# Michaelszeng/GCS-ADMM

Hardware: AMD Instinct MI355X
Metric: admm_iterations_per_sec (higher is better)
Workload: dtype f64; 1 GPU; benchmark4; V=42, E=94, n=2, state_dtype=f64, state_columns=incidence, inner_arithmetic=f64, vertex_program=workgroup, vertex_solves=warm start from the previous iteration's record (csrc/warm_start.h), parallelism=1 GPU

## Files before the change

### gcs_admm_amd/abi.py

```python
from __future__ import annotations

import ctypes as C
import os

import numpy as np

LIB_PATH = os.path.join(os.path.dirname(os.path.abspath(__file__)), "libgcsadmm.so")

F64, F32 = 0, 1
RUNNING, CONVERGED, MAX_IT, DIVERGED = -1, 0, 1, 2
BATCH_LARGE = 1
BATCH_TERMINALS = 4
STATUS_NAME = {RUNNING: "running", CONVERGED: "converged", MAX_IT: "max_it", DIVERGED: "diverged"}


class GraphDesc(C.Structure):
    _fields_ = [("n", C.c_int32), ("num_vertices", C.c_int32), ("num_edges", C.c_int32), ("num_incidences", C.c_int32),
                ("inc_ptr", C.c_void_p), ("inc_edge", C.c_void_p), ("inc_out", C.c_void_p),
                ("edge_inc_tail", C.c_void_p), ("edge_inc_head", C.c_void_p),
                ("poly_ptr", C.c_void_p), ("poly_A", C.c_void_p), ("poly_b", C.c_void_p), ("center", C.c_void_p),
                ("src", C.c_int32), ("dst", C.c_int32), ("state_dtype", C.c_int32), ("device", C.c_int32),
                ("inc_counted", C.c_void_p), ("edge_counted", C.c_void_p),
                ("nx_global", C.c_double), ("nmu_global", C.c_double),
                ("vertex_program", C.c_int32), ("wave_slots", C.c_int32), ("wave_align", C.c_int32),
                ("wave_store_dl", C.c_int32), ("wave_generic_rows", C.c_int32), ("edge_major_columns", C.c_int32),
                ("vertex_workspace", C.c_int32)]


class Params(C.Structure):
    _fields_ = [("rho", C.c_double), ("tau_incr", C.c_double), ("tau_decr", C.c_double), ("nu", C.c_double),
                ("it_rho_limit", C.c_int32), ("max_it", C.c_int32), ("eps_abs", C.c_double), ("eps_rel", C.c_double),
                ("eps_edge", C.c_double), ("ipm_tol", C.c_double), ("ipm_max_iter", C.c_int32), ("cold_start", C.c_int32)]


class State(C.Structure):
    _fields_ = [("copy", C.c_void_p), ("mu", C.c_void_p), ("zedge", C.c_void_p),
                ("xv", C.c_void_p), ("zv", C.c_void_p), ("yv", C.c_void_p)]


class HaloDesc(C.Structure):
    _fields_ = [("num_peers", C.c_int32), ("peer_rank", C.c_void_p), ("send_ptr", C.c_void_p), ("send_cols", C.c_void_p),
                ("recv_ptr", C.c_void_p), ("recv_cols", C.c_void_p)]


class ControlBlock(C.Structure):
    _fields_ = [("rho", C.c_double), ("mu_scale", C.c_double), ("sums", C.c_double * 5),
                ("pri", C.c_double), ("dual", C.c_double), ("eps_pri", C.c_double), ("eps_dual", C.c_double),
                ("it", C.c_int32), ("status", C.c_int32), ("inner_failures", C.c_int32), ("inner_iters", C.c_int32)]


class Snapshot(C.Structure):
    _fields_ = [("n", C.c_int32), ("state_dtype", C.c_int32), ("V", C.c_int32), ("E", C.c_int32),
                ("edge_key", C.c_void_p), ("edge_words", C.c_void_p), ("vertex_id", C.c_void_p), ("vertex_words", C.c_void_p),
                ("rho", C.c_void_p)]


_p, _i, _d = C.c_void_p, C.c_int32, C.c_double
_run, _run_timed = [_p, _p, _i, _p, _p], [_p, _p, _i, _p, _p] + [_p] * 4
_csr = [_i, _i, _p, _p, _p]
PROTOTYPES = {
    "gcsadmm_create": ([_p, _p], _i),
    "gcsadmm_destroy": ([_p], None),
    "gcsadmm_last_error": ([_p], C.c_char_p),
    "gcsadmm_reset": ([_p] * 3, _i),
    "gcsadmm_vertex_step": ([_p] * 3, _i),
    "gcsadmm_edge_step": ([_p] * 4, _i),
    "gcsadmm_control": ([_p] * 4, _i),
    "gcsadmm_run": (_run, _i),
    "gcsadmm_set_fused_tail": ([_p, _i], _i),
    "gcsadmm_read_control": ([_p] * 3, _i),
    "gcsadmm_cost": ([_p, _p, _d, _p, _p], _i),
    "gcsadmm_query": ([_p] * 6, _i),
    "gcsadmm_query_workspace": ([_p] * 4, _i),
    "gcsadmm_unit_iterations": ([_p, _p, _i, _p, _p], _i),
    "gcsadmm_run_timed": (_run_timed, _i),
    "gcsadmm_batch_create": ([_p, _i, _p], _i),
    "gcsadmm_batch_create_ex": ([_p, _i, _i, _p], _i),
    "gcsadmm_batch_query": ([_p] * 4, _i),
    "gcsadmm_batch_query_terminals": ([_p] * 3, _i),
    "gcsadmm_batch_destroy": ([_p], None),
    "gcsadmm_batch_last_error": ([_p], C.c_char_p),
    "gcsadmm_batch_bind": ([_p] * 4, _i),
    "gcsadmm_batch_run": ([_p, _i, _p], _i),
    "gcsadmm_batch_poll": ([_p] * 4, _i),
    "gcsadmm_export_state": ([_p] * 5, _i),
    "gcsadmm_import_state": ([_p] * 5, _i),
    "gcsadmm_batch_export_state": ([_p] * 4, _i),
    "gcsadmm_batch_import_state": ([_p] * 4, _i),
    "gcsadmm_vertex_prox": ([_p] * 6 + [_d, _i, _p, _p], _i),
    "gcsadmm_comm_unique_id": ([_p], _i),
    "gcsadmm_attach_comm": ([_p, _i, _i, _p, _p], _i),
    "gcsadmm_check_halo": ([_p, _i, _i, _p], _i),
    "gcsadmm_run_partitioned": (_run, _i),
    "gcsadmm_run_partitioned_timed": (_run_timed, _i),
    "gcsadmm_set_overlap": ([_p, _i, _p], _i),
    "gcsadmm_comm_count": ([_p, _p], _i),
    "gcsadmm_halo_pack": ([_p] * 3, _i),
    "gcsadmm_halo_unpack": ([_p] * 3, _i),
    "gcsadmm_halo_exchange": ([_p] * 3, _i),
    "gcsadmm_halo_buffers": ([_p] * 4, _i),
    "gcsadmm_polytope_last_error": ([], C.c_char_p),
    "gcsadmm_polytope_centers": (_csr + [_i, _p, _p, _p], _i),
    "gcsadmm_polytope_bounds": (_csr + [_p, _i, _p, _p, _p], _i),
    "gcsadmm_polytope_overlaps": (_csr + [_p, C.c_long, _p, _p, _d, _i, _p, _p], _i),
    "gcsadmm_scene_create": (_csr + [_i, _p], _i),
    "gcsadmm_scene_destroy": ([_p], None),
    "gcsadmm_scene_centers": ([_p] * 4, _i),
    "gcsadmm_scene_bounds": ([_p] * 4, _i),
    "gcsadmm_scene_set_boxes": ([_p] * 3, _i),
    "gcsadmm_scene_candidate_pairs": ([_p, _d, _p], _i),
    "gcsadmm_scene_overlaps": ([_p, _d, _p, _p], _i),
    "gcsadmm_scene_read_pairs": ([_p] * 5, _i),
    "gcsadmm_scene_restrict_paths": ([_p, _i, _p, _p, _p, _d, _i, _p, _p, _p, _p], _i),
    "gcsadmm_scene_locate_points": ([_p, _i, _p, _d, _d, _p], _i),
    "gcsadmm_scene_locate_boxes": ([_p, _i, _p, _p, _d, _p], _i),
    "gcsadmm_scene_read_hits": ([_p] * 4, _i),
    "gcsadmm_scene_project_points": ([_p, _i, _p, _p, _i, _p], _i),
    "gcsadmm_scene_read_projections": ([_p] * 5, _i),
    "gcsadmm_scene_add_regions": ([_p, _i, _p, _p, _p, _d, _d] + [_p] * 6, _i),
    "gcsadmm_scene_remove_regions": ([_p, _i, _p, _p], _i),
    "gcsadmm_scene_read_regions": ([_p] * 7, _i),
    "gcsadmm_scene_build_region_graph": ([_p] * 3, _i),
    "gcsadmm_scene_read_region_graph": ([_p] * 5, _i),
    "gcsadmm_scene_query_graphs": ([_p, _i, _p, _p, _p, _i] + [_p] * 8, _i),
    "gcsadmm_scene_region_paths": ([_p, _i, _p, _p, _p, _i] + [_p] * 4, _i),
    "gcsadmm_scene_informed_regions": ([_p, _i, _p, _p, _d, _p, _p], _i),
    "gcsadmm_scene_region_paths_sets": ([_p, _i, _p, _p, _p, _p, _i] + [_p] * 4, _i),
    "gcsadmm_scene_informed_regions_sets": ([_p, _i, _p, _p, _p, _d, _p, _p], _i),
    "gcsadmm_scene_induced_sizes": ([_p, _i] + [_p] * 6, _i),
    "gcsadmm_scene_induced_query_graphs": ([_p, _i, _p, _p, _p, _p, _i] + [_p] * 9, _i),
    "gcsadmm_walks_create": ([_i] + [_p] * 7 + [_i, _p], _i),
    "gcsadmm_walks_destroy": ([_p], None),
    "gcsadmm_walks_last_error": ([_p], C.c_char_p),
    "gcsadmm_walks_sample": ([_p, _p, _i, _p, _i, _i, _i] + [_p] * 4, _i),
}
EXPORTS = list(PROTOTYPES)


class GcsAdmmError(RuntimeError):
    pass


def check(status, message):
    if status:
        raise GcsAdmmError(message())


_lib = None


def select_library(path: str) -> None:
    global LIB_PATH
    path = os.path.abspath(path)
    if _lib is not None and _lib._name != path:
        raise RuntimeError(f"{_lib._name} is already loaded: select {path} before the first handle is made")
    LIB_PATH = path


def load_library() -> C.CDLL:
    global _lib
    if _lib is None:
        if not os.path.exists(LIB_PATH):
            raise RuntimeError(f"{LIB_PATH} is missing: run `python -m gcs_admm_amd.build` (hipcc, gfx950). "
                               "There is no CPU fallback.")
        import torch
        lib = C.CDLL(LIB_PATH)
        for name, (argtypes, restype) in PROTOTYPES.items():
            f = getattr(lib, name)
            f.argtypes, f.restype = argtypes, restype
        _lib = lib
    return _lib


def graph_desc(g, *, state_dtype, device, num_incidences=None, inc_counted=None, edge_counted=None, nx_global=0.0,
               nmu_global=0.0, columns="incidence", **knobs):
    if columns not in ("incidence", "edge"):
        raise ValueError("columns must be 'incidence' or 'edge'")
    E = g.num_edges
    NI = int(num_incidences) if num_incidences is not None else int(g.inc_ptr[-1])
    tail, head = g.edge_inc_tail.astype(np.int32), g.edge_inc_head.astype(np.int32)
    col_of = np.arange(NI, dtype=np.int64)
    if columns == "edge":
        if NI != 2 * E:
            raise ValueError("edge-major columns need exactly two columns per edge")
        col_of = np.empty(NI, dtype=np.int64)
        col_of[tail] = np.arange(E); col_of[head] = E + np.arange(E)
        tail, head = np.arange(E, dtype=np.int32), (E + np.arange(E)).astype(np.int32)
        if inc_counted is not None:
            ic = np.empty(NI, dtype=np.uint8)
            ic[col_of] = np.asarray(inc_counted, dtype=np.uint8)
            inc_counted = ic
    arrays = dict(inc_ptr=g.inc_ptr.astype(np.int32), inc_edge=g.inc_edge.astype(np.int32), inc_out=g.inc_out.astype(np.int32),
                  edge_inc_tail=tail, edge_inc_head=head, poly_ptr=g.poly_ptr.astype(np.int32), poly_A=g.poly_A.astype(np.float64),
                  poly_b=g.poly_b.astype(np.float64), center=g.interior.astype(np.float64),
                  inc_counted=None if inc_counted is None else np.asarray(inc_counted, dtype=np.uint8),
                  edge_counted=None if edge_counted is None else np.asarray(edge_counted, dtype=np.uint8))
    arrays = {k: None if a is None else np.ascontiguousarray(a) for k, a in arrays.items()}
    desc = GraphDesc(n=g.n, num_vertices=g.num_vertices, num_edges=E, num_incidences=NI, src=g.src, dst=g.dst,
                     state_dtype=state_dtype, device=device, nx_global=float(nx_global), nmu_global=float(nmu_global),
                     edge_major_columns=int(columns == "edge"), **{k: int(v) for k, v in knobs.items()},
                     **{k: None if a is None else a.ctypes.data for k, a in arrays.items()})
    return desc, list(arrays.values()), col_of
```

### gcs_admm_amd/csrc/create_plan.h

```cpp
#pragma once
#include <algorithm>
#include <cmath>
#include <string>
#include <vector>

#include "canonical_box.h"
#include "gcsadmm.h"
#include "state_transfer_core.h"
#include "step_args.h"
#include "vertex_program.h"
#include "warm_start.h"

int gcsadmm_wg_lds_bytes(int n, int units, int facets, bool box = false);
int gcsadmm_wg_lds_bytes_t512(int n, int units, int facets, bool box = false);
bool gcsadmm_wg_has_box(int n);
long long gcsadmm_terminal_ws_doubles(int n, int facets, int live_edges);
long long gcsadmm_terminal_record_doubles(int n, int facets, int live_edges);

namespace gcsadmm_k {

constexpr int REORDER_MIN_UNITS = 512;
constexpr int LDS_CU_BYTES = 160 * 1024;

inline int edge_unroll_rt(int dtype, int c, int E)
{
    const int u = dtype == GCSADMM_F32 ? (c <= 7 ? 4 : 2) : (c <= 7 ? 2 : 1);
    return (E + EDGE_BLOCK * u - 1) / (EDGE_BLOCK * u) >= 256 ? u : 1;
}

struct CreatePlan {
    std::vector<int> deg_in;
    std::vector<double> bc;
    std::vector<int> special_vtx, special_kind;
    int n_term = 0, term_vtx[2] = {-1, -1}, term_is_src[2] = {0, 0};
    long long term_ws_off[2] = {0, 0}, term_rec_off[2] = {0, 0}, term_ws_doubles = 0, term_rec_doubles = 0;
    int term_threads = 256, term_lds_doubles = 0;
    std::vector<int> wg_vtx;
    int wg_lds_bytes = 0, wg_box = 0, wg_t512 = 0;
    std::vector<int> split_vtx;
    std::vector<long long> split_off;
    long long split_doubles = 0;
    int split_lds_bytes = 0;
    std::vector<int> wave_slot_ptr{0}, wave_vtx;
    int slots_cap = 1, align_rows = 0, store_dl = 0, all_m4 = 0;
    int wave_mm = 1;
    int lds_bytes = 0;
    std::vector<long long> warm_ptr;
    bool wave_reorder = false, wg_reorder = false;
    std::vector<int> prox_vtx;
    int prox_lds_bytes = 0;
    std::vector<char> col_owned;
    std::vector<int> col_vertex;
    double nx = 0, nmu = 0;
    int edge_unroll = 1, edge_blocks = 1;
    int fused_tail = 0;
    std::vector<int> edge_tail, edge_head;
    int edges_ascending = 0;
    int n_waves() const { return (int)wave_slot_ptr.size() - 1; }
};

inline gcsadmm_status check_graph_desc(const gcsadmm_graph_desc *g, std::string &err)
{
    auto fail = [&](gcsadmm_status st, const char *msg) { err = msg; return st; };
    if (!g) return fail(GCSADMM_ERR_BAD_ARG, "null descriptor or output pointer");
    if (g->n < 1 || g->n > 8) return fail(GCSADMM_ERR_UNSUPPORTED, "the vertex kernels are instantiated for n = 1 .. 8");
    if (g->num_vertices < 0 || g->num_edges < 0) return fail(GCSADMM_ERR_BAD_ARG, "negative size");
    if (!g->inc_ptr || !g->poly_ptr || (g->num_edges > 0 && (!g->inc_edge || !g->inc_out || !g->edge_inc_tail || !g->edge_inc_head)) ||
        (g->num_vertices > 0 && (!g->poly_A || !g->poly_b || !g->center)))
        return fail(GCSADMM_ERR_BAD_ARG, "null graph array");
    if (g->state_dtype != GCSADMM_F64 && g->state_dtype != GCSADMM_F32) return fail(GCSADMM_ERR_BAD_ARG, "bad state_dtype");
    const int NIo = g->inc_ptr[g->num_vertices];
    if (g->inc_ptr[0] != 0 || NIo < 0 || g->num_incidences < NIo) return fail(GCSADMM_ERR_BAD_ARG, "inconsistent incidence CSR");
    return GCSADMM_OK;
}

inline gcsadmm_status make_create_plan(const gcsadmm_graph_desc &g, CreatePlan &p, std::string &err)
{
    auto fail = [&](gcsadmm_status st, const char *msg) { err = msg; return st; };
    const int V = g.num_vertices, E = g.num_edges, n = g.n;
    p = CreatePlan();

    std::vector<int> deg(V), fac(V);
    p.deg_in.assign(V, 0);
    int mm_all = 1;
    for (int v = 0; v < V; ++v) {
        const int lo = g.inc_ptr[v], hi = g.inc_ptr[v + 1];
        if (hi < lo) return fail(GCSADMM_ERR_BAD_ARG, "inc_ptr not monotone");
        bool seen_out = false;
        for (int k = lo; k < hi; ++k) {
            if (g.inc_edge[k] < 0 || g.inc_edge[k] >= E) return fail(GCSADMM_ERR_BAD_ARG, "inc_edge out of range");
            if (g.inc_out[k]) seen_out = true;
            else { if (seen_out) return fail(GCSADMM_ERR_BAD_ARG, "incoming incidences must precede outgoing ones"); p.deg_in[v]++; }
        }
        deg[v] = hi - lo;
        fac[v] = g.poly_ptr[v + 1] - g.poly_ptr[v];
        if (fac[v] < n + 1) return fail(GCSADMM_ERR_BAD_ARG, "polytope with fewer than n+1 facets cannot be bounded");
        mm_all = std::max(mm_all, fac[v]);
    }
    for (int e = 0; e < E; ++e)
        if (g.edge_inc_tail[e] < 0 || g.edge_inc_tail[e] >= g.num_incidences || g.edge_inc_head[e] < 0 || g.edge_inc_head[e] >= g.num_incidences)
            return fail(GCSADMM_ERR_BAD_ARG, "edge incidence slot out of range");
    if (g.edge_major_columns != 0 && g.edge_major_columns != 1) return fail(GCSADMM_ERR_BAD_ARG, "edge_major_columns must be 0 or 1");
    if (g.edge_major_columns) {
        if (g.num_incidences != 2 * (int64_t)E) return fail(GCSADMM_ERR_BAD_ARG, "edge-major columns: num_incidences must be 2 num_edges");
        for (int e = 0; e < E; ++e)
            if (g.edge_inc_tail[e] != e || g.edge_inc_head[e] != E + e)
                return fail(GCSADMM_ERR_BAD_ARG, "edge-major columns: edge_inc_tail[e] must be e and edge_inc_head[e] num_edges + e");
    }
    p.edge_tail.assign(E, -1); p.edge_head.assign(E, -1);
    for (int v = 0; v < V; ++v)
        for (int k = g.inc_ptr[v]; k < g.inc_ptr[v + 1]; ++k) (g.inc_out[k] ? p.edge_tail : p.edge_head)[g.inc_edge[k]] = v;
    p.edges_ascending = transfer_edges_ascend(E, p.edge_tail.data(), p.edge_head.data());
    auto poly_A = [&](int v) { return g.poly_A + (size_t)g.poly_ptr[v] * n; };

    const int MT = g.poly_ptr[V];
    p.bc.assign(MT > 0 ? MT : 1, 0.0);
    for (int v = 0; v < V; ++v)
        for (int j = g.poly_ptr[v]; j < g.poly_ptr[v + 1]; ++j) {
            double s = g.poly_b[j];
            for (int k = 0; k < n; ++k) s -= g.poly_A[(size_t)j * n + k] * g.center[(size_t)v * n + k];
            p.bc[j] = s;
            if (v != g.src && v != g.dst && !(s > 0.0)) return fail(GCSADMM_ERR_BAD_ARG, "center is not strictly inside its polytope");
        }

    auto live_edges = [&](int v, bool is_src) { return is_src ? deg[v] - p.deg_in[v] : p.deg_in[v]; };
    for (int term : {g.src, g.dst}) {
        if (term < 0 || term >= V) continue;
        double ext = 0;
        for (int j = g.poly_ptr[term]; j < g.poly_ptr[term + 1]; ++j) {
            double nrm = 0;
            for (int k = 0; k < n; ++k) nrm += g.poly_A[(size_t)j * n + k] * g.poly_A[(size_t)j * n + k];
            ext = std::max(ext, std::fabs(p.bc[j]) / std::sqrt(nrm > 0 ? nrm : 1.0));
        }
        if (ext > 1e-5) {
            if (g.src == g.dst) return fail(GCSADMM_ERR_UNSUPPORTED, "source and target are the same region");
            if (live_edges(term, term == g.src) < 1)
                return fail(GCSADMM_ERR_UNSUPPORTED, "a terminal that is a region needs an edge on its live side (outgoing for the source, incoming for the target)");
            p.term_vtx[p.n_term] = term; p.term_is_src[p.n_term] = term == g.src; ++p.n_term;
        }
    }
    auto is_region_terminal = [&](int v) { return (p.n_term > 0 && v == p.term_vtx[0]) || (p.n_term > 1 && v == p.term_vtx[1]); };
    auto is_special = [&](int v) { return v == g.src || v == g.dst || p.deg_in[v] == 0 || deg[v] - p.deg_in[v] == 0; };
    int n_generic = 0;
    for (int v = 0; v < V; ++v) n_generic += !is_region_terminal(v) && !is_special(v);
    constexpr int WG_AUTO_MAX = 1024;
    if (g.vertex_program < 0 || g.vertex_program > 3) return fail(GCSADMM_ERR_BAD_ARG, "vertex_program must be 0, 1, 2 or 3");
    if (g.vertex_workspace < 0 || g.vertex_workspace > 2) return fail(GCSADMM_ERR_BAD_ARG, "vertex_workspace must be 0, 1 or 2");
    const int ws_mode = g.vertex_workspace;
    const bool prefer_wg = g.vertex_program >= 2 || (g.vertex_program == 0 && n_generic <= WG_AUTO_MAX);
    bool wg_box = g.wave_generic_rows == 0 && gcsadmm_wg_has_box(n);
    bool wave_box = n == 2 && g.wave_generic_rows != 1 && g.wave_generic_rows != 2;
    std::vector<int> wave_cand;
    p.warm_ptr.assign(V + 1, 0);
    for (int v = 0; v < V; ++v) {
        p.warm_ptr[v + 1] = p.warm_ptr[v];
        if (is_region_terminal(v)) continue;
        if (is_special(v)) {
            if (deg[v] > MAX_SPECIAL_DEG) return fail(GCSADMM_ERR_UNSUPPORTED, "terminal vertex degree above 256");
            p.special_vtx.push_back(v);
            p.special_kind.push_back(v == g.src ? 1 : (v == g.dst ? 2 : 0));
            continue;
        }
        p.warm_ptr[v + 1] += gcs_ws::warm_record_doubles(n, fac[v], deg[v]);
        const bool wave_too_small = ws_mode == 1 && n == 2 && (size_t)gcs::lds_doubles(n, fac[v], 1, 0) * 8 > (size_t)LDS_CU_BYTES;
        if (n != 2 || deg[v] + 1 > gcs::WAVE || prefer_wg || wave_too_small) {
            p.wg_vtx.push_back(v);
            if (wg_box && !canonical_box(n, fac[v], poly_A(v))) wg_box = false;
        } else {
            wave_cand.push_back(v);
            p.wave_mm = std::max(p.wave_mm, fac[v]);
            if (wave_box && !canonical_box(2, fac[v], poly_A(v))) wave_box = false;
        }
    }

    const int n_wg = (int)p.wg_vtx.size();
    p.wg_t512 = n_wg > 0 && g.vertex_program != 3 && n_wg + 1 <= 256;
    p.wg_box = n_wg > 0 && wg_box;
    auto wg_bytes = [&](int v) { return p.wg_t512 ? gcsadmm_wg_lds_bytes_t512(n, deg[v] + 1, fac[v], wg_box)
                                                  : gcsadmm_wg_lds_bytes(n, deg[v] + 1, fac[v], wg_box); };
    if (ws_mode > 0) {
        std::vector<int> keep;
        for (int v : p.wg_vtx) (ws_mode == 2 || wg_bytes(v) > LDS_CU_BYTES ? p.split_vtx : keep).push_back(v);
        p.wg_vtx.swap(keep);
    }
    for (int v : p.wg_vtx) p.wg_lds_bytes = std::max(p.wg_lds_bytes, wg_bytes(v));
    if (p.wg_lds_bytes > LDS_CU_BYTES) return fail(GCSADMM_ERR_UNSUPPORTED, "a vertex sub-problem (degree x facets) does not fit the 160 KB of LDS of a CU");
    auto heavier = [&](int a, int b) { return (long)(deg[a] + 1) * fac[a] > (long)(deg[b] + 1) * fac[b]; };
    std::stable_sort(p.wg_vtx.begin(), p.wg_vtx.end(), heavier);
    std::stable_sort(p.split_vtx.begin(), p.split_vtx.end(), heavier);
    for (int v : p.split_vtx) {
        const int lds = gcsadmm_wg_lds_bytes(n, 0, fac[v], wg_box);
        if (lds > LDS_CU_BYTES) return fail(GCSADMM_ERR_UNSUPPORTED, "a vertex's border system and polytope do not fit the 160 KB of LDS of a CU");
        p.split_lds_bytes = std::max(p.split_lds_bytes, lds);
        p.split_off.push_back(p.split_doubles);
        p.split_doubles += ((gcsadmm_wg_lds_bytes(n, deg[v] + 1, fac[v], wg_box) - lds) / 8 + 31) / 32 * 32;
    }

    auto lds_need = [&](int slots, int store_dl) {
        return (size_t)(wave_box ? gcs_box::lds_doubles(n, p.wave_mm, slots, store_dl) : gcs::lds_doubles(n, p.wave_mm, slots, store_dl)) * 8;
    };
    int slots_max = gcs::MAX_SLOTS;
    if (!wave_cand.empty()) {
        while (slots_max > 1 && lds_need(slots_max, 0) > LDS_CU_BYTES) --slots_max;
        if (lds_need(slots_max, 0) > LDS_CU_BYTES) return fail(GCSADMM_ERR_UNSUPPORTED, "facet count too large for LDS");
        if (g.wave_slots > 0) slots_max = std::max(1, std::min(slots_max, (int)g.wave_slots));
        else slots_max = std::min(slots_max, std::max(1, ((int)wave_cand.size() + 1023) / 1024));
    }
    auto pack = [&](int align) {
        p.wave_slot_ptr.assign(1, 0); p.wave_vtx.clear();
        int lanes = 0, slots = 0, slots_used = 0;
        for (int v : wave_cand) {
            int base = gcs::group_base(lanes, deg[v], p.deg_in[v], align);
            if (base < 0 || slots + 1 > slots_max) {
                p.wave_slot_ptr.push_back((int)p.wave_vtx.size());
                slots = 0;
                base = gcs::group_base(0, deg[v], p.deg_in[v], align);
            }
            p.wave_vtx.push_back(v);
            lanes = base + deg[v] + 1; slots += 1;
            slots_used = std::max(slots_used, slots);
        }
        if ((int)p.wave_vtx.size() > p.wave_slot_ptr.back()) p.wave_slot_ptr.push_back((int)p.wave_vtx.size());
        p.slots_cap = std::max(1, slots_used);
    };
    pack(1);
    p.align_rows = g.wave_align == 1 ? 1 : (g.wave_align == 2 ? 0 : (p.n_waves() > 2048 ? 0 : 1));
    if (!p.align_rows) pack(0);
    p.all_m4 = wave_box ? 2 : 0;
    if (p.n_waves() > 0) {
        p.store_dl = g.wave_store_dl == 1 ? 1 : (g.wave_store_dl == 2 ? 0 : (lds_need(p.slots_cap, 1) <= 40 * 1024 ? 1 : 0));
        if (p.store_dl && lds_need(p.slots_cap, 1) > LDS_CU_BYTES) p.store_dl = 0;
        p.lds_bytes = (int)lds_need(p.slots_cap, p.store_dl);
    }

    long long largest = 0;
    int rows = 0;
    for (int i = 0; i < p.n_term; ++i) {
        const int v = p.term_vtx[i], live = live_edges(v, p.term_is_src[i]);
        const long long need = gcsadmm_terminal_ws_doubles(n, fac[v], live);
        p.term_ws_off[i] = p.term_ws_doubles; p.term_ws_doubles += need; largest = std::max(largest, need);
        p.term_rec_off[i] = p.term_rec_doubles; p.term_rec_doubles += gcsadmm_terminal_record_doubles(n, fac[v], live);
        rows = std::max(rows, live * 2 * fac[v]);
    }
    if (p.n_term > 0) {
        p.term_lds_doubles = largest * 8 <= 48 * 1024 ? (int)largest : 0;
        p.term_threads = rows <= 256 ? 64 : 256;
    }

    p.wave_reorder = p.n_waves() >= REORDER_MIN_UNITS;
    p.wg_reorder = n_wg >= REORDER_MIN_UNITS;
    for (int v = 0; v < V; ++v)
        if (v != g.src && v != g.dst) p.prox_vtx.push_back(v);
    p.prox_lds_bytes = gcsadmm_wg_lds_bytes(n, 1, mm_all);

    const size_t ncol = (size_t)std::max<int64_t>(g.num_incidences, 1);
    p.col_owned.assign(ncol, 0);
    p.col_vertex.assign(ncol, -1);
    for (int v = 0; v < V; ++v)
        for (int k = g.inc_ptr[v]; k < g.inc_ptr[v + 1]; ++k) {
            const int col = state_column(g.edge_major_columns, E, 0, k, g.inc_edge[k], g.inc_out[k]);
            p.col_owned[col] = 1; p.col_vertex[col] = v;
        }
    p.nx = g.nx_global > 0 ? g.nx_global : (4.0 * n + 1) * (V + 2.0 * E);
    p.nmu = g.nmu_global > 0 ? g.nmu_global : (4.0 * n + 2) * E;
    p.edge_unroll = edge_unroll_rt(g.state_dtype, 2 * n + 1, E);
    const int tile = EDGE_BLOCK * p.edge_unroll;
    p.edge_blocks = std::max(1, std::min((E + tile - 1) / tile, 2048));
    const bool partitioned = g.num_incidences > g.inc_ptr[V] || g.inc_counted != nullptr || g.edge_counted != nullptr;
    p.fused_tail = p.edge_blocks == 1 && E <= EDGE_BLOCK && p.n_waves() == 0 && p.split_vtx.empty() && p.n_term == 0 && !p.wg_vtx.empty() && !partitioned;
    return GCSADMM_OK;
}

}
```

### gcs_admm_amd/csrc/edge_step.h

```cpp
#pragma once
#include <hip/hip_runtime.h>

#include <cstdint>

#include "gcsadmm.h"
#include "step_args.h"

namespace gcsadmm_k {

constexpr int EDGE_WAVE = 64;

template <class T> struct EdgeArgs {
    int E, NI, c;
    const int *edge_inc_tail, *edge_inc_head;
    const uint8_t *inc_counted, *edge_counted;
    const T *copy;
    T *zedge, *mu;
    double *partials;
};
template <class U, class V> EdgeArgs<U> retype(const EdgeArgs<V> &a)
{
    return EdgeArgs<U>{a.E, a.NI, a.c, a.edge_inc_tail, a.edge_inc_head, a.inc_counted, a.edge_counted, (const U *)a.copy, (U *)a.zedge, (U *)a.mu, a.partials};
}

__device__ __forceinline__ double wave_sum(double v)
{
#pragma unroll
    for (int off = 32; off > 0; off >>= 1) v += __shfl_down(v, off, 64);
    return v;
}

__device__ __forceinline__ double scaled_plus(double scale, double x, double r)
{
#pragma clang fp contract(off)
    return scale * x + r;
}

struct ControlParams {
    double tau_incr, tau_decr, nu, eps_abs, eps_rel, nx, nmu;
    int it_rho_limit, max_it;
};

struct EdgeInKernel {
    static constexpr bool TAIL = false;
    template <class T> static __device__ __forceinline__ T load_copy(const T *p) { return *p; }
    static __device__ __forceinline__ int load_counter(const int *p) { return *p; }
    static __device__ __forceinline__ void store_counter(int *p, int v) { *p = v; }
    static __device__ __forceinline__ bool edge_thread() { return true; }
    static __device__ __forceinline__ void sync() { __syncthreads(); }
};
struct EdgeInTail {
    static constexpr bool TAIL = true;
    template <class T> static __device__ __forceinline__ T load_copy(const T *p) { return __hip_atomic_load(p, __ATOMIC_RELAXED, __HIP_MEMORY_SCOPE_AGENT); }
    static __device__ __forceinline__ int load_counter(const int *p) { return __hip_atomic_load(p, __ATOMIC_RELAXED, __HIP_MEMORY_SCOPE_AGENT); }
    static __device__ __forceinline__ void store_counter(int *p, int v) { __hip_atomic_store(p, v, __ATOMIC_RELAXED, __HIP_MEMORY_SCOPE_AGENT); }
    static __device__ __forceinline__ bool edge_thread() { return threadIdx.x < (unsigned)EDGE_BLOCK; }
    static __device__ __forceinline__ void sync() { __syncthreads(); }
};

struct EdgePre {
    int it = 0, ih = 0;
    double mu_scale = 1.0;
};
template <class T> __device__ __forceinline__ EdgePre edge_prefetch(const EdgeArgs<T> &a, double mu_scale)
{
    EdgePre p;
    p.mu_scale = mu_scale;
    if (threadIdx.x < (unsigned)EDGE_BLOCK && a.E > 0) {
        const int e = (int)threadIdx.x, ee = e < a.E ? e : a.E - 1;
        p.it = a.edge_inc_tail ? a.edge_inc_tail[ee] : ee; p.ih = a.edge_inc_head ? a.edge_inc_head[ee] : a.E + ee;
    }
    return p;
}

template <class P = EdgeInKernel>
__device__ void control_body(gcsadmm_control_block *cb, const double *sums, const ControlParams &p, int *counters, double *trace,
                             bool global_fails = false)
{
    if (cb->status != GCSADMM_RUNNING) return;
    double s[5];
    for (int k = 0; k < 5; ++k) { s[k] = sums[k]; cb->sums[k] = s[k]; }
    const int it = cb->it;
    double rho = cb->rho;
    const int fails = global_fails ? (int)(sums[5] + 0.5) : P::load_counter(&counters[0]), iters = P::load_counter(&counters[1]);
    P::store_counter(&counters[0], 0); P::store_counter(&counters[1], 0);
    cb->inner_failures = fails; cb->inner_iters = iters;
    const double tot = s[0] + s[1] + s[2] + s[3] + s[4];
    if (!(fabs(tot) <= 1.7976931348623157e308)) {
        cb->status = GCSADMM_DIVERGED;
        return;
    }
    const double pri = sqrt(s[0]), dual = rho * sqrt(2.0 * s[1]);
    double mu_scale = 1.0;
    if (pri >= p.nu * dual && it < p.it_rho_limit) { rho *= p.tau_incr; mu_scale = 1.0 / p.tau_incr; }
    else if (dual >= p.nu * pri && it < p.it_rho_limit) { rho *= 1.0 / p.tau_decr; mu_scale = p.tau_incr; }
    const double eps_pri = sqrt(p.nx) * p.eps_abs + p.eps_rel * fmax(sqrt(s[2]), sqrt(2.0 * s[3]));
    const double eps_dual = sqrt(p.nmu) * p.eps_abs + p.eps_rel * mu_scale * sqrt(s[4]);
    cb->rho = rho; cb->mu_scale = mu_scale;
    cb->pri = pri; cb->dual = dual; cb->eps_pri = eps_pri; cb->eps_dual = eps_dual;
    if (trace) {
        double *tr = trace + (size_t)(it - 1) * 6;
        tr[0] = rho; tr[1] = pri; tr[2] = dual; tr[3] = eps_pri; tr[4] = eps_dual; tr[5] = (double)fails;
    }
    if (pri < eps_pri && dual < eps_dual) { cb->status = GCSADMM_CONVERGED; return; }
    cb->it = it + 1;
    if (it + 1 > p.max_it) cb->status = GCSADMM_MAX_IT;
}

template <class T, int C> __host__ __device__ constexpr int edge_unroll() { return sizeof(T) == 4 ? (C <= 7 ? 4 : 2) : (C <= 7 ? 2 : 1); }

template <class T>
__device__ __forceinline__ void edge_word(const EdgeArgs<T> &a, int w, int e, int it, int ih, T cu_t, T cw_t, T zo_t, T mu_t, T mw_t, double mu_scale,
                                          double we, double wt, double wh, double (&s)[5])
{
    const double cu = (double)cu_t, cw = (double)cw_t, zo = (double)zo_t;
    const T zn_t = (T)(0.5 * (cu + cw));
    const double zn = (double)zn_t;
    const double ru = cu - zn, rw = cw - zn;
    const T mu_u_t = (T)scaled_plus(mu_scale, (double)mu_t, ru);
    const T mu_w_t = (T)scaled_plus(mu_scale, (double)mw_t, rw);
    a.mu[(size_t)w * a.NI + it] = mu_u_t;
    a.mu[(size_t)w * a.NI + ih] = mu_w_t;
    a.zedge[(size_t)w * a.E + e] = zn_t;
    const double mu_u = (double)mu_u_t, mu_w = (double)mu_w_t;
    s[0] += wt * ru * ru + wh * rw * rw;
    s[1] += we * (zn - zo) * (zn - zo);
    s[2] += wt * cu * cu + wh * cw * cw;
    s[3] += we * zn * zn;
    s[4] += wt * mu_u * mu_u + wh * mu_w * mu_w;
}

#ifndef GCS_TAIL_WORDS
#define GCS_TAIL_WORDS 5
#endif
template <class T, int C> __host__ __device__ constexpr int tail_words() { return C < GCS_TAIL_WORDS ? C : GCS_TAIL_WORDS; }

template <class T, int MODE, int C, int U, class P = EdgeInKernel>
__device__ __forceinline__ void edge_body(const EdgeArgs<T> &a, gcsadmm_control_block *cb, double *sums, const ControlParams &cp, int *counters,
                                          double *trace, unsigned *ticket, const unsigned bx, const unsigned nblocks, double (*red)[5], int *is_last,
                                          const EdgePre &pre = EdgePre())
{
    static_assert(!P::TAIL || (MODE == 1 && U == 1), "the tail of the vertex launch is the single-workgroup edge step");
    double mu_scale;
    if constexpr (P::TAIL) mu_scale = pre.mu_scale;
    else {
        if (cb->status != GCSADMM_RUNNING) return;
        mu_scale = cb->mu_scale;
    }
    double s[5] = {0, 0, 0, 0, 0};
    if constexpr (P::TAIL) {
        constexpr int CH = tail_words<T, C>();
        const int e = (int)threadIdx.x;
        if (P::edge_thread() && e < a.E) {
            const int it = pre.it, ih = pre.ih;
            const double we = a.edge_counted ? (double)a.edge_counted[e] : 1.0;
            const double wt = a.inc_counted ? (double)a.inc_counted[it] : 1.0;
            const double wh = a.inc_counted ? (double)a.inc_counted[ih] : 1.0;
#pragma unroll
            for (int w0 = 0; w0 < C; w0 += CH) {
                T cu_[CH], cw_[CH], zo_[CH], mu_[CH], mw_[CH];
#pragma unroll
                for (int j = 0; j < CH; ++j) {
                    const int w = w0 + j;
                    if (w >= C) break;
                    cu_[j] = P::load_copy(&a.copy[(size_t)w * a.NI + it]); cw_[j] = P::load_copy(&a.copy[(size_t)w * a.NI + ih]);
                    zo_[j] = a.zedge[(size_t)w * a.E + e];
                    mu_[j] = a.mu[(size_t)w * a.NI + it]; mw_[j] = a.mu[(size_t)w * a.NI + ih];
                }
#pragma unroll
                for (int j = 0; j < CH; ++j) {
                    const int w = w0 + j;
                    if (w >= C) break;
                    edge_word(a, w, e, it, ih, cu_[j], cw_[j], zo_[j], mu_[j], mw_[j], mu_scale, we, wt, wh, s);
                }
            }
        }
    } else
    for (int base = bx * (U * EDGE_BLOCK); base < a.E; base += nblocks * (U * EDGE_BLOCK)) {
        int it[U], ih[U];
        T cu_[U][C], cw_[U][C], zo_[U][C], mu_[U][C], mw_[U][C];
#pragma unroll
        for (int q = 0; q < U; ++q) {
            const int e = base + q * EDGE_BLOCK + (int)threadIdx.x, ee = e < a.E ? e : a.E - 1;
            it[q] = a.edge_inc_tail ? a.edge_inc_tail[ee] : ee; ih[q] = a.edge_inc_head ? a.edge_inc_head[ee] : a.E + ee;
#pragma unroll
            for (int w = 0; w < C; ++w) {
                cu_[q][w] = a.copy[(size_t)w * a.NI + it[q]]; cw_[q][w] = a.copy[(size_t)w * a.NI + ih[q]];
                zo_[q][w] = a.zedge[(size_t)w * a.E + ee];
                mu_[q][w] = a.mu[(size_t)w * a.NI + it[q]]; mw_[q][w] = a.mu[(size_t)w * a.NI + ih[q]];
            }
        }
#pragma unroll
        for (int q = 0; q < U; ++q) {
            const int e = base + q * EDGE_BLOCK + (int)threadIdx.x;
            if (e >= a.E) break;
            const double we = a.edge_counted ? (double)a.edge_counted[e] : 1.0;
            const double wt = a.inc_counted ? (double)a.inc_counted[it[q]] : 1.0;
            const double wh = a.inc_counted ? (double)a.inc_counted[ih[q]] : 1.0;
#pragma unroll
            for (int w = 0; w < C; ++w)
                edge_word(a, w, e, it[q], ih[q], cu_[q][w], cw_[q][w], zo_[q][w], mu_[q][w], mw_[q][w], mu_scale, we, wt, wh, s);
        }
    }
    const int lane = threadIdx.x & 63, wv = threadIdx.x >> 6;
#pragma unroll
    for (int k = 0; k < 5; ++k) {
        const double t = wave_sum(s[k]);
        if (lane == 0 && P::edge_thread()) red[wv][k] = t;
    }
    P::sync();
    if (threadIdx.x < 5) {
        double t = 0;
        for (int q = 0; q < EDGE_BLOCK / EDGE_WAVE; ++q) t += red[q][threadIdx.x];
        if (MODE >= 2) __hip_atomic_store(&a.partials[(size_t)bx * 5 + threadIdx.x], t, __ATOMIC_RELAXED, __HIP_MEMORY_SCOPE_AGENT);
        else a.partials[(size_t)bx * 5 + threadIdx.x] = t;
        if (MODE == 1) sums[threadIdx.x] = t;
        if constexpr (P::TAIL) red[0][threadIdx.x] = t;
    }
    if (MODE == 1) {
        P::sync();
        if (threadIdx.x == 0) control_body<P>(cb, P::TAIL ? &red[0][0] : sums, cp, counters, trace);
    }
    if (MODE >= 2) {
        if (threadIdx.x < EDGE_WAVE) asm volatile("s_waitcnt vmcnt(0)" ::: "memory");
        if (threadIdx.x == 0) {
            const unsigned t = __hip_atomic_fetch_add(ticket, 1u, __ATOMIC_RELAXED, __HIP_MEMORY_SCOPE_AGENT);
            *is_last = (t == nblocks - 1);
        }
        __syncthreads();
        if (!*is_last) return;
        double acc[5] = {0, 0, 0, 0, 0};
        for (int b = threadIdx.x; b < (int)nblocks; b += EDGE_BLOCK)
            for (int k = 0; k < 5; ++k) acc[k] += __hip_atomic_load(&a.partials[(size_t)b * 5 + k], __ATOMIC_RELAXED, __HIP_MEMORY_SCOPE_AGENT);
        __syncthreads();
        for (int k = 0; k < 5; ++k) red[threadIdx.x][k] = acc[k];
        __syncthreads();
        for (int off = EDGE_BLOCK / 2; off > 0; off >>= 1) {
            if ((int)threadIdx.x < off)
                for (int k = 0; k < 5; ++k) red[threadIdx.x][k] += red[threadIdx.x + off][k];
            __syncthreads();
        }
        if (threadIdx.x < 5) sums[threadIdx.x] = red[0][threadIdx.x];
        __syncthreads();
        if (threadIdx.x == 0) {
            if (MODE == 2) control_body(cb, sums, cp, counters, trace);
            else sums[5] = (double)counters[0];
            __hip_atomic_store(ticket, 0u, __ATOMIC_RELAXED, __HIP_MEMORY_SCOPE_AGENT);
        }
    }
}

}
```

### gcs_admm_amd/csrc/gcsadmm.hip

```cpp
#include <hip/hip_runtime.h>

#include <algorithm>
#include <cmath>
#include <cstdio>
#include <cstring>
#include <memory>
#include <new>
#include <string>
#include <type_traits>
#include <vector>

#include "gcsadmm.h"
#include "hip_owners.h"
#include "terminal_launch.h"
#ifdef GCS_PHASE_TIMING
__device__ unsigned long long g_sub_cycles[16];
__device__ __forceinline__ void gcs_stamp(int k)
{
    static __shared__ unsigned long long last;
    __builtin_amdgcn_sched_barrier(0);
    if (threadIdx.x == 0) {
        const unsigned long long t = __builtin_amdgcn_s_memtime();
        if (k > 0) atomicAdd(&g_sub_cycles[k], t - last);
        last = t;
    }
    __builtin_amdgcn_sched_barrier(0);
}
#define GCS_STAMP(k) gcs_stamp(k)
#endif
#include "vertex_kernel.h"
#include "vertex_wave_batch_kernel.h"
#include "vertex_wg_launch.h"
#include "warm_start.h"
#include "canonical_box.h"
#include "create_plan.h"
#include "batch_plan.h"
#include "edge_step.h"
#include "halo_plan.h"
#include "loop_kernels.h"
#include "rccl_api.h"

struct Halo : HaloPlan {
    DevBuf<int> d_send_cols, d_send_base, d_send_stride, d_recv_cols, d_recv_base, d_recv_stride;
    DevBuf<char> d_sendbuf, d_recvbuf;
    DevBuf<double> d_sums6;
    bool attached() const { return (bool)d_sums6; }
};
struct Overlap {
    int n_wave_b = 0;
    DevBuf<int> d_split_ids, d_split_order;
    Stream comm_stream;
    Event ev_boundary, ev_halo;
};
struct Terminals {
    DevBuf<double> d_term_ws, d_term_rec;
    Stream term_stream;
    Event ev_term_fork, ev_term_join;
};

struct gcsadmm_handle_s {
    int n = 0, V = 0, E = 0, NI = 0, c = 0, dtype = 0, device = 0, src = -1, dst = -1;
    int edge_major = 0;
    CreatePlan plan;
    gcsadmm_params params{};
    bool params_set = false;
    int vertex_steps = 0;
    unsigned resets = 0;
    gcsadmm_batch_s *batch = nullptr;
    std::vector<gcsadmm_batch_s *> batches;
    int overlap_mode = 0;
    int fused_tail_mode = 1;
    std::string err;
    void *comm = nullptr;
    int rank = 0, world = 1;
    std::vector<int> iota;
    struct Graph {
        DevBuf<int> d_inc_ptr, d_deg_in, d_inc_edge, d_poly_ptr, d_edge_inc_tail, d_edge_inc_head;
        DevBuf<int> d_edge_tail, d_edge_head;
        DevBuf<int> d_wave_slot_ptr, d_wave_vtx, d_special_vtx, d_special_kind, d_wg_vtx;
        DevBuf<double> d_poly_A, d_poly_bc, d_center;
        DevBuf<uint8_t> d_inc_counted, d_edge_counted;
        DevBuf<int> d_split_vtx;
        DevBuf<long long> d_split_off;
        DevBuf<double> d_split_ws;
        DevBuf<double> d_warm;
        DevBuf<long long> d_warm_ptr;
        DevBuf<int> d_wave_iters, d_wave_order, d_wg_iters, d_wg_order;
    } g;
    struct Loop {
        DevBuf<gcsadmm_control_block> d_cb;
        DevBuf<int> d_counters;
        DevBuf<double> d_partials, d_sums;
        DevBuf<unsigned> d_ticket;
        DevBuf<char> d_transfer;
    } loop;
    struct Prox { DevBuf<int> d_prox_vtx, d_prox_counters; } prox;
    Halo halo;
    Overlap overlap;
    Terminals term;
    std::vector<Event> events;

    int n_special() const { return (int)g.d_special_vtx.size(); }
    int n_wg() const { return (int)g.d_wg_vtx.size(); }
    int n_split() const { return (int)g.d_split_vtx.size(); }
    bool fuses() const { return plan.fused_tail && fused_tail_mode != 0 && !halo.attached(); }
};

struct gcsadmm_batch_s {
    int device = 0;
    std::string err;
    std::vector<gcsadmm_handle> members;
    std::vector<unsigned> resets;
    std::vector<gcsadmm_state> states;
    DevBuf<char> d_transfer;
    BatchPlan plan;
    bool bound = false;
    unsigned flags = 0;
    DevBuf<char> d_vertex_table, d_edge_table;
    DevBuf<char> d_wave_table;
    DevBuf<const gcsadmm_control_block *> d_cbs;
    DevBuf<int> d_poll;
    DevBuf<char> d_term_table;
    Stream term_stream;
    Event ev_term_fork, ev_term_join;
    std::vector<int> poll_host;
};


static thread_local std::string g_create_error;

#define HIPCHK(obj, call)                                                                            \
    do {                                                                                             \
        hipError_t e_ = (call);                                                                      \
        if (e_ != hipSuccess) {                                                                      \
            (obj)->err = std::string(#call) + ": " + hipGetErrorString(e_);                          \
            return GCSADMM_ERR_HIP;                                                                  \
        }                                                                                            \
    } while (0)

template <class F> static gcsadmm_status entry(std::string &err, F &&body)
{
    try {
        return body();
    } catch (const std::bad_alloc &) {
        try { err = "out of host memory"; } catch (...) { err.clear(); }
        return GCSADMM_ERR_NO_MEMORY;
    }
}
template <class O, class A, class F> static gcsadmm_status guarded_entry(O *obj, A &&args, F &&body)
{
    if (!obj) return GCSADMM_ERR_BAD_ARG;
    return entry(obj->err, [&]() -> gcsadmm_status {
        const gcsadmm_status refused = args();
        if (refused != GCSADMM_OK) return refused;
        DeviceGuard device_guard_(obj->device);
        if (device_guard_.err != hipSuccess) { obj->err = std::string("hipSetDevice: ") + hipGetErrorString(device_guard_.err); return GCSADMM_ERR_HIP; }
        return body();
    });
}
template <class A, class F> static gcsadmm_status handle_entry(gcsadmm_handle h, A &&args, F &&body) { return guarded_entry(h, args, body); }
template <class A, class F> static gcsadmm_status batch_entry(gcsadmm_batch_s *b, A &&args, F &&body) { return guarded_entry(b, args, body); }
static gcsadmm_status bad_unless(bool ok) { return ok ? GCSADMM_OK : GCSADMM_ERR_BAD_ARG; }

template <class F> static auto with_state(const gcsadmm_handle_s *h, F &&f) { return with_state_type(h->dtype == GCSADMM_F64, f); }
static size_t state_bytes(const gcsadmm_handle_s *h) { return h->dtype == GCSADMM_F64 ? 8 : 4; }

static ControlParams control_params(const gcsadmm_handle_s *h)
{
    const gcsadmm_params &p = h->params;
    return ControlParams{p.tau_incr, p.tau_decr, p.nu, p.eps_abs, p.eps_rel, h->plan.nx, h->plan.nmu, p.it_rho_limit, p.max_it};
}

static StepDesc make_step_graph(gcsadmm_handle h)
{
    StepDesc a{};
    a.inc_ptr = h->g.d_inc_ptr.get(); a.deg_in = h->g.d_deg_in.get(); a.inc_edge = h->g.d_inc_edge.get(); a.poly_ptr = h->g.d_poly_ptr.get();
    a.poly_A = h->g.d_poly_A.get(); a.poly_bc = h->g.d_poly_bc.get(); a.center = h->g.d_center.get();
    return a;
}
static StepDesc make_step(gcsadmm_handle h, const gcsadmm_state *st)
{
    StepDesc a = make_step_graph(h);
    a.E = h->E; a.NI = h->NI; a.edge_major = h->edge_major;
    a.zedge = st->zedge; a.mu = st->mu; a.copy = st->copy; a.xv = st->xv; a.zv = st->zv; a.yv = st->yv;
    a.counters = h->loop.d_counters.get(); a.cb = h->loop.d_cb.get();
    a.eps_edge = h->params.eps_edge; a.ipm_tol = h->params.ipm_tol; a.ipm_max_iter = h->params.ipm_max_iter;
    a.warm = h->params.cold_start ? nullptr : h->g.d_warm.get(); a.warm_ptr = h->g.d_warm_ptr.get();
    return a;
}

static WgLaunchDesc make_wg_desc(gcsadmm_handle h, const gcsadmm_state *st, bool with_special)
{
    WgLaunchDesc d;
    d.step = make_step(h, st);
    d.n = h->n; d.dtype = h->dtype; d.n_vtx = h->n_wg(); d.n_special = with_special ? h->n_special() : 0; d.lds_bytes = h->plan.wg_lds_bytes;
    d.vtx = h->g.d_wg_vtx.get(); d.special_vtx = h->g.d_special_vtx.get(); d.special_kind = h->g.d_special_kind.get(); d.box = h->plan.wg_box;
    d.order = h->g.d_wg_order.get(); d.unit_iters = h->g.d_wg_iters.get();
    return d;
}

static gcsadmm_k::TermLaunchDesc make_term_desc(gcsadmm_handle h, const gcsadmm_state *st)
{
    gcsadmm_k::TermLaunchDesc d;
    const CreatePlan &p = h->plan;
    d.step = make_step(h, st);
    d.n = h->n; d.dtype = h->dtype; d.count = p.n_term; d.threads = p.term_threads; d.lds_doubles = p.term_lds_doubles;
    for (int i = 0; i < 2; ++i) {
        d.t.vtx[i] = p.term_vtx[i]; d.t.is_src[i] = p.term_is_src[i]; d.t.ws_off[i] = p.term_ws_off[i]; d.t.rec_off[i] = p.term_rec_off[i];
    }
    d.t.ws = h->term.d_term_ws.get();
    d.t.rec = h->params.cold_start ? nullptr : h->term.d_term_rec.get();
    return d;
}

static VertexLaunchDesc make_launch_desc(gcsadmm_handle h, const gcsadmm_state *st)
{
    VertexLaunchDesc d;
    const CreatePlan &p = h->plan;
    d.step = make_step(h, st);
    d.n_waves = p.n_waves(); d.n_special = h->n_special(); d.all_m4 = p.all_m4; d.lds_bytes = p.lds_bytes; d.align_rows = p.align_rows;
    d.store_dl = p.store_dl; d.MM = p.wave_mm;
    d.wave_slot_ptr = h->g.d_wave_slot_ptr.get(); d.wave_vtx = h->g.d_wave_vtx.get(); d.special_vtx = h->g.d_special_vtx.get(); d.special_kind = h->g.d_special_kind.get();
    d.wave_order = h->g.d_wave_order.get(); d.wave_iters = h->g.d_wave_iters.get();
    return d;
}

struct VertexLaunch {
    int part = -1;
    bool reorder = false;
    const WgTailDesc *tail = nullptr;
};
static gcsadmm_status launch_vertex(gcsadmm_handle h, const gcsadmm_state *st, hipStream_t s, const VertexLaunch &req = {})
{
    const int part = req.part;
    const auto &g = h->g;
    const int n_waves = h->plan.n_waves();
    const gcsadmm_control_block *cb = h->loop.d_cb.get();
    auto launch_waves = [&](const VertexLaunchDesc &d) { with_state(h, [&](auto t) { launch_vertex_dim<2, decltype(t)>(d, s); }); };
    const bool with_term = h->plan.n_term > 0 && part <= 0;
    if (with_term) {
        HIPCHK(h, hipEventRecord(h->term.ev_term_fork.get(), s));
        HIPCHK(h, hipStreamWaitEvent(h->term.term_stream.get(), h->term.ev_term_fork.get(), 0));
        gcsadmm_terminal_launch(make_term_desc(h, st), h->term.term_stream.get());
        HIPCHK(h, hipEventRecord(h->term.ev_term_join.get(), h->term.term_stream.get()));
    }
    struct Join {
        gcsadmm_handle h; hipStream_t s; bool on;
        ~Join() { if (on) (void)hipStreamWaitEvent(s, h->term.ev_term_join.get(), 0); }
    } join_{h, s, with_term};
    if (part >= 0) {
        const Overlap &o = h->overlap;
        VertexLaunchDesc d = make_launch_desc(h, st);
        const int off = part ? o.n_wave_b : 0, cnt = part ? n_waves - o.n_wave_b : o.n_wave_b;
        d.wave_order = o.d_split_order.get() + off;
        d.n_waves = cnt;
        if (part) d.n_special = 0;
        launch_waves(d);
        if (req.reorder && g.d_wave_iters)
            hipLaunchKernelGGL(reorder_kernel, dim3(1), dim3(REORDER_THREADS), 0, s, cnt, g.d_wave_iters.get(), o.d_split_order.get() + off, cb, o.d_split_ids.get() + off);
        HIPCHK(h, hipGetLastError());
        return GCSADMM_OK;
    }
    const bool special_on_wave = n_waves > 0;
    if (n_waves > 0) launch_waves(make_launch_desc(h, st));
    if (h->n_wg() > 0 || (!special_on_wave && h->n_special() > 0)) {
        WgLaunchDesc d = make_wg_desc(h, st, !special_on_wave);
        if (req.tail) d.tail = *req.tail;
        if (h->plan.wg_t512) gcsadmm_wg_launch_t512(d, s);
        else gcsadmm_wg_launch(d, s);
    }
    if (h->n_split() > 0) {
        WgLaunchDesc d = make_wg_desc(h, st, false);
        d.n_vtx = h->n_split(); d.vtx = g.d_split_vtx.get(); d.lds_bytes = h->plan.split_lds_bytes; d.order = nullptr; d.unit_iters = nullptr;
        gcsadmm_wg_launch_split(d, WgSplitArgs{g.d_split_ws.get(), g.d_split_off.get()}, s);
    }
    if (++h->vertex_steps % REORDER_EVERY == 0) {
        if (g.d_wave_order) hipLaunchKernelGGL(reorder_kernel, dim3(1), dim3(REORDER_THREADS), 0, s, n_waves, g.d_wave_iters.get(), g.d_wave_order.get(), cb);
        if (g.d_wg_order) hipLaunchKernelGGL(reorder_kernel, dim3(1), dim3(REORDER_THREADS), 0, s, h->n_wg(), g.d_wg_iters.get(), g.d_wg_order.get(), cb);
    }
    HIPCHK(h, hipGetLastError());
    return GCSADMM_OK;
// ... 344 lines not shown
        HIPCHK(b, hipEventRecord(b->ev_term_join.get(), b->term_stream.get()));
    }
    if (bp.vertex_grid_x > 0)
        gcsadmm_wg_launch_batch(WgBatchLaunch{bp.n, bp.dtype, bp.box, b->d_vertex_table.get(), (unsigned)bp.vertex_grid_x, (unsigned)bp.wg_members.size(), bp.vertex_lds_bytes}, s);
    each_wave_launch(b, [&](const WaveBatchLaunch &w) { wave_batch_launch(w, s); });
    if (with_term) HIPCHK(b, hipStreamWaitEvent(s, b->ev_term_join.get(), 0));
    with_state_type(bp.dtype == GCSADMM_F64, [&](auto t) {
        using T = decltype(t);
        const auto *table = (const EdgeBatchEntry<T> *)b->d_edge_table.get();
        dispatch_dim<1, 2, 3, 4, 5, 6, 7, 8>(bp.n, [&](auto N) {
            hipLaunchKernelGGL((edge_batch_kernel<T, 2 * decltype(N)::value + 1>), dim3(bp.edge_grid_x, bp.count), dim3(EDGE_BLOCK), 0, s, table);
        });
    });
    HIPCHK(b, hipGetLastError());
    return GCSADMM_OK;
}

static gcsadmm_status partitioned_tail(gcsadmm_handle h, const gcsadmm_state *st, double *trace_dev, hipStream_t s, const Event *ev)
{
    double *sums6 = h->halo.d_sums6.get();
    gcsadmm_status r = launch_edge(h, st, sums6, s, EdgeMode::Sums6);
    if (r != GCSADMM_OK) return r;
    if (ev) HIPCHK(h, hipEventRecord(ev[0].get(), s));
    const double *reduced = sums6;
    if (h->comm) {
        NCCLCHK(h, rccl().AllReduce(sums6, sums6 + 6, 6, ncclFloat64, ncclSum, (ncclComm_t)h->comm, s));
        reduced = sums6 + 6;
    }
    if (ev) HIPCHK(h, hipEventRecord(ev[1].get(), s));
    hipLaunchKernelGGL(control_kernel, dim3(1), dim3(1), 0, s, h->loop.d_cb.get(), reduced, control_params(h), h->loop.d_counters.get(), trace_dev, true);
    HIPCHK(h, hipGetLastError());
    if (ev) HIPCHK(h, hipEventRecord(ev[2].get(), s));
    return GCSADMM_OK;
}

static gcsadmm_status run_partitioned_loop(gcsadmm_handle h, const gcsadmm_state *st, int k, double *trace_dev, hipStream_t s, const Event *ev)
{
    if (!h->comm && h->world > 1) { h->err = "gcsadmm_run_partitioned needs a communicator (gcsadmm_attach_comm with an id)"; return GCSADMM_ERR_BAD_ARG; }
    gcsadmm_status r;
    const Overlap &o = h->overlap;
    if (!ev && o.n_wave_b > 0 && h->overlap_mode != 2) {
        hipStream_t sc = o.comm_stream.get();
        for (int i = 0; i < k; ++i) {
            const bool reorder = ++h->vertex_steps % REORDER_EVERY == 0;
            HIPCHK(h, hipEventRecord(o.ev_boundary.get(), s));
            HIPCHK(h, hipStreamWaitEvent(sc, o.ev_boundary.get(), 0));
            if ((r = launch_vertex(h, st, sc, VertexLaunch{0, reorder})) != GCSADMM_OK) return r;
            if ((r = halo_exchange(h, st, sc)) != GCSADMM_OK) return r;
            HIPCHK(h, hipEventRecord(o.ev_halo.get(), sc));
            if ((r = launch_vertex(h, st, s, VertexLaunch{1, reorder})) != GCSADMM_OK) return r;
            HIPCHK(h, hipStreamWaitEvent(s, o.ev_halo.get(), 0));
            if ((r = partitioned_tail(h, st, trace_dev, s, nullptr)) != GCSADMM_OK) return r;
        }
        HIPCHK(h, hipEventRecord(o.ev_halo.get(), sc));
        HIPCHK(h, hipStreamWaitEvent(s, o.ev_halo.get(), 0));
        return GCSADMM_OK;
    }
    for (int i = 0; i < k; ++i) {
        if (ev) HIPCHK(h, hipEventRecord(ev[6 * i + 0].get(), s));
        if ((r = launch_vertex(h, st, s)) != GCSADMM_OK) return r;
        if (ev) HIPCHK(h, hipEventRecord(ev[6 * i + 1].get(), s));
        if ((r = halo_exchange(h, st, s)) != GCSADMM_OK) return r;
        if (ev) HIPCHK(h, hipEventRecord(ev[6 * i + 2].get(), s));
        if ((r = partitioned_tail(h, st, trace_dev, s, ev ? ev + 6 * i + 3 : nullptr)) != GCSADMM_OK) return r;
    }
    return GCSADMM_OK;
}
static gcsadmm_status need_partitioned(gcsadmm_handle h, bool args_ok)
{
    if (!args_ok) return GCSADMM_ERR_BAD_ARG;
    if (!h->halo.attached()) h->err = "gcsadmm_attach_comm has not been called";
    return bad_unless(h->halo.attached());
}

extern "C" gcsadmm_status gcsadmm_batch_create_ex(const gcsadmm_handle *members, int32_t count, int32_t flags, struct gcsadmm_batch_s **out)
{
    if (out) *out = nullptr;
    return entry(g_create_error, [&]() -> gcsadmm_status {
        std::unique_ptr<gcsadmm_batch_s> b;
        gcsadmm_status st = batch_make(members, count, (unsigned)flags, out, b);
        if (st != GCSADMM_OK) return st;
        st = guarded_entry(b.get(), [] { return GCSADMM_OK; }, [&] { return batch_finish(b, hipSuccess, out); });
        if (b) g_create_error = b->err;
        return st;
    });
}

extern "C" {

const char *gcsadmm_last_error(gcsadmm_handle h) { return h ? h->err.c_str() : g_create_error.c_str(); }

void gcsadmm_destroy(gcsadmm_handle h)
{
    if (!h) return;
    DeviceGuard device_guard_(h->device);
    batches_forget(h);
    if (h->comm && rccl().ok()) (void)rccl().CommDestroy((ncclComm_t)h->comm);
    delete h;
}

gcsadmm_status gcsadmm_create(const gcsadmm_graph_desc *g, gcsadmm_handle *out)
{
    if (out) *out = nullptr;
    return entry(g_create_error, [&]() -> gcsadmm_status {
        auto fail = [&](gcsadmm_status st, const std::string &msg) { g_create_error = msg; return st; };
        std::string msg;
        gcsadmm_status st;
        if (!out) return fail(GCSADMM_ERR_BAD_ARG, "null descriptor or output pointer");
        if ((st = check_graph_desc(g, msg)) != GCSADMM_OK) return fail(st, msg);
        int ndev = 0;
        if (hipGetDeviceCount(&ndev) != hipSuccess || ndev <= 0) return fail(GCSADMM_ERR_NO_DEVICE, "no HIP device");
        if (g->device < 0 || g->device >= ndev) return fail(GCSADMM_ERR_BAD_ARG, "device ordinal out of range");
        CreatePlan plan;
        if ((st = make_create_plan(*g, plan, msg)) != GCSADMM_OK) return fail(st, msg);

        const int V = g->num_vertices, E = g->num_edges, n = g->n, NIo = g->inc_ptr[V], MT = g->poly_ptr[V];
        DeviceGuard device_guard_(g->device);
        auto h = std::make_unique<gcsadmm_handle_s>();
        h->n = n; h->V = V; h->E = E; h->NI = g->num_incidences; h->c = 2 * n + 1;
        h->edge_major = g->edge_major_columns; h->src = g->src; h->dst = g->dst;
        h->dtype = g->state_dtype; h->device = g->device;
        h->plan = std::move(plan);
        CreatePlan &p = h->plan;
        auto bail = [&](hipError_t e, const char *what) { return fail(GCSADMM_ERR_HIP, std::string(what) + ": " + hipGetErrorString(e)); };
        hipError_t e;
        if ((e = device_guard_.err) != hipSuccess) return bail(e, "hipSetDevice");
#define UP(group, dst, src, cnt) if ((e = h->group.dst.upload(src, (size_t)(cnt))) != hipSuccess) return bail(e, "upload " #dst)
        UP(g, d_inc_ptr, g->inc_ptr, V + 1);
        UP(g, d_deg_in, p.deg_in.data(), V);
        UP(g, d_inc_edge, g->inc_edge, NIo);
        UP(g, d_poly_ptr, g->poly_ptr, V + 1);
        UP(g, d_edge_inc_tail, g->edge_inc_tail, E);
        UP(g, d_edge_inc_head, g->edge_inc_head, E);
        UP(g, d_wave_slot_ptr, p.wave_slot_ptr.data(), p.wave_slot_ptr.size());
        UP(g, d_wave_vtx, p.wave_vtx.data(), p.wave_vtx.size());
        UP(g, d_special_vtx, p.special_vtx.data(), p.special_vtx.size());
        UP(g, d_special_kind, p.special_kind.data(), p.special_kind.size());
        UP(g, d_wg_vtx, p.wg_vtx.data(), p.wg_vtx.size());
        if (!p.split_vtx.empty()) {
            UP(g, d_split_vtx, p.split_vtx.data(), p.split_vtx.size());
            UP(g, d_split_off, p.split_off.data(), p.split_off.size());
            UP(g, d_split_ws, nullptr, p.split_doubles);
        }
        UP(g, d_poly_A, g->poly_A, (size_t)MT * n);
        UP(g, d_poly_bc, p.bc.data(), MT);
        UP(g, d_center, g->center, (size_t)V * n);
        if (g->inc_counted) UP(g, d_inc_counted, g->inc_counted, g->num_incidences);
        if (g->edge_counted) UP(g, d_edge_counted, g->edge_counted, E);
        UP(loop, d_cb, nullptr, 1);
        UP(loop, d_counters, nullptr, 2);
        UP(loop, d_partials, nullptr, (size_t)p.edge_blocks * 5);
        UP(loop, d_sums, nullptr, 5);
        UP(loop, d_ticket, nullptr, 1);
        if (p.n_term > 0) {
            UP(term, d_term_ws, nullptr, p.term_ws_doubles);
            UP(term, d_term_rec, nullptr, p.term_rec_doubles);
            if ((e = create_owned(h->term.term_stream, hipStreamCreateWithFlags, hipStreamNonBlocking)) != hipSuccess) return bail(e, "hipStreamCreate");
            if ((e = create_owned(h->term.ev_term_fork, hipEventCreateWithFlags, hipEventDisableTiming)) != hipSuccess) return bail(e, "hipEventCreate");
            if ((e = create_owned(h->term.ev_term_join, hipEventCreateWithFlags, hipEventDisableTiming)) != hipSuccess) return bail(e, "hipEventCreate");
        }
        UP(g, d_warm_ptr, p.warm_ptr.data(), V + 1);
        UP(g, d_warm, nullptr, p.warm_ptr[V]);
        const int n_waves = p.n_waves(), n_wg = h->n_wg();
        h->iota.resize(std::max(std::max(n_waves, n_wg), 1));
        for (size_t i = 0; i < h->iota.size(); ++i) h->iota[i] = (int)i;
        if (p.wave_reorder) { UP(g, d_wave_iters, nullptr, n_waves); UP(g, d_wave_order, h->iota.data(), n_waves); }
        if (p.wg_reorder) { UP(g, d_wg_iters, nullptr, n_wg); UP(g, d_wg_order, h->iota.data(), n_wg); }
        UP(prox, d_prox_vtx, p.prox_vtx.data(), p.prox_vtx.size());
        UP(prox, d_prox_counters, nullptr, 2);
#undef UP
        auto release = [](auto &v) { v.clear(); v.shrink_to_fit(); };
        release(p.bc); release(p.deg_in); release(p.warm_ptr); release(p.prox_vtx); release(p.special_vtx); release(p.special_kind);
        release(p.wg_vtx); release(p.split_vtx); release(p.split_off);
        if (p.lds_bytes > 48 * 1024) {
            e = with_state(h.get(), [&](auto t) { return set_lds_attr<2, decltype(t)>(p.all_m4, p.lds_bytes); });
            if (e != hipSuccess) return bail(e, "hipFuncSetAttribute(MaxDynamicSharedMemorySize)");
        }
        if (p.wg_lds_bytes > 48 * 1024 && (e = p.wg_t512 ? gcsadmm_wg_set_lds_t512(h->n, h->dtype, p.wg_lds_bytes)
                                                          : gcsadmm_wg_set_lds(h->n, h->dtype, p.wg_lds_bytes)) != hipSuccess)
            return bail(e, "hipFuncSetAttribute(MaxDynamicSharedMemorySize, workgroup program)");
        if (p.split_lds_bytes > 48 * 1024 && (e = gcsadmm_wg_set_split_lds(h->n, h->dtype, p.split_lds_bytes)) != hipSuccess)
            return bail(e, "hipFuncSetAttribute(MaxDynamicSharedMemorySize, split workgroup program)");
        *out = h.release();
        return GCSADMM_OK;
    });
}

gcsadmm_status gcsadmm_reset(gcsadmm_handle h, const gcsadmm_params *p, void *stream)
{
    return handle_entry(h, [&] {
        if (!p) return GCSADMM_ERR_BAD_ARG;
        if (!(p->rho > 0) || p->max_it < 1 || !(p->ipm_tol > 0) || p->ipm_max_iter < 1) { h->err = "bad parameter"; return GCSADMM_ERR_BAD_ARG; }
        h->params = *p; h->params_set = true; ++h->resets;
        return GCSADMM_OK;
    }, [&] {
        gcsadmm_control_block cb{};
        cb.rho = p->rho; cb.mu_scale = 1.0; cb.it = 1; cb.status = GCSADMM_RUNNING;
        hipStream_t s = (hipStream_t)stream;
        HIPCHK(h, hipMemcpyAsync(h->loop.d_cb.get(), &cb, sizeof(cb), hipMemcpyHostToDevice, s));
        HIPCHK(h, h->loop.d_counters.zero(s));
        HIPCHK(h, h->g.d_warm.zero(s));
        HIPCHK(h, h->term.d_term_rec.zero(s));
        h->vertex_steps = 0;
        const Overlap &o = h->overlap;
        if (o.d_split_order) HIPCHK(h, hipMemcpyAsync(o.d_split_order.get(), o.d_split_ids.get(), sizeof(int) * o.d_split_order.size(), hipMemcpyDeviceToDevice, s));
        for (const DevBuf<int> *order : {&h->g.d_wave_order, &h->g.d_wg_order})
            if (*order) HIPCHK(h, hipMemcpyAsync(order->get(), h->iota.data(), sizeof(int) * order->size(), hipMemcpyHostToDevice, s));
        HIPCHK(h, hipStreamSynchronize(s));
        return GCSADMM_OK;
    });
}

gcsadmm_status gcsadmm_vertex_step(gcsadmm_handle h, const gcsadmm_state *st, void *stream)
{
    return handle_entry(h, [&] { return bad_unless(state_ok(h, st)); }, [&] { return launch_vertex(h, st, (hipStream_t)stream); });
}

gcsadmm_status gcsadmm_edge_step(gcsadmm_handle h, const gcsadmm_state *st, double *sums_dev, void *stream)
{
    return handle_entry(h, [&] { return bad_unless(state_ok(h, st) && sums_dev); },
                        [&] { return launch_edge(h, st, sums_dev, (hipStream_t)stream, EdgeMode::Partials); });
}

gcsadmm_status gcsadmm_control(gcsadmm_handle h, const double *sums_dev, double *trace_dev, void *stream)
{
    return handle_entry(h, [&] { return bad_unless(sums_dev && h->params_set); }, [&] {
        hipLaunchKernelGGL(control_kernel, dim3(1), dim3(1), 0, (hipStream_t)stream, h->loop.d_cb.get(), sums_dev, control_params(h), h->loop.d_counters.get(), trace_dev, false);
        HIPCHK(h, hipGetLastError());
        return GCSADMM_OK;
    });
}

gcsadmm_status gcsadmm_run(gcsadmm_handle h, const gcsadmm_state *st, int32_t k, double *trace_dev, void *stream)
{
    return handle_entry(h, [&] { return bad_unless(state_ok(h, st) && k >= 0); }, [&] {
        hipStream_t s = (hipStream_t)stream;
        gcsadmm_status r = GCSADMM_OK;
        if (h->fuses()) {
            const WgTailDesc tail = make_wg_tail(h, st, trace_dev);
            for (int i = 0; i < k && r == GCSADMM_OK; ++i) r = launch_vertex(h, st, s, VertexLaunch{-1, false, &tail});
            return r;
        }
        const EdgeMode mode = edge_mode_with_control(h);
        for (int i = 0; i < k && r == GCSADMM_OK; ++i)
            if ((r = launch_vertex(h, st, s)) == GCSADMM_OK) r = launch_edge(h, st, h->loop.d_sums.get(), s, mode, trace_dev);
        return r;
    });
}

gcsadmm_status gcsadmm_comm_unique_id(void *id128)
{
    return entry(g_create_error, [&] {
        if (!id128) return GCSADMM_ERR_BAD_ARG;
        if (!rccl().ok()) { g_create_error = rccl().err; return GCSADMM_ERR_HIP; }
        static_assert(sizeof(ncclUniqueId) == 128, "ncclUniqueId is 128 bytes");
        ncclUniqueId id;
        if (rccl().GetUniqueId(&id) != ncclSuccess) { g_create_error = "ncclGetUniqueId failed"; return GCSADMM_ERR_HIP; }
        std::memcpy(id128, &id, sizeof(id));
        return GCSADMM_OK;
    });
}

gcsadmm_status gcsadmm_check_halo(gcsadmm_handle h, int32_t rank, int32_t world, const gcsadmm_halo_desc *halo)
{
    return h ? check_halo_of(h, rank, world, halo) : GCSADMM_ERR_BAD_ARG;
}

gcsadmm_status gcsadmm_attach_comm(gcsadmm_handle h, int32_t rank, int32_t world, const void *id128, const gcsadmm_halo_desc *halo)
{
    return handle_entry(h, [&] {
        const gcsadmm_status st = check_halo_of(h, rank, world, halo);
        if (st != GCSADMM_OK) return st;
        if (id128 && !rccl().ok()) { h->err = rccl().err; return GCSADMM_ERR_HIP; }
        return GCSADMM_OK;
    }, [&] {
        h->rank = rank; h->world = world;
        const gcsadmm_status st = halo_upload(h, halo);
        if (st != GCSADMM_OK) { h->halo = {}; return st; }
        if (id128) {
            ncclUniqueId id;
            std::memcpy(&id, id128, sizeof(id));
            ncclComm_t comm = nullptr;
            const ncclResult_t r = rccl().CommInitRank(&comm, world, id, rank);
            if (r != ncclSuccess) {
                h->err = std::string("ncclCommInitRank: ") + rccl().text(r);
                h->halo = {};
                return GCSADMM_ERR_HIP;
            }
            h->comm = comm;
        }
        return overlap_setup(h);
    });
}

gcsadmm_status gcsadmm_halo_pack(gcsadmm_handle h, const gcsadmm_state *st, void *stream)
{
    return handle_entry(h, [&] { return bad_unless(need_halo(h, st)); },
                        [&] { return with_state(h, [&](auto t) { return halo_pack<decltype(t)>(h, st, (hipStream_t)stream); }); });
}
gcsadmm_status gcsadmm_halo_unpack(gcsadmm_handle h, const gcsadmm_state *st, void *stream)
{
    return handle_entry(h, [&] { return bad_unless(need_halo(h, st)); },
                        [&] { return with_state(h, [&](auto t) { return halo_unpack<decltype(t)>(h, st, (hipStream_t)stream); }); });
}
gcsadmm_status gcsadmm_halo_buffers(gcsadmm_handle h, void **send_buf, void **recv_buf, int64_t *num_elements)
{
    if (!h || !h->halo.attached()) { if (h) h->err = "no halo attached"; return GCSADMM_ERR_BAD_ARG; }
    if (send_buf) *send_buf = h->halo.d_sendbuf.get();
    if (recv_buf) *recv_buf = h->halo.d_recvbuf.get();
    if (num_elements) *num_elements = (int64_t)h->c * h->halo.n_send;
    return GCSADMM_OK;
}

gcsadmm_status gcsadmm_halo_exchange(gcsadmm_handle h, const gcsadmm_state *st, void *stream)
{
    return handle_entry(h, [&] { return bad_unless(need_halo(h, st)); }, [&] { return halo_exchange(h, st, (hipStream_t)stream); });
}

gcsadmm_status gcsadmm_run_partitioned(gcsadmm_handle h, const gcsadmm_state *st, int32_t k, double *trace_dev, void *stream)
{
    return handle_entry(h, [&] { return need_partitioned(h, state_ok(h, st) && k >= 0); },
                        [&] { return run_partitioned_loop(h, st, k, trace_dev, (hipStream_t)stream, nullptr); });
}

gcsadmm_status gcsadmm_run_partitioned_timed(gcsadmm_handle h, const gcsadmm_state *st, int32_t k, double *trace_dev, void *stream,
                                             float *vertex_ms, float *halo_ms, float *edge_ms, float *reduce_ms)
{
    return handle_entry(h, [&] { return need_partitioned(h, state_ok(h, st) && k >= 0 && vertex_ms && halo_ms && edge_ms && reduce_ms); }, [&] {
        hipStream_t s = (hipStream_t)stream;
        gcsadmm_status r = ensure_events(h, (size_t)6 * k);
        if (r == GCSADMM_OK) r = run_partitioned_loop(h, st, k, trace_dev, s, h->events.data());
        if (r != GCSADMM_OK) return r;
        HIPCHK(h, hipStreamSynchronize(s));
        float *const out[4] = {vertex_ms, halo_ms, edge_ms, reduce_ms};
        const int from[4] = {0, 1, 2, 3}, to[4] = {1, 2, 3, 5};
        for (int q = 0; q < 4 && r == GCSADMM_OK; ++q) r = elapsed_sum(h, 6, k, from[q], to[q], out[q]);
        return r;
    });
}

int32_t gcsadmm_set_fused_tail(gcsadmm_handle h, int32_t mode)
{
    if (!h) return 0;
    h->fused_tail_mode = mode != 0;
    return h->fuses() ? 1 : 0;
}

gcsadmm_status gcsadmm_set_overlap(gcsadmm_handle h, int32_t mode, int32_t *boundary_units)
{
    return handle_entry(h, [&] {
        if (mode < 0 || mode > 2) return GCSADMM_ERR_BAD_ARG;
        if (boundary_units) *boundary_units = 0;
        return need_partitioned(h, true);
    }, [&] {
        h->overlap_mode = mode;
        const gcsadmm_status r = overlap_setup(h);
        if (boundary_units) *boundary_units = h->overlap.n_wave_b;
        return r;
    });
}

gcsadmm_status gcsadmm_comm_count(gcsadmm_handle h, int32_t *count)
{
    return handle_entry(h, [&] {
        if (!count) return GCSADMM_ERR_BAD_ARG;
        *count = 0;
        if (h->comm && !rccl().CommCount) { h->err = "librccl lacks ncclCommCount"; return GCSADMM_ERR_HIP; }
        return GCSADMM_OK;
    }, [&] {
        int n = 0;
        if (h->comm) NCCLCHK(h, rccl().CommCount((ncclComm_t)h->comm, &n));
        *count = n;
        return GCSADMM_OK;
    });
}

gcsadmm_status gcsadmm_vertex_prox(gcsadmm_handle h, const double *q_dev, const double *c_dev, double *xv_dev, double *zv_dev,
                                   double *yv_dev, double ipm_tol, int32_t ipm_max_iter, int32_t *failures_host, void *stream)
{
    return handle_entry(h, [&] {
        if (!q_dev || !c_dev || !xv_dev || !zv_dev || !yv_dev || !(ipm_tol > 0) || ipm_max_iter < 1) { h->err = "bad prox argument"; return GCSADMM_ERR_BAD_ARG; }
        if (h->plan.prox_lds_bytes > 160 * 1024) { h->err = "facet count too large for LDS"; return GCSADMM_ERR_UNSUPPORTED; }
        if (h->plan.n_term > 0) { h->err = "the prox kernel (v1 x-update) takes its terminals as points; this graph has a terminal that is a region"; return GCSADMM_ERR_UNSUPPORTED; }
        return GCSADMM_OK;
    }, [&] {
        hipStream_t s = (hipStream_t)stream;
        HIPCHK(h, h->prox.d_prox_counters.zero(s));
        WgLaunchDesc d{};
        d.n = h->n; d.dtype = GCSADMM_F64; d.n_vtx = (int)h->prox.d_prox_vtx.size(); d.lds_bytes = h->plan.prox_lds_bytes; d.vtx = h->prox.d_prox_vtx.get();
        StepDesc &p = d.step = make_step_graph(h);
        p.xv = xv_dev; p.zv = zv_dev; p.yv = yv_dev; p.counters = h->prox.d_prox_counters.get(); p.ipm_tol = ipm_tol; p.ipm_max_iter = ipm_max_iter;
        gcsadmm_wg_launch_prox(d, q_dev, c_dev, h->src, h->dst, s);
        HIPCHK(h, hipGetLastError());
        if (failures_host) {
            int cnt[2] = {0, 0};
            HIPCHK(h, hipMemcpyAsync(cnt, h->prox.d_prox_counters.get(), sizeof(cnt), hipMemcpyDeviceToHost, s));
            HIPCHK(h, hipStreamSynchronize(s));
            *failures_host = cnt[0];
        }
        return GCSADMM_OK;
    });
}

gcsadmm_status gcsadmm_run_timed(gcsadmm_handle h, const gcsadmm_state *st, int32_t k, double *trace_dev, void *stream,
                                 float *vertex_ms, int32_t *vertex_launches, float *edge_ms, int32_t *edge_launches)
{
    return handle_entry(h, [&] { return bad_unless(state_ok(h, st) && k >= 0 && vertex_ms && edge_ms && vertex_launches && edge_launches); }, [&] {
        hipStream_t s = (hipStream_t)stream;
        gcsadmm_status r = ensure_events(h, (size_t)4 * k);
        if (r != GCSADMM_OK) return r;
        const std::vector<Event> &ev = h->events;
        const EdgeMode mode = edge_mode_with_control(h);
        for (int i = 0; i < k; ++i) {
            HIPCHK(h, hipEventRecord(ev[4 * i + 0].get(), s));
            if ((r = launch_vertex(h, st, s)) != GCSADMM_OK) return r;
            HIPCHK(h, hipEventRecord(ev[4 * i + 1].get(), s));
            HIPCHK(h, hipEventRecord(ev[4 * i + 2].get(), s));
            if ((r = launch_edge(h, st, h->loop.d_sums.get(), s, mode, trace_dev)) != GCSADMM_OK) return r;
            HIPCHK(h, hipEventRecord(ev[4 * i + 3].get(), s));
        }
        HIPCHK(h, hipStreamSynchronize(s));
        if ((r = elapsed_sum(h, 4, k, 0, 1, vertex_ms)) != GCSADMM_OK || (r = elapsed_sum(h, 4, k, 2, 3, edge_ms)) != GCSADMM_OK) return r;
        *vertex_launches = k; *edge_launches = k;
        return GCSADMM_OK;
    });
}

gcsadmm_status gcsadmm_read_control(gcsadmm_handle h, gcsadmm_control_block *out, void *stream)
{
    return handle_entry(h, [&] { return bad_unless(out); }, [&] {
        HIPCHK(h, hipMemcpyAsync(out, h->loop.d_cb.get(), sizeof(*out), hipMemcpyDeviceToHost, (hipStream_t)stream));
        HIPCHK(h, hipStreamSynchronize((hipStream_t)stream));
        return GCSADMM_OK;
    });
}

gcsadmm_status gcsadmm_cost(gcsadmm_handle h, const gcsadmm_state *st, double eps_edge, double *cost_dev, void *stream)
{
    return handle_entry(h, [&] { return bad_unless(st && st->zv && st->zedge && cost_dev); }, [&] {
        with_state(h, [&](auto t) {
            using T = decltype(t);
            hipLaunchKernelGGL((cost_kernel<T>), dim3(1), dim3(256), 0, (hipStream_t)stream, h->V, h->E, h->n, st->zv,
                               (const T *)st->zedge, h->g.d_edge_counted.get(), eps_edge, cost_dev);
        });
        HIPCHK(h, hipGetLastError());
        return GCSADMM_OK;
    });
}

#ifdef GCS_PHASE_TIMING
int gcsadmm_debug_sub_cycles(unsigned long long *out16)
{
    return (int)hipMemcpyFromSymbol(out16, HIP_SYMBOL(g_sub_cycles), 16 * sizeof(unsigned long long));
}

int gcsadmm_debug_phase_cycles(unsigned long long *out64)
{
    return (int)hipMemcpyFromSymbol(out64, HIP_SYMBOL(g_phase_cycles), 64 * sizeof(unsigned long long));
}
#endif

gcsadmm_status gcsadmm_query(gcsadmm_handle h, int32_t *num_waves, int32_t *lds_bytes, int32_t *num_special,
                             int32_t *num_workgroup_vertices, int32_t *workgroup_lds_bytes)
{
    if (!h) return GCSADMM_ERR_BAD_ARG;
    if (num_waves) *num_waves = h->plan.n_waves();
    if (lds_bytes) *lds_bytes = h->plan.lds_bytes;
    if (num_special) *num_special = h->n_special();
    if (num_workgroup_vertices) *num_workgroup_vertices = h->n_wg();
    if (workgroup_lds_bytes) *workgroup_lds_bytes = h->plan.wg_lds_bytes;
    return GCSADMM_OK;
}

gcsadmm_status gcsadmm_query_workspace(gcsadmm_handle h, int32_t *num_split_vertices, int32_t *split_lds_bytes, int64_t *workspace_bytes)
{
    if (!h) return GCSADMM_ERR_BAD_ARG;
    if (num_split_vertices) *num_split_vertices = h->n_split();
    if (split_lds_bytes) *split_lds_bytes = h->plan.split_lds_bytes;
    if (workspace_bytes) *workspace_bytes = (int64_t)((size_t)h->plan.split_doubles * sizeof(double));
    return GCSADMM_OK;
}

gcsadmm_status gcsadmm_unit_iterations(gcsadmm_handle h, int32_t *out, int32_t capacity, int32_t *count, void *stream)
{
    return handle_entry(h, [&] { return bad_unless(count); }, [&] {
        const auto &g = h->g;
        const int *src = g.d_wave_iters ? g.d_wave_iters.get() : g.d_wg_iters.get();
        const int n = g.d_wave_iters ? h->plan.n_waves() : (g.d_wg_iters ? h->n_wg() : 0);
        *count = n;
        if (n == 0 || !out) return GCSADMM_OK;
        HIPCHK(h, hipStreamSynchronize((hipStream_t)stream));
        HIPCHK(h, hipMemcpy(out, src, sizeof(int) * (size_t)(n < capacity ? n : capacity), hipMemcpyDeviceToHost));
        return GCSADMM_OK;
    });
}

const char *gcsadmm_batch_last_error(struct gcsadmm_batch_s *b) { return b ? b->err.c_str() : g_create_error.c_str(); }

void gcsadmm_batch_destroy(struct gcsadmm_batch_s *b)
{
    if (!b) return;
    DeviceGuard device_guard_(b->device);
    batch_unbind(b);
    for (gcsadmm_handle h : b->members)
        if (h) h->batches.erase(std::remove(h->batches.begin(), h->batches.end(), b), h->batches.end());
    delete b;
}

gcsadmm_status gcsadmm_batch_create(const gcsadmm_handle *members, int32_t count, struct gcsadmm_batch_s **out)
{
    if (out) *out = nullptr;
    return entry(g_create_error, [&]() -> gcsadmm_status {
        std::unique_ptr<gcsadmm_batch_s> b;
        const gcsadmm_status st = batch_make(members, count, 0, out, b);
        if (st != GCSADMM_OK) return st;
        DeviceGuard device_guard_(b->device);
        return batch_finish(b, device_guard_.err, out);
    });
}

gcsadmm_status gcsadmm_batch_query(struct gcsadmm_batch_s *b, int32_t *wg_members, int32_t *wave_groups, int32_t *wave_members)
{
    return batch_entry(b, [&] { return GCSADMM_OK; }, [&] {
        const BatchPlan &bp = b->plan;
        if (wg_members) *wg_members = bp.vertex_grid_x > 0 ? (int32_t)bp.wg_members.size() : 0;
        if (wave_groups) *wave_groups = (int32_t)bp.wave_groups.size();
        if (wave_members) *wave_members = (int32_t)std::count_if(bp.wave_grid.begin(), bp.wave_grid.end(), [](int g) { return g > 0; });
        return GCSADMM_OK;
    });
}

gcsadmm_status gcsadmm_batch_query_terminals(struct gcsadmm_batch_s *b, int32_t *term_groups, int32_t *terminals)
{
    return batch_entry(b, [&] { return GCSADMM_OK; }, [&] {
        const BatchPlan &bp = b->plan;
        int32_t total = 0;
        for (const TermGroup &g : bp.term_groups) total += (int32_t)g.member.size();
        if (term_groups) *term_groups = (int32_t)bp.term_groups.size();
        if (terminals) *terminals = total;
        return GCSADMM_OK;
    });
}

gcsadmm_status gcsadmm_batch_bind(struct gcsadmm_batch_s *b, const gcsadmm_state *states, double *const *traces_dev, void *stream)
{
    BatchPlan bp;
    return batch_entry(b, [&] {
        if (!states) { b->err = "null state array"; return GCSADMM_ERR_BAD_ARG; }
        const gcsadmm_status st = batch_plan_of(b->members, b->flags, bp, b->err);
        if (st != GCSADMM_OK) return st;
        for (int i = 0; i < (int)b->members.size(); ++i) {
            gcsadmm_handle h = b->members[i];
            const std::string who = "member " + std::to_string(i) + ": ";
            if (!state_ok(h, &states[i])) { b->err = who + h->err; return GCSADMM_ERR_BAD_ARG; }
            if (h->batch && h->batch != b) { b->err = who + "the handle is bound to another batch (destroy that batch, or bind it to other states, first)"; return GCSADMM_ERR_BAD_ARG; }
        }
        return GCSADMM_OK;
    }, [&] {
        const int count = (int)b->members.size();
        HIPCHK(b, hipStreamSynchronize((hipStream_t)stream));
        batch_unbind(b);
        b->plan = bp;
        const size_t vbytes = gcsadmm_wg_batch_entry_bytes(bp.dtype);
        std::vector<char> vtab(vbytes * bp.wg_members.size());
        std::vector<const gcsadmm_control_block *> cbs((size_t)count);
        b->resets.assign((size_t)count, 0u);
        b->states.assign(states, states + count);
        for (int i = 0; i < count; ++i) {
            cbs[i] = b->members[i]->loop.d_cb.get();
            b->resets[i] = b->members[i]->resets;
        }
        for (size_t r = 0; r < bp.wg_members.size(); ++r) {
            const int i = bp.wg_members[r];
            WgLaunchDesc d = make_wg_desc(b->members[i], &states[i], bp.wave_grid[i] == 0);
            d.order = nullptr;
            gcsadmm_wg_batch_fill(d, vtab.data() + vbytes * r);
        }
        if (!vtab.empty()) HIPCHK(b, hipMemcpy(b->d_vertex_table.get(), vtab.data(), vtab.size(), hipMemcpyHostToDevice));
        const size_t wbytes = wave_batch_entry_bytes(bp.dtype);
        std::vector<char> wtab;
        for (const WaveGroup &g : bp.wave_groups)
            for (int i : g.members) {
                wtab.resize(wtab.size() + wbytes);
                wave_batch_fill(make_launch_desc(b->members[i], &states[i]), bp.dtype, wtab.data() + wtab.size() - wbytes);
            }
// ... 100 lines not shown
```

### gcs_admm_amd/csrc/step_args.h

```cpp
#pragma once
#include <type_traits>

#include "gcs_math.h"

struct gcsadmm_control_block;

namespace gcsadmm_k {

constexpr int MAX_SPECIAL_DEG = 256;
constexpr int EDGE_BLOCK = 256;
constexpr int FUSED_TAIL_LDS_BYTES = (EDGE_BLOCK / 64 * 5 + 1) * 8;
constexpr int wg_launch_lds_bytes(int plan_lds_bytes, bool fused_tail)
{
    int b = 4 * MAX_SPECIAL_DEG * 8;
    if (plan_lds_bytes > b) b = plan_lds_bytes;
    if (fused_tail && FUSED_TAIL_LDS_BYTES > b) b = FUSED_TAIL_LDS_BYTES;
    return b;
}

struct StepArgsBase {
    const int *inc_ptr;
    const int *deg_in;
    const int *inc_edge;
    const int *poly_ptr;
    const double *poly_A;
    const double *poly_bc;
    const double *center;
    int E, NI;
    int edge_major = 0;
    double *xv, *zv, *yv;
    int *counters;
    double eps_edge, ipm_tol;
    int ipm_max_iter;
    double *warm = nullptr;
    const long long *warm_ptr = nullptr;
    int publish = 0;
};

template <class T> GCS_HD void store_copy(T *p, T v, int publish)
{
#if defined(__HIP_DEVICE_COMPILE__)
    if (publish) { __hip_atomic_store(p, v, __ATOMIC_RELAXED, __HIP_MEMORY_SCOPE_AGENT); return; }
#endif
    (void)publish;
    *p = v;
}

template <class T> struct StepArgs : StepArgsBase {
    const T *zedge, *mu;
    T *copy;
};

struct StepDesc : StepArgsBase {
    const void *zedge, *mu;
    void *copy;
    const gcsadmm_control_block *cb;
    template <class T> StepArgs<T> typed() const
    {
        StepArgs<T> a;
        static_cast<StepArgsBase &>(a) = *this;
        a.zedge = (const T *)zedge; a.mu = (const T *)mu; a.copy = (T *)copy;
        return a;
    }
};

GCS_HD int state_column(int edge_major, int E, int lo, int k, int edge, bool out) { return edge_major ? edge + (out ? 0 : E) : lo + k; }
template <class A> GCS_HD int state_column(const A &a, int lo, int k, int edge, bool out) { return state_column(a.edge_major, a.E, lo, k, edge, out); }
template <class A> GCS_HD int state_column(const A &a, int lo, int k, const int *edges, bool out)
{
    return state_column(a.edge_major, a.E, lo, k, a.edge_major ? edges[k] : 0, out);
}

template <class A> GCS_HD double consensus_target(const A &a, int w, int edge, int col, double mu_scale)
{
    return (double)a.zedge[(size_t)w * a.E + edge] - mu_scale * (double)a.mu[(size_t)w * a.NI + col];
}

template <int... Ns, class F> bool dispatch_dim(int n, F &&f)
{
    return ((n == Ns ? (f(std::integral_constant<int, Ns>()), true) : false) || ...);
}

template <class F> auto with_state_type(bool f64, F &&f) { return f64 ? f(double()) : f(float()); }

}
```

### gcs_admm_amd/csrc/vertex_wg.h

```cpp
#pragma once
#include <type_traits>

#include "gcs_math.h"
#include "step_args.h"
#include "warm_start.h"

#if defined(__HIP_DEVICE_COMPILE__)
#define WG_DEVICE 1
#else
#define WG_DEVICE 0
#endif

namespace gcs_wg {

using gcs_math::REG_DELTA;
using gcs_math::rcp;
using gcs_math::rcp1;
using gcs_math::rsqrt_nr;
using gcs_math::sqrt_nr;

#ifndef GCS_WG_THREADS
#define GCS_WG_THREADS 256
#endif
constexpr int WG_THREADS = GCS_WG_THREADS;
// ... 250 lines not shown
template <int DIM> GCS_HD void wave_ldl(double *Mq, double *rd)
{
    static_assert(DIM <= 64, "one row per lane");
#if WG_DEVICE
    const int lane = wg_tid() & 63, row = lane < DIM ? lane : DIM - 1;
    double a[DIM];
#pragma unroll
    for (int j = 0; j < DIM; ++j) a[j] = Mq[row * DIM + j];
    const double od = Mq[row * DIM + row];
    double myr = 0.0;
#pragma unroll
    for (int k = 0; k < DIM; ++k) {
        const double dk = lane_bcast(a[k], k);
        const double odk = lane_bcast(od, k);
        const double rk = rcp(gcs_math::pivot_floor(dk, odk)), col = a[k], l = col * rk;
        a[k] = l;
        if (lane == k) myr = rk;
#pragma unroll
        for (int j = k + 1; j < DIM; ++j) a[j] -= l * lane_bcast(col, j);
    }
    if (lane < DIM) {
#pragma unroll
        for (int j = 0; j < DIM - 1; ++j) Mq[lane * DIM + j] = a[j];
        rd[lane] = myr;
    }
#else
    double od[DIM], col[DIM];
    for (int k = 0; k < DIM; ++k) od[k] = Mq[k * DIM + k];
    for (int k = 0; k < DIM; ++k) {
        const double rk = rcp(gcs_math::pivot_floor(Mq[k * DIM + k], od[k]));
        rd[k] = rk;
        for (int i = k + 1; i < DIM; ++i) col[i] = Mq[i * DIM + k];
        for (int i = k + 1; i < DIM; ++i) {
            const double l = col[i] * rk;
            Mq[i * DIM + k] = l;
            for (int j = k + 1; j <= i; ++j) Mq[i * DIM + j] -= l * col[j];
        }
    }
#endif
}

template <int DIM> GCS_HD void wave_ldl_solve(const double *Mq, const double *rd, const double *b, double *x)
{
#if WG_DEVICE
    const int lane = wg_tid() & 63, row = lane < DIM ? lane : DIM - 1;
    double l[DIM], v = b[row];
#pragma unroll
    for (int k = 0; k < DIM - 1; ++k) l[k] = k < row ? Mq[row * DIM + k] : 0.0;
#pragma unroll
    for (int k = 0; k < DIM - 1; ++k) v -= l[k] * lane_bcast(v, k);
    v *= rd[row];
#pragma unroll
    for (int k = 1; k < DIM; ++k) l[k] = k > row ? Mq[k * DIM + row] : 0.0;
#pragma unroll
    for (int k = DIM - 1; k >= 1; --k) v -= l[k] * lane_bcast(v, k);
    if (lane < DIM) x[lane] = v;
#else
    double v[DIM];
    for (int i = 0; i < DIM; ++i) v[i] = b[i];
    for (int k = 0; k < DIM - 1; ++k)
        for (int i = k + 1; i < DIM; ++i) v[i] -= Mq[i * DIM + k] * v[k];
    for (int i = 0; i < DIM; ++i) v[i] *= rd[i];
    for (int k = DIM - 1; k >= 1; --k)
        for (int i = 0; i < k; ++i) v[i] -= Mq[k * DIM + i] * v[k];
    for (int i = 0; i < DIM; ++i) x[i] = v[i];
#endif
}

template <int DIM, bool LOWREG> GCS_HD void ldl_inverse_col(const double *Lm, const double *rd, int c, double *out, int ldo)
{
    double x[DIM];
#pragma unroll
    for (int i = 0; i < DIM; ++i) {
        double s = (i == c) ? 1.0 : 0.0;
#pragma unroll
        for (int k = 0; k < i; ++k) s -= Lm[i * DIM + k] * x[k];
        x[i] = s;
        if constexpr (DIM > 9) WG_FENCE();
    }
#pragma unroll
    for (int i = DIM - 1; i >= 0; --i) {
        double s = x[i] * rd[i];
#pragma unroll
        for (int k = i + 1; k < DIM; ++k) s -= Lm[k * DIM + i] * x[k];
        x[i] = s;
        if constexpr (LOWREG) out[i * ldo + c] = s;
        if constexpr (DIM > 9) WG_FENCE();
    }
    if constexpr (!LOWREG) {
#pragma unroll
        for (int i = 0; i < DIM; ++i) out[i * ldo + c] = x[i];
    }
}

template <int Q> GCS_HD void soc_apply_W(const double *wb, double eta, const double *x, double *y)
{
    double dd = 0;
#pragma unroll
    for (int k = 1; k < Q; ++k) dd += wb[k] * x[k];
    const double f = x[0] + dd * rcp(1.0 + wb[0]);
    y[0] = eta * (wb[0] * x[0] + dd);
#pragma unroll
    for (int k = 1; k < Q; ++k) y[k] = eta * (x[k] + wb[k] * f);
}
template <int Q> GCS_HD void soc_apply_Wi(const double *wb, double eta, const double *x, double *y)
{
    double dd = 0;
#pragma unroll
    for (int k = 1; k < Q; ++k) dd += wb[k] * x[k];
    const double ieta = rcp(eta), f = -x[0] + dd * rcp(1.0 + wb[0]);
    y[0] = ieta * (wb[0] * x[0] - dd);
#pragma unroll
    for (int k = 1; k < Q; ++k) y[k] = ieta * (x[k] + wb[k] * f);
}
template <int Q> GCS_HD void soc_apply_W2(const double *wb, double eta, const double *x, double *y)
{
    double vx = wb[0] * x[0];
#pragma unroll
    for (int k = 1; k < Q; ++k) vx -= wb[k] * x[k];
    const double ieta = rcp(eta), ie2 = ieta * ieta;
    y[0] = ie2 * (2.0 * wb[0] * vx - x[0]);
#pragma unroll
    for (int k = 1; k < Q; ++k) y[k] = ie2 * (x[k] - 2.0 * wb[k] * vx);
}

#define WG_ROWS_BEGIN_(pl, DS)                                                                                                 \
    WG_FOR_AT(rt_, (BOX ? U * 2 * N : U * m2), (pl).at(BOX ? U * 2 * N : U * m2)) {                                            \
        int u, i, jk_;                                                                                                         \
        if constexpr (BOX) { u = rt_ / (2 * N); const int ik_ = rt_ - u * (2 * N); i = ik_ / N; jk_ = ik_ - i * N; }           \
        else { u = fdiv(rt_, inv_m2); const int rem_ = rt_ - u * m2; i = rem_ >= m; jk_ = rem_ - i * m; }                      \
        double *un = UN(u);                                                                                                    \
        double ap_ = 0, ax_ = 0, adp_ = 0, adx_ = 0;                                                                           \
        if constexpr (BOX) {                                                                                                   \
            ap_ = un[W::P + i * N + jk_]; ax_ = sm[W::XV + i * N + jk_];                                                       \
            if (DS) { adp_ = un[W::DW + i * N + jk_]; adx_ = sm[W::DX + i * N + jk_]; }                                        \
        } else {                                                                                                               \
            _Pragma("unroll") for (int k_ = 0; k_ < N; ++k_) {                                                                 \
                const double a_ = A[jk_ * N + k_];                                                                             \
                ap_ += a_ * un[W::P + i * N + k_]; ax_ += a_ * sm[W::XV + i * N + k_];                                         \
                if (DS) { adp_ += a_ * un[W::DW + i * N + k_]; adx_ += a_ * sm[W::DX + i * N + k_]; }                          \
            }                                                                                                                  \
        }                                                                                                                      \
        const double yy_ = un[W::P + 2 * N], dy_ = DS ? un[W::DW + 2 * N] : 0.0;                                               \
        _Pragma("unroll") for (int rq_ = 0; rq_ < (BOX ? 4 : 2); ++rq_) {                                                      \
            const int ty = BOX ? rq_ >> 1 : rq_, j = BOX ? jk_ + (rq_ & 1) * N : jk_, ro = ty * m2 + i * m + j;                \
            const double sg_ = (BOX && (rq_ & 1)) ? -1.0 : 1.0, b_ = BC[j];                                                    \
            const double s = ty == 0 ? b_ * yy_ - sg_ * ap_ : b_ * (1.0 - yy_) - sg_ * (ax_ - ap_);                            \
            const double ds = ty == 0 ? b_ * dy_ - sg_ * adp_ : -(b_ * dy_) - sg_ * (adx_ - adp_);                             \
            (void)ds;
#define WG_ROWS_BEGIN(pl) WG_ROWS_BEGIN_(pl, false)
#define WG_ROWS_BEGIN_DS(pl) WG_ROWS_BEGIN_(pl, true)
#define WG_ROWS_END() }}

template <int N, class T, bool BOX = false, bool SPLIT = false>
GCS_HD void wg_solve_vertex(const WgArgs<T> &a, int v, double rho, double mu_scale, double *sm, int &status_out, int &iters_out,
                            double *units = nullptr)
{
    using D = WD<N>;
    using SO = WSoc<N>;
    using W = std::conditional_t<BOX, WLBox<N>, WL<N>>;
    constexpr int NW = D::NW, NX = D::NX, NB1 = D::NB1, Q = D::Q, NS = D::NS, TA = D::TA;
#ifndef GCS_WG_CONE_PAIR_MAXN
#define GCS_WG_CONE_PAIR_MAXN 3
#endif
    constexpr bool CONE_PAIR = N <= GCS_WG_CONE_PAIR_MAXN;
    const bool prox = a.prox_q != nullptr;
    const int lo = a.inc_ptr[v], p0 = a.poly_ptr[v];
    int d = prox ? 0 : a.inc_ptr[v + 1] - lo, d_in = prox ? 0 : a.deg_in[v], m = a.poly_ptr[v + 1] - p0;
    int d_out, U, R, m2, US, oR1, oR2;
    bool sides;
    double *PA;
    const double *A, *BC;
    constexpr int oLAM = W::ROWS;
    auto derive = [&] {
        d_out = d - d_in; sides = d > 0;
        U = d + 1; R = 4 * m; m2 = 2 * m;
        US = W::unit_stride(m);
        oR1 = W::ROWS + R; oR2 = W::ROWS + 2 * R;
        PA = sm + W::FIXED + (SPLIT ? 0 : pad2(U * US));
        A = PA; BC = PA + pad2(m * N);
    };
    constexpr bool REGION_OPAQUE = N != 6 && N != 1;
    if constexpr (REGION_OPAQUE) { d = wg_uniform(d); d_in = wg_uniform(d_in); m = wg_uniform(m); }
    derive();
#define WG_REGION()                                                                                                            \
    do {                                                                                                                       \
        if constexpr (REGION_OPAQUE) {                                                                                         \
            gcs_wg::wg_opaque(d); gcs_wg::wg_opaque(d_in); gcs_wg::wg_opaque(m);                                               \
            derive();                                                                                                          \
        }                                                                                                                      \
    } while (0)
    const float inv_m2 = 1.0f / (float)m2;
    double *const UB = SPLIT ? units : sm + W::FIXED;
    auto UN = [&](int u) -> double * { return UB + u * US; };
    constexpr bool WG_VM = SPLIT;
    const double *CEN = sm + W::CEN;
    double *SOC = sm + W::SOC, *SC = sm + W::SC;
    int red_phase = 0;
    WG_STAMP_INIT();
    const int deg = (4 * m + 2) * (d + 1) + 1;
    const double inv_deg = 1.0 / (double)deg;
    auto side_of = [&](int u) { return (u - 1) >= d_in ? 1 : 0; };
    auto side_lo = [&](int s) { return s ? d_in + 1 : 1; };
    auto side_hi = [&](int s) { return s ? d : d_in; };

    using WR = gcs_ws::WRec<N>;
    double *const wrec = (a.warm != nullptr && !prox) ? a.warm + a.warm_ptr[v] : nullptr;
    const int WUS = WR::unit_stride(m);
    double dtm = 0.0;
    Place pl0;
    WG_FOR_AT(t, d * NW, pl0.at(d * NW)) {
        const int e = t / NW, w = t - e * NW, edge = a.inc_edge[lo + e];
        const bool out = e >= d_in;
        const int inc = gcsadmm_k::state_column(a, lo, e, edge, out);
        double *un = UN(e + 1);
        const double Tw = gcsadmm_k::consensus_target(a, w, edge, inc, mu_scale);
        int slot = -1;
        if (w == 2 * N) slot = 2 * N;
        else if (out) slot = w;
        else if (w < N) { un[W::TF + w] = Tw; un[W::TG + N + w] = 0.0; }
        else slot = w - N;
        if (slot >= 0) {
            un[W::TG + slot] = Tw;
            if (wrec) dtm = fmax(dtm, fabs(Tw - wrec[WR::UNITS + (e + 1) * WUS + WR::TG + slot]));
        }
    }
    WG_FOR_AT(t, m * N, pl0.at(m * N)) PA[t] = a.poly_A[(size_t)p0 * N + t];
    WG_FOR_AT(j, m + N, pl0.at(m + N)) {
        if (j < m) PA[pad2(m * N) + j] = a.poly_bc[p0 + j];
        else sm[W::CEN + (j - m)] = a.center[(size_t)v * N + (j - m)];
    }
    if (prox) {
        WG_FOR(k, NX + NW) {
            sm[W::PQ + k] = a.prox_q[(size_t)v * (NX + NW) + k];
            sm[W::PC + k] = a.prox_c[(size_t)v * (NX + NW) + k];
        }
    }
    bool use_warm = false;
    double mu_ref = gcs_ws::WS_COLD_REF, ws_dT = -1.0;
    if (wrec) {
        const Red3 rt = wg_reduce<WG_VM>(Red3{-dtm, 0.0, 0.0}, sm + W::RED, red_phase);
        const bool comparable = wg_uniform((int)(wrec[0] == 1.0 && wrec[1] == rho)) != 0;
        ws_dT = wg_uniform(comparable ? -rt.mn * rho : -1.0);
        use_warm = wg_uniform((int)(comparable && ws_dT <= gcs_ws::ws_theta(wrec))) != 0;
        if (use_warm) mu_ref = wg_uniform(fmax(gcs_ws::WS_MU_MIN, gcs_ws::WS_KAPPA * ws_dT));
    }
    const bool ws_started_warm = use_warm;
    const float inv_R2 = 1.0f / (float)(R / 2);

    WG_STAMP(0);
    auto gval = [&](const double *un, int u, int k, bool wk) {
        double g = un[W::G0 + k];
        if (wk) {
            g += un[W::GU + k];
            if (u == 0 && k < 2 * N) g += k < N ? -SOC[SO::KS + 1 + k] : SOC[SO::KS + 1 + (k - N)];
        }
        return g;
    };
    auto te_tasks = [&](Place &pl, bool wk) {
        WG_FOR_AT(t, d * NW, pl.at(d * NW)) {
            const int u = 1 + t / NW, i = t - (u - 1) * NW;
            double *un = UN(u);
            double s = 0;
            if constexpr (BOX) {
                double wg = 0;
#pragma unroll
                for (int k = 0; k < NW; ++k) wg += un[W::BW + k] * gval(un, u, k, wk);
                s = -(un[W::BRS] * un[W::BW + i]) * wg;
                if (i < 2 * N) s -= un[W::BD + i] * gval(un, u, i, wk);
            } else {
#pragma unroll
                for (int k = 0; k < NW; ++k) s -= un[W::B + i * NW + k] * gval(un, u, k, wk);
            }
            un[W::TE + i] = s;
        }
    };
    auto bg_tasks = [&](Place &pl) {
        WG_FOR_AT(t, 2 * NW, pl.at(2 * NW)) {
            const int s = t / NW, i = t - s * NW;
            double acc = 0;
#pragma unroll 4
            for (int u = side_lo(s); u <= side_hi(s); ++u) acc += UN(u)[W::TE + i];
            sm[W::BG + t] = acc;
        }
        WG_FOR_AT(t, 2 * NX, pl.at(2 * NX)) {
            const int part = t / NX, c = t - part * NX, h = c / N;
            const int ulo = part ? 1 + d / 2 : 1, uhi = part ? d : d / 2;
            double acc = 0;
#pragma unroll 2
            for (int u = ulo; u <= uhi; ++u) {
                const double *un = UN(u);
                if constexpr (BOX) acc += un[W::XD + c] * un[W::TE + c] + un[W::XY + c] * un[W::TE + 2 * N];
                else {
#pragma unroll
                    for (int k = 0; k < N; ++k) acc += un[W::X + (h * N + k) * NX + c] * un[W::TE + h * N + k];
                    acc += un[W::X + 2 * N * NX + c] * un[W::TE + 2 * N];
                }
            }
            sm[W::XBG + t] = acc;
        }
    };
    auto v_tasks = [&](Place &pl) {
        WG_FOR_AT(t, 2 * NW, pl.at(2 * NW)) {
            const int s = t / NW, i = t - s * NW;
            const double *Bsi = sm + W::BSI + s * NW * NW;
            double acc = 0;
#pragma unroll
            for (int k = 0; k < NW; ++k) acc += Bsi[i * NW + k] * (sm[W::RP + s * NW + k] - sm[W::BG + s * NW + k]);
            sm[W::VV + t] = acc;
        }
    };
    auto rhs_tasks = [&](Place &pl, bool wk) {
        const double *u0 = UN(0);
        auto base_z = [&](int i) { return -gval(u0, 0, i, wk) - sm[W::VV + i] - sm[W::VV + NW + i]; };
        WG_FOR_AT(q, NX, pl.at(NX)) {
            double r = -REG_DELTA * sm[W::XV + q] - sm[W::XBG + q] - sm[W::XBG + NX + q];
            if (prox) r -= sm[W::PQ + q] * (sm[W::XV + q] + CEN[q < N ? q : q - N] - sm[W::PC + q]);
            if (wk) r -= sm[W::SOL + q];
            for (int s = 0; s < 2; ++s) {
                const double *BXs = sm + W::BXS + s * NW * NX;
#pragma unroll
                for (int i = 0; i < NW; ++i) r -= BXs[i * NX + q] * sm[W::VV + s * NW + i];
            }
            sm[W::RHS + q] = r;
        }
        WG_FOR_AT(k, N, pl.at(N))
            sm[W::RHS + NX + k] = base_z(k) + SOC[SO::CV + k] * SC[SC_GT] * rcp(SC[SC_C0]);
        WG_FOR_AT(k, N, pl.at(N))
            sm[W::RHS + NX + N + k] = base_z(k) + base_z(N + k);
        WG_FOR_AT(k, 1, pl.at(1)) sm[W::RHS + NX + 2 * N + k] = base_z(2 * N);
    };
    auto solve_head = [&](bool wk) {
        {
            Place pl;
            te_tasks(pl, wk);
            if (wk) {
                WG_FOR_AT(q, NX, pl.at(NX)) {
                    double acc = 0;
#pragma unroll 4
                    for (int u = 0; u <= d; ++u) acc += UN(u)[W::GX + q];
                    sm[W::SOL + q] = acc;
                }
            }
        }
        WG_ARRIVE(30);
        WG_SYNC();
        WG_STAMP(30); WG_REGION();
        { Place pl; bg_tasks(pl); }
        WG_ARRIVE(31);
        WG_SYNC();
        WG_STAMP(31); WG_REGION();
        { Place pl; v_tasks(pl); }
        WG_ARRIVE(32);
        WG_SYNC();
        WG_STAMP(32); WG_REGION();
        { Place pl; rhs_tasks(pl, wk); }
        WG_ARRIVE(33);
        WG_SYNC();
        WG_STAMP(33); WG_REGION();
    };
    auto cone_dir = [&](int dt_slot, bool wk, double (&xs)[Q], double (&dl)[Q]) {
        const double *u0 = UN(0);
        double wb[Q], ys[Q];
        xs[0] = SC[dt_slot];
#pragma unroll
        for (int k = 0; k < N; ++k) xs[1 + k] = u0[W::DW + k] - u0[W::DW + N + k];
#pragma unroll
        for (int k = 0; k < Q; ++k) wb[k] = SOC[SO::WB + k];
        soc_apply_W2<Q>(wb, SC[SC_ETA], xs, ys);
// ... 885 lines not shown
```

### gcs_admm_amd/csrc/vertex_wg.hip

```cpp
#include "vertex_wg_kernel.h"

using namespace gcsadmm_k;

#ifndef GCS_WG_SYM
#define GCS_WG_SYM(name) name
#endif

hipError_t GCS_WG_SYM(gcsadmm_wg_set_lds_dims)(int n, int dtype, int lds_bytes);
void GCS_WG_SYM(gcsadmm_wg_launch_dims)(const WgLaunchDesc &d, hipStream_t s);
void GCS_WG_SYM(gcsadmm_wg_launch_prox_dims)(const WgLaunchDesc &d, const double *q, const double *c, int src, int dst, hipStream_t s);


int GCS_WG_SYM(gcsadmm_wg_lds_bytes)(int n, int units, int facets, bool box) { return 8 * gcs_wg::wg_lds_doubles_n(n, units, facets, box); }
bool GCS_WG_SYM(gcsadmm_wg_has_box)(int n) { return gcs_wg::wg_has_box(n); }

hipError_t GCS_WG_SYM(gcsadmm_wg_set_lds)(int n, int dtype, int lds_bytes)
{
    hipError_t e = hipSuccess;
    if (dispatch_dim<2, 3, 6>(n, [&](auto nn) { e = set_lds<InLdsKernels, decltype(nn)::value>(dtype, lds_bytes); })) return e;
    return GCS_WG_SYM(gcsadmm_wg_set_lds_dims)(n, dtype, lds_bytes);
}

void GCS_WG_SYM(gcsadmm_wg_launch)(const WgLaunchDesc &d, hipStream_t s)
{
    if (!dispatch_dim<2, 3, 6>(d.n, [&](auto nn) { launch<decltype(nn)::value>(d, s); })) GCS_WG_SYM(gcsadmm_wg_launch_dims)(d, s);
}

void GCS_WG_SYM(gcsadmm_wg_launch_prox)(const WgLaunchDesc &d, const double *q, const double *c, int src, int dst, hipStream_t s)
{
    if (!dispatch_dim<2, 3, 6>(d.n, [&](auto nn) { launch_prox<decltype(nn)::value>(d, q, c, src, dst, s); }))
        GCS_WG_SYM(gcsadmm_wg_launch_prox_dims)(d, q, c, src, dst, s);
}

#if GCS_WG_THREADS == 256
hipError_t gcsadmm_wg_set_split_lds_dims(int n, int dtype, int lds_bytes);
void gcsadmm_wg_launch_split_dims(const WgLaunchDesc &d, const WgSplitArgs &w, hipStream_t s);

hipError_t gcsadmm_wg_set_split_lds(int n, int dtype, int lds_bytes)
{
    hipError_t e = hipSuccess;
    if (dispatch_dim<2, 3, 6>(n, [&](auto nn) { e = set_lds<SplitKernels, decltype(nn)::value>(dtype, lds_bytes); })) return e;
    return gcsadmm_wg_set_split_lds_dims(n, dtype, lds_bytes);
}

void gcsadmm_wg_launch_split(const WgLaunchDesc &d, const WgSplitArgs &w, hipStream_t s)
{
    if (!dispatch_dim<2, 3, 6>(d.n, [&](auto nn) { launch_split<decltype(nn)::value>(d, w, s); })) gcsadmm_wg_launch_split_dims(d, w, s);
}

hipError_t gcsadmm_wg_set_batch_lds_dims(int n, int dtype, int lds_bytes);
void gcsadmm_wg_launch_batch_dims(const WgBatchLaunch &b, hipStream_t s);

size_t gcsadmm_wg_batch_entry_bytes(int dtype) { return dtype == GCSADMM_F64 ? sizeof(WgBatchEntry<double>) : sizeof(WgBatchEntry<float>); }

int gcsadmm_wg_batch_fill(const WgLaunchDesc &d, void *entry_host)
{
    const int grid_x = d.n_vtx + (d.n_special + WG_THREADS - 1) / WG_THREADS;
    with_state(d.dtype, [&](auto t) {
        using T = decltype(t);
        *(WgBatchEntry<T> *)entry_host = WgBatchEntry<T>{in_lds_args<T>(d), SpecialArgs{d.n_special, d.special_vtx, d.special_kind}, d.step.cb, grid_x};
    });
    return grid_x;
}

hipError_t gcsadmm_wg_set_batch_lds(int n, int dtype, int lds_bytes)
{
    hipError_t e = hipSuccess;
    if (dispatch_dim<2, 3, 6>(n, [&](auto nn) { e = set_lds<BatchKernels, decltype(nn)::value>(dtype, lds_bytes); })) return e;
    return gcsadmm_wg_set_batch_lds_dims(n, dtype, lds_bytes);
}

void gcsadmm_wg_launch_batch(const WgBatchLaunch &b, hipStream_t s)
{
    if (!dispatch_dim<2, 3, 6>(b.n, [&](auto nn) { launch_batch<decltype(nn)::value>(b, s); })) gcsadmm_wg_launch_batch_dims(b, s);
}
#endif

#ifdef GCS_WG_TIMING
extern "C" int gcsadmm_debug_wg_cycles(unsigned long long *cycles64, unsigned long long *counts64)
{
    int e = (int)hipMemcpyFromSymbol(cycles64, HIP_SYMBOL(gcs_wg::g_wg_cycles), 64 * sizeof(unsigned long long));
    if (e == 0) e = (int)hipMemcpyFromSymbol(counts64, HIP_SYMBOL(gcs_wg::g_wg_counts), 64 * sizeof(unsigned long long));
    return e;
}
extern "C" int gcsadmm_debug_wg_wave_cycles(unsigned long long *cycles512)
{
    return (int)hipMemcpyFromSymbol(cycles512, HIP_SYMBOL(gcs_wg::g_wg_wave_cycles), 512 * sizeof(unsigned long long));
}
#endif
#ifdef GCS_WG_BLOCKTIME
extern "C" int gcsadmm_debug_wg_blocks(unsigned long long *ticks64, unsigned long long *iters64)
{
    int e = (int)hipMemcpyFromSymbol(ticks64, HIP_SYMBOL(g_wg_block_ticks), 64 * sizeof(unsigned long long));
    if (e == 0) e = (int)hipMemcpyFromSymbol(iters64, HIP_SYMBOL(g_wg_block_iters), 64 * sizeof(unsigned long long));
    return e;
}
#endif
```

### gcs_admm_amd/csrc/vertex_wg_dims.hip

```cpp
#include "vertex_wg_kernel.h"

using namespace gcsadmm_k;

#ifndef GCS_WG_SYM
#define GCS_WG_SYM(name) name
#endif

hipError_t GCS_WG_SYM(gcsadmm_wg_set_lds_dims)(int n, int dtype, int lds_bytes)
{
    hipError_t e = hipErrorInvalidValue;
    dispatch_dim<1, 4, 5, 7, 8>(n, [&](auto nn) { e = set_lds<InLdsKernels, decltype(nn)::value>(dtype, lds_bytes); });
    return e;
}

void GCS_WG_SYM(gcsadmm_wg_launch_dims)(const WgLaunchDesc &d, hipStream_t s)
{
    dispatch_dim<1, 4, 5, 7, 8>(d.n, [&](auto nn) { launch<decltype(nn)::value>(d, s); });
}

void GCS_WG_SYM(gcsadmm_wg_launch_prox_dims)(const WgLaunchDesc &d, const double *q, const double *c, int src, int dst, hipStream_t s)
{
    dispatch_dim<1, 4, 5, 7, 8>(d.n, [&](auto nn) { launch_prox<decltype(nn)::value>(d, q, c, src, dst, s); });
}

#if GCS_WG_THREADS == 256
hipError_t gcsadmm_wg_set_split_lds_dims(int n, int dtype, int lds_bytes)
{
    hipError_t e = hipErrorInvalidValue;
    dispatch_dim<1, 4, 5, 7, 8>(n, [&](auto nn) { e = set_lds<SplitKernels, decltype(nn)::value>(dtype, lds_bytes); });
    return e;
}

void gcsadmm_wg_launch_split_dims(const WgLaunchDesc &d, const WgSplitArgs &w, hipStream_t s)
{
    dispatch_dim<1, 4, 5, 7, 8>(d.n, [&](auto nn) { launch_split<decltype(nn)::value>(d, w, s); });
}

hipError_t gcsadmm_wg_set_batch_lds_dims(int n, int dtype, int lds_bytes)
{
    hipError_t e = hipErrorInvalidValue;
    dispatch_dim<1, 4, 5, 7, 8>(n, [&](auto nn) { e = set_lds<BatchKernels, decltype(nn)::value>(dtype, lds_bytes); });
    return e;
}

void gcsadmm_wg_launch_batch_dims(const WgBatchLaunch &b, hipStream_t s)
{
    dispatch_dim<1, 4, 5, 7, 8>(b.n, [&](auto nn) { launch_batch<decltype(nn)::value>(b, s); });
}
#endif
```

### gcs_admm_amd/csrc/vertex_wg_kernel.h

```cpp
#pragma once
#include <hip/hip_runtime.h>

#include <algorithm>

#include "special_vertex.h"
#include "vertex_wg.h"
#include "vertex_wg_launch.h"

namespace {

using namespace gcsadmm_k;
using gcs_wg::WG_THREADS;

#ifdef GCS_WG_TIMING
#define GCS_WG_MIN_BLOCKS 1
#else
#define GCS_WG_MIN_BLOCKS (gcs_wg::WG_THREADS <= 256 ? 2 : 1)
#endif
#if defined(GCS_WG_TIMING) && !defined(GCS_WG_BLOCKTIME)
#define GCS_WG_BLOCKTIME 1
#endif
#ifdef GCS_WG_BLOCKTIME
__device__ unsigned long long g_wg_block_ticks[64], g_wg_block_iters[64];
#endif
template <int N, bool BOX> constexpr int wg_min_blocks() { return GCS_WG_MIN_BLOCKS == 1 ? 1 : (N <= 3 ? 4 : 2); }
template <int N, class T, bool BOX>
__device__ __forceinline__ void vertex_wg_body(const gcs_wg::WgArgs<T> &a, const SpecialArgs &sp, double rho, double mu_scale, int bx, double *smem)
{
    if (bx >= a.n_vtx) {
        const int i = (bx - a.n_vtx) * WG_THREADS + (int)threadIdx.x;
        if (i < sp.count) {
            double *vals = smem + (sp.kind[i] == 2 ? 2 * MAX_SPECIAL_DEG : 0);
            special_body<N, T>(a, sp, i, rho, mu_scale, vals, vals + MAX_SPECIAL_DEG);
        }
        return;
    }
    int status = 0, iters = 0;
#ifdef GCS_WG_BLOCKTIME
    const unsigned long long t_begin = __builtin_amdgcn_s_memtime();
#endif
    const int slot = a.order ? a.order[bx] : bx;
    gcs_wg::wg_solve_vertex<N, T, BOX>(a, a.vtx[slot], rho, mu_scale, smem, status, iters);
    if (threadIdx.x == 0) {
        if (status != 0) atomicAdd(&a.counters[0], 1);
        atomicAdd(&a.counters[1], iters);
        if (a.unit_iters) a.unit_iters[slot] = iters;
#ifdef GCS_WG_BLOCKTIME
        if (bx < 64) {
            g_wg_block_ticks[bx] += __builtin_amdgcn_s_memtime() - t_begin;
            g_wg_block_iters[bx] += (unsigned long long)iters;
        }
#endif
    }
}

template <class T> struct WgTail {
    int enabled;
    EdgeArgs<T> edge;
    gcsadmm_control_block *cb;
    double *sums;
    ControlParams cp;
    int *counters;
    double *trace;
    unsigned *ticket;
};

template <class T, int C>
__device__ __forceinline__ void wg_fused_tail(const WgTail<T> &t, double mu_scale, bool closed_form, double *smem)
{
    const EdgePre pre = edge_prefetch(t.edge, mu_scale);
    asm volatile("s_waitcnt vmcnt(0)" ::: "memory");
    __syncthreads();
    double(*red)[5] = (double(*)[5])smem;
    int *is_last = (int *)(smem + EDGE_BLOCK / EDGE_WAVE * 5);
    if (threadIdx.x == 0) {
        if (closed_form) {
            __builtin_amdgcn_fence(__ATOMIC_RELEASE, "agent");
            asm volatile("s_waitcnt vmcnt(0)" ::: "memory");
        }
        const unsigned k = __hip_atomic_fetch_add(t.ticket, 1u, __ATOMIC_RELAXED, __HIP_MEMORY_SCOPE_AGENT);
        *is_last = (k == gridDim.x - 1);
    }
    __syncthreads();
    if (!*is_last) return;
    edge_body<T, 1, C, 1, EdgeInTail>(t.edge, t.cb, t.sums, t.cp, t.counters, t.trace, t.ticket, 0, 1, red, is_last, pre);
    if (threadIdx.x == 0) __hip_atomic_store(t.ticket, 0u, __ATOMIC_RELAXED, __HIP_MEMORY_SCOPE_AGENT);
}

template <class T> constexpr size_t wg_tail_kernarg_offset()
{
    static_assert(alignof(gcs_wg::WgArgs<T>) == 8 && alignof(SpecialArgs) == 8 && alignof(WgTail<T>) == 8, "kernarg layout: every argument starts on 8 bytes");
    return sizeof(gcs_wg::WgArgs<T>) + sizeof(SpecialArgs) + sizeof(const gcsadmm_control_block *);
}

template <int N, class T, bool BOX>
__global__ __launch_bounds__(WG_THREADS, (wg_min_blocks<N, BOX>())) void vertex_wg_kernel(gcs_wg::WgArgs<T> a, SpecialArgs sp, const gcsadmm_control_block *cb,
                                                                                 WgTail<T> )
{
    extern __shared__ __attribute__((aligned(16))) double smem[];
    if (cb->status != GCSADMM_RUNNING) return;
    vertex_wg_body<N, T, BOX>(a, sp, cb->rho, cb->mu_scale, (int)blockIdx.x, smem);
    typedef const __attribute__((address_space(4))) char *KernargPtr;
    KernargPtr kp = (KernargPtr)__builtin_amdgcn_kernarg_segment_ptr();
    asm volatile("" : "+s"(kp));
    typedef const __attribute__((address_space(4))) WgTail<T> *TailPtr;
    TailPtr tp = (TailPtr)(kp + wg_tail_kernarg_offset<T>());
    if (!tp->enabled) return;
    const WgTail<T> tail = *(const WgTail<T> *)tp;
    const double mu_scale = __hip_atomic_load(&tail.cb->mu_scale, __ATOMIC_RELAXED, __HIP_MEMORY_SCOPE_WORKGROUP);
    wg_fused_tail<T, 2 * N + 1>(tail, mu_scale, (int)blockIdx.x >= a.n_vtx, smem);
}

#if GCS_WG_THREADS == 256
template <class T> struct WgBatchEntry {
    gcs_wg::WgArgs<T> a;
    SpecialArgs sp;
    const gcsadmm_control_block *cb;
    int grid_x;
};
template <int N, class T, bool BOX>
__global__ __launch_bounds__(WG_THREADS, (wg_min_blocks<N, BOX>())) void vertex_wg_batch_kernel(const WgBatchEntry<T> *__restrict__ table)
{
    extern __shared__ __attribute__((aligned(16))) double smem[];
    __builtin_assume_dereferenceable(table + blockIdx.y, sizeof(WgBatchEntry<T>));
    const WgBatchEntry<T> e = *(const WgBatchEntry<T> *)((const __attribute__((address_space(4))) WgBatchEntry<T> *)table + blockIdx.y);
    if ((int)blockIdx.x >= e.grid_x || e.cb->status != GCSADMM_RUNNING) return;
    vertex_wg_body<N, T, BOX>(e.a, e.sp, e.cb->rho, e.cb->mu_scale, (int)blockIdx.x, smem);
}
#endif

template <int N, bool BOX> constexpr int wg_split_min_blocks() { return N >= 7 ? 1 : wg_min_blocks<N, BOX>(); }
template <int N, class T, bool BOX>
__global__ __launch_bounds__(WG_THREADS, (wg_split_min_blocks<N, BOX>())) void vertex_wg_split_kernel(gcs_wg::WgArgs<T> a, WgSplitArgs w,
                                                                                              const gcsadmm_control_block *cb)
{
    extern __shared__ __attribute__((aligned(16))) double smem[];
    if (cb->status != GCSADMM_RUNNING) return;
    int status = 0, iters = 0;
    gcs_wg::wg_solve_vertex<N, T, BOX, true>(a, a.vtx[blockIdx.x], cb->rho, cb->mu_scale, smem, status, iters, w.units + w.unit_off[blockIdx.x]);
    if (threadIdx.x == 0) {
        if (status != 0) atomicAdd(&a.counters[0], 1);
        atomicAdd(&a.counters[1], iters);
    }
}

struct InLdsKernels { template <int N, class T, bool BOX> static constexpr auto kernel() { return vertex_wg_kernel<N, T, BOX>; } };
struct SplitKernels { template <int N, class T, bool BOX> static constexpr auto kernel() { return vertex_wg_split_kernel<N, T, BOX>; } };
#if GCS_WG_THREADS == 256
struct BatchKernels { template <int N, class T, bool BOX> static constexpr auto kernel() { return vertex_wg_batch_kernel<N, T, BOX>; } };
#endif
template <int N> constexpr bool WG_HAS_BOX = N == 3 || N == 6;
template <class F> auto with_state(int dtype, F &&f) { return with_state_type(dtype == GCSADMM_F64, f); }

template <class K, int N, class T, class X, class... More>
void launch_kernels(const WgLaunchDesc &d, const gcs_wg::WgArgs<T> &a, unsigned grid, int lds, const X &extra, hipStream_t s, const More &...more)
{
    if constexpr (WG_HAS_BOX<N>) {
        if (d.box) { hipLaunchKernelGGL((K::template kernel<N, T, true>()), dim3(grid), dim3(WG_THREADS), lds, s, a, extra, d.step.cb, more...); return; }
    }
    hipLaunchKernelGGL((K::template kernel<N, T, false>()), dim3(grid), dim3(WG_THREADS), lds, s, a, extra, d.step.cb, more...);
}

template <class K, int N> hipError_t set_lds(int dtype, int lds_bytes)
{
    return with_state(dtype, [&](auto t) {
        using T = decltype(t);
        hipError_t e = hipFuncSetAttribute((const void *)K::template kernel<N, T, false>(), hipFuncAttributeMaxDynamicSharedMemorySize, lds_bytes);
        if constexpr (WG_HAS_BOX<N>)
            if (e == hipSuccess) e = hipFuncSetAttribute((const void *)K::template kernel<N, T, true>(), hipFuncAttributeMaxDynamicSharedMemorySize, lds_bytes);
        return e;
    });
}

template <class T> gcs_wg::WgArgs<T> in_lds_args(const WgLaunchDesc &d)
{
    gcs_wg::WgArgs<T> a;
    static_cast<StepArgs<T> &>(a) = d.step.typed<T>();
    a.n_vtx = d.n_vtx; a.vtx = d.vtx; a.order = d.order; a.unit_iters = d.unit_iters;
    return a;
}

template <class T> WgTail<T> in_lds_tail(const WgTailDesc &d)
{
    return WgTail<T>{d.enabled, retype<T>(d.edge), d.cb, d.sums, d.cp, d.counters, d.trace, d.ticket};
}

template <int N> void launch(const WgLaunchDesc &d, hipStream_t s)
{
    with_state(d.dtype, [&](auto t) {
        using T = decltype(t);
        gcs_wg::WgArgs<T> a = in_lds_args<T>(d);
        a.publish = d.tail.enabled;
        const SpecialArgs sp{d.n_special, d.special_vtx, d.special_kind};
        const unsigned grid = (unsigned)(d.n_vtx + (d.n_special + WG_THREADS - 1) / WG_THREADS);
        if (grid == 0) return;
        launch_kernels<InLdsKernels, N, T>(d, a, grid, wg_launch_lds_bytes(d.lds_bytes, d.tail.enabled != 0), sp, s, in_lds_tail<T>(d.tail));
    });
}

#if GCS_WG_THREADS == 256
template <int N> void launch_batch(const WgBatchLaunch &b, hipStream_t s)
{
    with_state(b.dtype, [&](auto t) {
        using T = decltype(t);
        const auto *table = (const WgBatchEntry<T> *)b.table;
        if constexpr (WG_HAS_BOX<N>) {
            if (b.box) { hipLaunchKernelGGL((vertex_wg_batch_kernel<N, T, true>), dim3(b.grid_x, b.count), dim3(WG_THREADS), b.lds_bytes, s, table); return; }
        }
        hipLaunchKernelGGL((vertex_wg_batch_kernel<N, T, false>), dim3(b.grid_x, b.count), dim3(WG_THREADS), b.lds_bytes, s, table);
    });
}
#endif

template <int N> void launch_split(const WgLaunchDesc &d, const WgSplitArgs &w, hipStream_t s)
{
    if (d.n_vtx <= 0) return;
    with_state(d.dtype, [&](auto t) {
        using T = decltype(t);
        gcs_wg::WgArgs<T> a;
        static_cast<StepArgs<T> &>(a) = d.step.typed<T>();
        a.n_vtx = d.n_vtx; a.vtx = d.vtx;
        launch_kernels<SplitKernels, N, T>(d, a, (unsigned)d.n_vtx, d.lds_bytes, w, s);
    });
}

template <int N>
__global__ __launch_bounds__(WG_THREADS, 2) void vertex_prox_kernel(gcs_wg::WgArgs<double> a, int src, int dst)
{
    extern __shared__ __attribute__((aligned(16))) double smem[];
    constexpr int NX = 2 * N, NU = 4 * N + 1;
    if ((int)blockIdx.x >= a.n_vtx) {
        const int t = (int)threadIdx.x;
        const int v = t == 0 ? src : (t == 1 ? dst : -1);
        if (v < 0) return;
        const double *q = a.prox_q + (size_t)v * NU, *c = a.prox_c + (size_t)v * NU;
        double num = q[2 * NX] * c[2 * NX], den = q[2 * NX];
        for (int k = 0; k < NX; ++k) {
            const double pt = a.center[(size_t)v * N + (k < N ? k : k - N)];
            num += q[NX + k] * pt * c[NX + k];
            den += q[NX + k] * pt * pt;
        }
        double y = den > 0.0 ? num / den : 0.5;
        y = y < 0.0 ? 0.0 : (y > 1.0 ? 1.0 : y);
        for (int k = 0; k < NX; ++k) {
            const double pt = a.center[(size_t)v * N + (k < N ? k : k - N)];
            a.xv[(size_t)v * NX + k] = pt;
            a.zv[(size_t)v * NX + k] = y * pt;
        }
        a.yv[v] = y;
        return;
    }
    int status = 0, iters = 0;
    gcs_wg::wg_solve_vertex<N, double>(a, a.vtx[blockIdx.x], 1.0, 1.0, smem, status, iters);
    if (threadIdx.x == 0 && a.counters) {
        if (status != 0) atomicAdd(&a.counters[0], 1);
        atomicAdd(&a.counters[1], iters);
    }
}

template <int N> void launch_prox(const WgLaunchDesc &d, const double *q, const double *c, int src, int dst, hipStream_t s)
{
    gcs_wg::WgArgs<double> a{};
    static_cast<StepArgs<double> &>(a) = d.step.typed<double>();
    a.n_vtx = d.n_vtx; a.vtx = d.vtx; a.prox_q = q; a.prox_c = c;
    if (d.lds_bytes > 48 * 1024)
        (void)hipFuncSetAttribute((const void *)vertex_prox_kernel<N>, hipFuncAttributeMaxDynamicSharedMemorySize, d.lds_bytes);
    hipLaunchKernelGGL((vertex_prox_kernel<N>), dim3(d.n_vtx + 1), dim3(WG_THREADS), d.lds_bytes, s, a, src, dst);
}

}
```

### gcs_admm_amd/csrc/vertex_wg_launch.h

```cpp
#pragma once
#include <hip/hip_runtime.h>

#include "edge_step.h"
#include "gcsadmm.h"
#include "step_args.h"

namespace gcsadmm_k {

struct WgTailDesc {
    int enabled = 0;
    EdgeArgs<void> edge{};
    gcsadmm_control_block *cb = nullptr;
    double *sums = nullptr;
    ControlParams cp{};
    int *counters = nullptr;
    double *trace = nullptr;
    unsigned *ticket = nullptr;
};

struct WgLaunchDesc {
    StepDesc step;
    int n, dtype;
    int n_vtx, n_special, lds_bytes;
    const int *vtx;
    const int *special_vtx, *special_kind;
    int box;
    const int *order;
    int *unit_iters;
    WgTailDesc tail;
};

struct WgSplitArgs {
    double *units;
    const long long *unit_off;
};

struct WgBatchLaunch {
    int n, dtype, box;
    const void *table;
    unsigned grid_x, count;
    int lds_bytes;
};

}

hipError_t gcsadmm_wg_set_lds(int n, int dtype, int lds_bytes);
void gcsadmm_wg_launch(const gcsadmm_k::WgLaunchDesc &d, hipStream_t s);

hipError_t gcsadmm_wg_set_lds_t512(int n, int dtype, int lds_bytes);
void gcsadmm_wg_launch_t512(const gcsadmm_k::WgLaunchDesc &d, hipStream_t s);

hipError_t gcsadmm_wg_set_split_lds(int n, int dtype, int lds_bytes);
void gcsadmm_wg_launch_split(const gcsadmm_k::WgLaunchDesc &d, const gcsadmm_k::WgSplitArgs &w, hipStream_t s);

size_t gcsadmm_wg_batch_entry_bytes(int dtype);
int gcsadmm_wg_batch_fill(const gcsadmm_k::WgLaunchDesc &d, void *entry_host);
hipError_t gcsadmm_wg_set_batch_lds(int n, int dtype, int lds_bytes);
void gcsadmm_wg_launch_batch(const gcsadmm_k::WgBatchLaunch &b, hipStream_t s);

void gcsadmm_wg_launch_prox(const gcsadmm_k::WgLaunchDesc &d, const double *q, const double *c, int src, int dst, hipStream_t s);
```

### gcs_admm_amd/solver.py

```python
from __future__ import annotations

import contextlib
import ctypes as C
import time
from typing import Optional

import numpy as np

from . import abi
from .abi import (CONVERGED, DIVERGED, EXPORTS, F32, F64, MAX_IT, RUNNING, STATUS_NAME,
                  ControlBlock, GcsAdmmError, GraphDesc, HaloDesc, Params, State)
from .graph import GcsGraph


load_library = abi.load_library


def halo_arrays(send_idx, recv_idx):
    peers = sorted(send_idx)
    if sorted(recv_idx) != peers:
        raise ValueError("a partition sends to and receives from the same neighbours")
    cnt = [len(send_idx[r]) for r in peers]
    if cnt != [len(recv_idx[r]) for r in peers]:
        raise ValueError("send and receive lists of a neighbour must be equally long")
    ptr = np.zeros(len(peers) + 1, np.int32); ptr[1:] = np.cumsum(cnt)
    cat = lambda d: (np.concatenate([np.asarray(d[r], np.int32) for r in peers]) if peers else np.zeros(0, np.int32))
    return np.asarray(peers, np.int32), ptr, np.ascontiguousarray(cat(send_idx)), np.ascontiguousarray(cat(recv_idx))


class DeviceSolver:

    def __init__(self, graph: GcsGraph, state_dtype: str = "f64", device: Optional[int] = None,
                 num_incidences: Optional[int] = None, inc_counted=None, edge_counted=None,
                 nx_global: float = 0.0, nmu_global: float = 0.0, program: str = "auto", wave_slots: int = 0,
                 wave_align: int = 0, wave_store_dl: int = 0, wave_generic_rows: int = 0, columns: str = "incidence",
                 vertex_workspace: int = 0):
        import torch
        if not torch.cuda.is_available():
            raise RuntimeError("no HIP device visible: the ADMM loop only runs on the GPU (no CPU fallback)")
        self.torch = torch
        self.lib = load_library()
        self.g = g = graph
        self.device_index = torch.cuda.current_device() if device is None else int(device)
        self.device = torch.device("cuda", self.device_index)
        self.dtype_code = {"f64": F64, "f32": F32}[state_dtype]
        self.tdtype = torch.float64 if state_dtype == "f64" else torch.float32
        desc, self._keep, self.col_of = abi.graph_desc(
            g, state_dtype=self.dtype_code, device=self.device_index, num_incidences=num_incidences, inc_counted=inc_counted,
            edge_counted=edge_counted, nx_global=nx_global, nmu_global=nmu_global, columns=columns,
            vertex_program={"auto": 0, "wavefront": 1, "workgroup": 2, "workgroup256": 3}[program], wave_slots=wave_slots,
            wave_align=wave_align, wave_store_dl=wave_store_dl, wave_generic_rows=wave_generic_rows, vertex_workspace=vertex_workspace)
        self.NI, self.edge_major = desc.num_incidences, columns == "edge"
        h = C.c_void_p()
        self._call("gcsadmm_create", C.byref(desc), C.byref(h), handle=False, select=False)
        self.h = h
        c, E, V, n = g.c, g.num_edges, g.num_vertices, g.n
        z = lambda *s, dt=self.tdtype: torch.zeros(*s, dtype=dt, device=self.device)
        self.copy, self.mu, self.zedge = z(c, max(self.NI, 1)), z(c, max(self.NI, 1)), z(c, max(E, 1))
        self.xv, self.zv, self.yv = z(V, 2 * n, dt=torch.float64), z(V, 2 * n, dt=torch.float64), z(V, dt=torch.float64)
        self.sums = z(5, dt=torch.float64)
        self._cost = z(1, dt=torch.float64)
        self.state = State(self.copy.data_ptr(), self.mu.data_ptr(), self.zedge.data_ptr(),
                           self.xv.data_ptr(), self.zv.data_ptr(), self.yv.data_ptr())
        self.params = None
        self.trace = None

    def _call(self, name, *args, handle=True, select=True):
        h = self.h if handle else None
        with self.torch.cuda.device(self.device) if select else contextlib.nullcontext():
            st = getattr(self.lib, name)(*((h,) if handle else ()), *args)
        abi.check(st, lambda: f"{name} failed ({st}): {self.lib.gcsadmm_last_error(h).decode()}")

    def _stream(self):
        return self.torch.cuda.current_stream(self.device).cuda_stream

    def close(self):
        if getattr(self, "h", None):
            self._call("gcsadmm_destroy", select=False)
            self.h = None

    def __del__(self):
        try:
            self.close()
        except Exception:
            pass

    def reset(self, rho=1.0, tau_incr=2.0, tau_decr=2.0, nu=10.0, it_rho_limit=100, max_it=1000, eps_abs=1e-4,
              eps_rel=1e-3, eps_edge=1e-4, ipm_tol=None, ipm_max_iter=60, zero_state=True, cold_start=False):
        if ipm_tol is None:
            from . import IPM_TOL as ipm_tol
        self.params = Params(rho, tau_incr, tau_decr, nu, it_rho_limit, max_it, eps_abs, eps_rel, eps_edge,
                             ipm_tol, ipm_max_iter, 1 if cold_start else 0)
        if zero_state:
            for t in (self.copy, self.mu, self.zedge, self.xv, self.zv, self.yv):
                t.zero_()
        self.trace = self.torch.zeros(max_it, 6, dtype=self.torch.float64, device=self.device)
        self._call("gcsadmm_reset", C.byref(self.params), self._stream())

    def vertex_step(self):
        self._call("gcsadmm_vertex_step", C.byref(self.state), self._stream())

    def edge_step(self):
        self._call("gcsadmm_edge_step", C.byref(self.state), self.sums.data_ptr(), self._stream())
        return self.sums

    def control(self, sums=None):
        s = self.sums if sums is None else sums
        self._call("gcsadmm_control", s.data_ptr(), self.trace.data_ptr(), self._stream())

    def enqueue(self, k: int):
        self._call("gcsadmm_run", C.byref(self.state), int(k), self.trace.data_ptr(), self._stream())

    def set_fused_tail(self, mode: int = 1) -> bool:
        return bool(self.lib.gcsadmm_set_fused_tail(self.h, int(mode)))

    def enqueue_timed(self, k: int):
        vm, em = C.c_float(0), C.c_float(0)
        vl, el = C.c_int32(0), C.c_int32(0)
        self._call("gcsadmm_run_timed", C.byref(self.state), int(k), self.trace.data_ptr(), self._stream(),
                   C.byref(vm), C.byref(vl), C.byref(em), C.byref(el))
        return dict(vertex_ms=vm.value, vertex_launches=vl.value, edge_ms=em.value, edge_launches=el.value)

    def vertex_prox(self, q, c, ipm_tol: float = 1e-10, ipm_max_iter: int = 60):
        torch = self.torch
        V, n = self.g.num_vertices, self.g.n
        qd = torch.as_tensor(np.ascontiguousarray(q, dtype=np.float64), device=self.device)
        cd = torch.as_tensor(np.ascontiguousarray(c, dtype=np.float64), device=self.device)
        assert qd.shape == (V, 4 * n + 1) and cd.shape == qd.shape
        xv = torch.zeros(V, 2 * n, dtype=torch.float64, device=self.device); zv = torch.zeros_like(xv)
        yv = torch.zeros(V, dtype=torch.float64, device=self.device)
        fails = C.c_int32(0)
        self._call("gcsadmm_vertex_prox", qd.data_ptr(), cd.data_ptr(), xv.data_ptr(), zv.data_ptr(), yv.data_ptr(),
                   float(ipm_tol), int(ipm_max_iter), C.byref(fails), self._stream(), select=False)
        return xv, zv, yv, fails.value

    def unique_id(self) -> bytes:
        buf = (C.c_ubyte * 128)()
        self._call("gcsadmm_comm_unique_id", buf, handle=False, select=False)
        return bytes(buf)

    def _halo_desc(self, send_idx, recv_idx):
        peers, ptr, sc, rc = halo_arrays(send_idx, recv_idx)
        if self.edge_major:
            sc = np.ascontiguousarray(self.col_of[sc].astype(np.int32)); rc = np.ascontiguousarray(self.col_of[rc].astype(np.int32))
        self._halo_keep = (peers, ptr, sc, rc)
        return HaloDesc(len(peers), peers.ctypes.data, ptr.ctypes.data, sc.ctypes.data, ptr.ctypes.data, rc.ctypes.data)

    def check_halo(self, rank: int, world: int, send_idx, recv_idx):
        self._call("gcsadmm_check_halo", int(rank), int(world), C.byref(self._halo_desc(send_idx, recv_idx)), select=False)

    def attach_comm(self, rank: int, world: int, unique_id, send_idx, recv_idx):
        idb = (C.c_ubyte * 128).from_buffer_copy(unique_id) if unique_id is not None else None
        self._call("gcsadmm_attach_comm", int(rank), int(world), idb, C.byref(self._halo_desc(send_idx, recv_idx)))
        self.has_comm = unique_id is not None

    def enqueue_partitioned(self, k: int):
        self._call("gcsadmm_run_partitioned", C.byref(self.state), int(k), self.trace.data_ptr(), self._stream())

    def enqueue_partitioned_timed(self, k: int):
        v, hl, e, r = (C.c_float(0) for _ in range(4))
        self._call("gcsadmm_run_partitioned_timed", C.byref(self.state), int(k), self.trace.data_ptr(), self._stream(),
                   C.byref(v), C.byref(hl), C.byref(e), C.byref(r))
        return dict(vertex_ms=v.value, halo_ms=hl.value, edge_ms=e.value, reduce_ms=r.value)

    def set_overlap(self, mode: int = 0) -> int:
        n = C.c_int32(0)
        self._call("gcsadmm_set_overlap", int(mode), C.byref(n))
        return n.value

    def comm_count(self) -> int:
        n = C.c_int32(0)
        self._call("gcsadmm_comm_count", C.byref(n), select=False)
        return n.value

    def halo_pack(self):
        self._call("gcsadmm_halo_pack", C.byref(self.state), self._stream(), select=False)

    def halo_unpack(self):
        self._call("gcsadmm_halo_unpack", C.byref(self.state), self._stream(), select=False)

    def halo_exchange(self):
        self._call("gcsadmm_halo_exchange", C.byref(self.state), self._stream(), select=False)

    def halo_buffers(self):
        a, b, n = C.c_void_p(), C.c_void_p(), C.c_int64(0)
        self._call("gcsadmm_halo_buffers", C.byref(a), C.byref(b), C.byref(n), select=False)
        return a.value, b.value, n.value

    def read_control(self) -> ControlBlock:
        cb = ControlBlock()
        self._call("gcsadmm_read_control", C.byref(cb), self._stream(), select=False)
        return cb

    def query(self):
        a, b, c, d, e = (C.c_int32(0) for _ in range(5))
        self._call("gcsadmm_query", C.byref(a), C.byref(b), C.byref(c), C.byref(d), C.byref(e), select=False)
        return dict(num_waves=a.value, lds_bytes=b.value, num_special=c.value, num_workgroup_vertices=d.value,
                    workgroup_lds_bytes=e.value)

    def query_workspace(self):
        a, b, c = C.c_int32(0), C.c_int32(0), C.c_int64(0)
        self._call("gcsadmm_query_workspace", C.byref(a), C.byref(b), C.byref(c), select=False)
        return dict(num_split_vertices=a.value, split_lds_bytes=b.value, workspace_bytes=c.value)

    def unit_iterations(self):
        n = C.c_int32(0)
        self._call("gcsadmm_unit_iterations", None, 0, C.byref(n), self._stream())
        out = np.zeros(n.value, np.int32)
        if n.value:
            self._call("gcsadmm_unit_iterations", out.ctypes.data, n.value, C.byref(n), self._stream())
        return out

    def export_state(self, vertex_ids):
        from .transfer import StateSnapshot, check_vertex_ids
        ids = check_vertex_ids(vertex_ids, self.g.num_vertices)
        snap = StateSnapshot(self.g.n, "f64" if self.dtype_code == F64 else "f32", self.g.num_vertices, self.g.num_edges, self.device)
        self._call("gcsadmm_export_state", C.byref(self.state), ids.ctypes.data, C.byref(snap.c), self._stream())
        return snap

    def import_state(self, snapshot, vertex_ids):
        from .transfer import check_vertex_ids
        ids = check_vertex_ids(vertex_ids, self.g.num_vertices)
        self._call("gcsadmm_import_state", C.byref(self.state), ids.ctypes.data, C.byref(snapshot.c), self._stream())

    def cost(self) -> float:
        eps = self.params.eps_edge if self.params is not None else 1e-4
        self._call("gcsadmm_cost", C.byref(self.state), eps, self._cost.data_ptr(), self._stream(), select=False)
        return float(self._cost.item())

    def _loop(self, enqueue, chunk, params, clock=False):
        self.reset(**params)
        max_it, done, dev_ms = self.params.max_it, 0, 0.0
        if clock:
            self.torch.cuda.synchronize(self.device)
        t0 = time.perf_counter()
        while True:
            k = min(chunk, max_it - done)
            if k > 0:
                dev_ms += enqueue(k) or 0.0
                done += k
            cb = self.read_control()
            if cb.status != RUNNING or done >= max_it:
                return cb, time.perf_counter() - t0, dev_ms

    def solve_partitioned(self, chunk: int = 25, **params):
        return self._loop(self.enqueue_partitioned, chunk, params)[0]

    def solve(self, chunk: int = 25, timed: bool = False, **params):
        def enqueue_timed(k):
            tm = self.enqueue_timed(k)
            return tm["vertex_ms"] + tm["edge_ms"]
        cb, wall, dev_ms = self._loop(enqueue_timed if timed else self.enqueue, chunk, params, clock=True)
        return self.record(cb, wall, dev_ms * 1e-3 if timed else None)

    def record(self, cb, wall_time_s, device_time_s=None):
        tr = self.trace[:min(cb.it, self.params.max_it)].cpu().numpy()
        return dict(iterations=int(cb.it), status=STATUS_NAME[cb.status],
                    rho_seq=np.concatenate([[self.params.rho], tr[:, 0]]),
                    pri_res_seq=np.concatenate([[0.0], tr[:, 1]]),
                    dual_res_seq=np.concatenate([[0.0], tr[:, 2]]),
                    eps_pri_seq=tr[:, 3], eps_dual_seq=tr[:, 4],
                    inner_failures=int(tr[:, 5].sum()), cost=self.cost(),
                    wall_time_s=wall_time_s, device_time_s=device_time_s)
```

### include/gcsadmm.h

```cpp
#ifndef GCSADMM_H
#define GCSADMM_H

#include <stdint.h>

#ifdef __cplusplus
extern "C" {
#endif

typedef enum gcsadmm_status {
    GCSADMM_OK = 0,
    GCSADMM_ERR_BAD_ARG = 1,
    GCSADMM_ERR_UNSUPPORTED = 2,
    GCSADMM_ERR_HIP = 3,
    GCSADMM_ERR_NO_DEVICE = 4,
    GCSADMM_ERR_NO_MEMORY = 5
} gcsadmm_status;

enum { GCSADMM_F64 = 0, GCSADMM_F32 = 1 };

enum { GCSADMM_RUNNING = -1, GCSADMM_CONVERGED = 0, GCSADMM_MAX_IT = 1, GCSADMM_DIVERGED = 2 };

typedef struct gcsadmm_graph_desc {
    int32_t n;
    int32_t num_vertices;
    int32_t num_edges;
    int32_t num_incidences;
    const int32_t *inc_ptr;
    const int32_t *inc_edge;
    const int32_t *inc_out;
    const int32_t *edge_inc_tail;
    const int32_t *edge_inc_head;
    const int32_t *poly_ptr;
    const double *poly_A;
    const double *poly_b;
    const double *center;
    int32_t src, dst;
    int32_t state_dtype;
    int32_t device;
    const uint8_t *inc_counted;
    const uint8_t *edge_counted;
    double nx_global, nmu_global;
    int32_t vertex_program;
    int32_t wave_slots;
    int32_t wave_align;
    int32_t wave_store_dl;
    int32_t wave_generic_rows;
    int32_t edge_major_columns;
    int32_t vertex_workspace;
} gcsadmm_graph_desc;

typedef struct gcsadmm_params {
    double rho;
    double tau_incr;
    double tau_decr;
    double nu;
    int32_t it_rho_limit;
    int32_t max_it;
    double eps_abs;
    double eps_rel;
    double eps_edge;
    double ipm_tol;
    int32_t ipm_max_iter;
    int32_t cold_start;
} gcsadmm_params;

typedef struct gcsadmm_state {
    void *copy;
    void *mu;
    void *zedge;
    double *xv;
    double *zv;
    double *yv;
} gcsadmm_state;

typedef struct gcsadmm_control_block {
    double rho;
    double mu_scale;
    double sums[5];
    double pri, dual, eps_pri, eps_dual;
    int32_t it;
    int32_t status;
    int32_t inner_failures;
    int32_t inner_iters;
} gcsadmm_control_block;

typedef struct gcsadmm_handle_s *gcsadmm_handle;

gcsadmm_status gcsadmm_create(const gcsadmm_graph_desc *desc, gcsadmm_handle *out);
void gcsadmm_destroy(gcsadmm_handle h);
const char *gcsadmm_last_error(gcsadmm_handle h);

gcsadmm_status gcsadmm_reset(gcsadmm_handle h, const gcsadmm_params *p, void *stream);

gcsadmm_status gcsadmm_vertex_step(gcsadmm_handle h, const gcsadmm_state *st, void *stream);

gcsadmm_status gcsadmm_edge_step(gcsadmm_handle h, const gcsadmm_state *st, double *sums_dev, void *stream);

gcsadmm_status gcsadmm_control(gcsadmm_handle h, const double *sums_dev, double *trace_dev, void *stream);

gcsadmm_status gcsadmm_run(gcsadmm_handle h, const gcsadmm_state *st, int32_t k, double *trace_dev, void *stream);

int32_t gcsadmm_set_fused_tail(gcsadmm_handle h, int32_t mode);

gcsadmm_status gcsadmm_read_control(gcsadmm_handle h, gcsadmm_control_block *out, void *stream);

gcsadmm_status gcsadmm_cost(gcsadmm_handle h, const gcsadmm_state *st, double eps_edge, double *cost_dev, void *stream);

gcsadmm_status gcsadmm_query(gcsadmm_handle h, int32_t *num_waves, int32_t *lds_bytes, int32_t *num_special,
                             int32_t *num_workgroup_vertices, int32_t *workgroup_lds_bytes);

gcsadmm_status gcsadmm_query_workspace(gcsadmm_handle h, int32_t *num_split_vertices, int32_t *split_lds_bytes, int64_t *workspace_bytes);

gcsadmm_status gcsadmm_unit_iterations(gcsadmm_handle h, int32_t *out, int32_t capacity, int32_t *count, void *stream);

gcsadmm_status gcsadmm_run_timed(gcsadmm_handle h, const gcsadmm_state *st, int32_t k, double *trace_dev,
                                 void *stream, float *vertex_ms, int32_t *vertex_launches,
                                 float *edge_ms, int32_t *edge_launches);

typedef struct gcsadmm_batch_s gcsadmm_batch_s;
enum { GCSADMM_BATCH_LARGE = 1, GCSADMM_BATCH_TERMINALS = 4 };

gcsadmm_status gcsadmm_batch_create(const gcsadmm_handle *members, int32_t count, struct gcsadmm_batch_s **out);
gcsadmm_status gcsadmm_batch_create_ex(const gcsadmm_handle *members, int32_t count, int32_t flags, struct gcsadmm_batch_s **out);
gcsadmm_status gcsadmm_batch_query(struct gcsadmm_batch_s *b, int32_t *wg_members, int32_t *wave_groups, int32_t *wave_members);
gcsadmm_status gcsadmm_batch_query_terminals(struct gcsadmm_batch_s *b, int32_t *term_groups, int32_t *terminals);
void gcsadmm_batch_destroy(struct gcsadmm_batch_s *b);
const char *gcsadmm_batch_last_error(struct gcsadmm_batch_s *b);

gcsadmm_status gcsadmm_batch_bind(struct gcsadmm_batch_s *b, const gcsadmm_state *states, double *const *traces_dev, void *stream);

gcsadmm_status gcsadmm_batch_run(struct gcsadmm_batch_s *b, int32_t k, void *stream);

gcsadmm_status gcsadmm_batch_poll(struct gcsadmm_batch_s *b, int32_t *status, int32_t *it, void *stream);

typedef struct gcsadmm_snapshot {
    int32_t n, state_dtype;
    int32_t V, E;
    int64_t *edge_key;
    void *edge_words;
    int32_t *vertex_id;
    double *vertex_words;
    double *rho;
} gcsadmm_snapshot;

gcsadmm_status gcsadmm_export_state(gcsadmm_handle h, const gcsadmm_state *state, const int32_t *vertex_id, gcsadmm_snapshot *snapshot, void *stream);
gcsadmm_status gcsadmm_import_state(gcsadmm_handle h, const gcsadmm_state *state, const int32_t *vertex_id, const gcsadmm_snapshot *snapshot, void *stream);
gcsadmm_status gcsadmm_batch_export_state(struct gcsadmm_batch_s *b, const int32_t *const *vertex_ids, gcsadmm_snapshot *const *snapshots, void *stream);
gcsadmm_status gcsadmm_batch_import_state(struct gcsadmm_batch_s *b, const int32_t *const *vertex_ids, const gcsadmm_snapshot *const *snapshots, void *stream);

gcsadmm_status gcsadmm_vertex_prox(gcsadmm_handle h, const double *q_dev, const double *c_dev, double *xv_dev, double *zv_dev,
                                   double *yv_dev, double ipm_tol, int32_t ipm_max_iter, int32_t *failures_host, void *stream);

typedef struct gcsadmm_halo_desc {
    int32_t num_peers;
    const int32_t *peer_rank;
    const int32_t *send_ptr;
    const int32_t *send_cols;
    const int32_t *recv_ptr;
    const int32_t *recv_cols;
} gcsadmm_halo_desc;

gcsadmm_status gcsadmm_comm_unique_id(void *id128);

gcsadmm_status gcsadmm_attach_comm(gcsadmm_handle h, int32_t rank, int32_t world, const void *id128, const gcsadmm_halo_desc *halo);
gcsadmm_status gcsadmm_check_halo(gcsadmm_handle h, int32_t rank, int32_t world, const gcsadmm_halo_desc *halo);

gcsadmm_status gcsadmm_run_partitioned(gcsadmm_handle h, const gcsadmm_state *st, int32_t k, double *trace_dev, void *stream);

gcsadmm_status gcsadmm_run_partitioned_timed(gcsadmm_handle h, const gcsadmm_state *st, int32_t k, double *trace_dev, void *stream,
                                             float *vertex_ms, float *halo_ms, float *edge_ms, float *reduce_ms);

gcsadmm_status gcsadmm_set_overlap(gcsadmm_handle h, int32_t mode, int32_t *boundary_units);

gcsadmm_status gcsadmm_comm_count(gcsadmm_handle h, int32_t *count);

gcsadmm_status gcsadmm_halo_pack(gcsadmm_handle h, const gcsadmm_state *st, void *stream);
gcsadmm_status gcsadmm_halo_unpack(gcsadmm_handle h, const gcsadmm_state *st, void *stream);
gcsadmm_status gcsadmm_halo_exchange(gcsadmm_handle h, const gcsadmm_state *st, void *stream);
gcsadmm_status gcsadmm_halo_buffers(gcsadmm_handle h, void **send_buf, void **recv_buf, int64_t *num_elements);

const char *gcsadmm_polytope_last_error(void);

int gcsadmm_polytope_centers(int n, int num_polytopes, const int *poly_ptr, const double *poly_A, const double *poly_b,
                             int device, double *centers, double *radii, int *status);

int gcsadmm_polytope_bounds(int n, int num_polytopes, const int *poly_ptr, const double *poly_A, const double *poly_b,
                            const double *centers, int device, double *lo, double *hi, int *status);

int gcsadmm_polytope_overlaps(int n, int num_polytopes, const int *poly_ptr, const double *poly_A, const double *poly_b,
                              const double *centers, long num_pairs, const int *pair_a, const int *pair_b, double tol,
                              int device, unsigned char *overlap, int *status);

typedef struct gcsadmm_scene_s *gcsadmm_scene;

int gcsadmm_scene_create(int n, int num_polytopes, const int *poly_ptr, const double *poly_A, const double *poly_b, int device,
                         gcsadmm_scene *out);
void gcsadmm_scene_destroy(gcsadmm_scene s);

int gcsadmm_scene_centers(gcsadmm_scene s, double *centers, double *radii, int *status);

int gcsadmm_scene_bounds(gcsadmm_scene s, double *lo, double *hi, int *status);

int gcsadmm_scene_set_boxes(gcsadmm_scene s, const double *lo, const double *hi);

int gcsadmm_scene_candidate_pairs(gcsadmm_scene s, double pad, int64_t *num_pairs);

int gcsadmm_scene_overlaps(gcsadmm_scene s, double tol, int64_t *num_overlapping, int64_t *num_undecided);

int gcsadmm_scene_read_pairs(gcsadmm_scene s, int *pair_a, int *pair_b, unsigned char *overlap, int *status);

int gcsadmm_scene_restrict_paths(gcsadmm_scene s, int num_paths, const int *path_ptr, const int *path_poly, const double *start, double tol,
                                 int max_iter, double *points, double *cost, int *iterations, int *status);

int gcsadmm_scene_locate_points(gcsadmm_scene s, int num_points, const double *points, double eps, double tol, int64_t *num_hits);

int gcsadmm_scene_locate_boxes(gcsadmm_scene s, int num_boxes, const double *lo, const double *hi, double tol, int64_t *num_hits);

int gcsadmm_scene_read_hits(gcsadmm_scene s, int64_t *hit_ptr, int *hit_region, unsigned char *hit_class);

int gcsadmm_scene_project_points(gcsadmm_scene s, int num_points, const double *points, const double *radius, int max_iter, int64_t *num_hits);
int gcsadmm_scene_read_projections(gcsadmm_scene s, double *distance, double *nearest, int *status, int *iterations);

int gcsadmm_scene_add_regions(gcsadmm_scene s, int num_new, const int *poly_ptr, const double *poly_A, const double *poly_b,
                              double pad, double tol, double *centers, double *radii, int *center_status,
                              int64_t *num_new_pairs, int64_t *num_overlapping, int64_t *num_undecided);
int gcsadmm_scene_remove_regions(gcsadmm_scene s, int num_removed, const int *regions, int64_t *num_pairs_left);
int gcsadmm_scene_read_regions(gcsadmm_scene s, double *centers, double *radii, int *center_status, double *lo, double *hi, int *box_status);

int gcsadmm_scene_build_region_graph(gcsadmm_scene s, const unsigned char *overlap, int64_t *num_edges);
int gcsadmm_scene_read_region_graph(gcsadmm_scene s, int64_t *row_ptr, int *edge_tail, int *edge_head, int *reverse);
int gcsadmm_scene_query_graphs(gcsadmm_scene s, int num_queries, const int64_t *term_ptr, const int *term_region,
                               const unsigned char *st_adjacent, int chunk_queries, const int64_t *edge_off, int *edge_tail, int *edge_head,
                               int *inc_ptr, int *inc_edge, int *inc_out, int *edge_inc_tail, int *edge_inc_head);

int gcsadmm_scene_region_paths(gcsadmm_scene s, int num_queries, const double *points, const int64_t *term_ptr, const int *term_region,
                               int max_len, int *path_region, int *path_len, double *path_cost, int *status);
int gcsadmm_scene_informed_regions(gcsadmm_scene s, int num_queries, const double *points, const double *bound, double pad,
                                   unsigned char *keep, int64_t *num_kept);

int gcsadmm_scene_region_paths_sets(gcsadmm_scene s, int num_queries, const double *lo, const double *hi, const int64_t *term_ptr,
                                    const int *term_region, int max_len, int *path_region, int *path_len, double *path_cost, int *status);
int gcsadmm_scene_informed_regions_sets(gcsadmm_scene s, int num_queries, const double *lo, const double *hi, const double *bound, double pad,
                                        unsigned char *keep, int64_t *num_kept);

int gcsadmm_scene_induced_sizes(gcsadmm_scene s, int num_queries, const unsigned char *keep, const int64_t *term_ptr, const int *term_region,
                                const unsigned char *st_adjacent, int *num_kept, int64_t *num_edges);
int gcsadmm_scene_induced_query_graphs(gcsadmm_scene s, int num_queries, const unsigned char *keep, const int64_t *term_ptr, const int *term_region,
                                       const unsigned char *st_adjacent, int chunk_queries, const int64_t *vertex_off, const int64_t *edge_off,
                                       int *edge_tail, int *edge_head, int *inc_ptr, int *inc_edge, int *inc_out, int *edge_inc_tail,
                                       int *edge_inc_head);

typedef struct gcsadmm_walks_s gcsadmm_walks_s;
int gcsadmm_walks_create(int num_problems, const int64_t *vertex_off, const int64_t *edge_off, const int *out_ptr, const int *out_head,
                         const int *out_edge, const int *src, const int *dst, int device, struct gcsadmm_walks_s **out);
// ... 10 lines not shown
```

Baseline: 10470 iterations/s.

## Run up to 32 ADMM iterations per launch with resident workgroups and grid barrier

```diff
diff --git a/gcs_admm_amd/abi.py b/gcs_admm_amd/abi.py
--- a/gcs_admm_amd/abi.py
+++ b/gcs_admm_amd/abi.py
@@ -56,6 +56,12 @@
 
 
 _p, _i, _d = C.c_void_p, C.c_int32, C.c_double
+
+
+def resident_window_mode(window: int = 0) -> int:
+    return 2 | (max(0, int(window)) << 8)
+
+
 _run, _run_timed = [_p, _p, _i, _p, _p], [_p, _p, _i, _p, _p] + [_p] * 4
 _csr = [_i, _i, _p, _p, _p]
 PROTOTYPES = {
diff --git a/gcs_admm_amd/csrc/create_plan.h b/gcs_admm_amd/csrc/create_plan.h
--- a/gcs_admm_amd/csrc/create_plan.h
+++ b/gcs_admm_amd/csrc/create_plan.h
@@ -6,6 +6,7 @@
 
 #include "canonical_box.h"
 #include "gcsadmm.h"
+#include "resident_wait.h"
 #include "state_transfer_core.h"
 #include "step_args.h"
 #include "vertex_program.h"
@@ -54,6 +55,7 @@
     double nx = 0, nmu = 0;
     int edge_unroll = 1, edge_blocks = 1;
     int fused_tail = 0;
+    int resident_window = 0;
     std::vector<int> edge_tail, edge_head;
     int edges_ascending = 0;
     int n_waves() const { return (int)wave_slot_ptr.size() - 1; }
@@ -271,4 +273,24 @@
     return GCSADMM_OK;
 }
 
-}
+constexpr bool RESIDENT_WINDOW_AUTO = true;
+
+inline int wg_launch_grid(int n_wg, int n_special, int wg_threads) { return n_wg + (n_special + wg_threads - 1) / wg_threads; }
+
+inline int set_resident_window(CreatePlan &p, int n_special, int wg_threads, int compute_units, int blocks_per_cu)
+{
+    const int n_wg = (int)p.wg_vtx.size();
+    const long long resident = (long long)std::max(compute_units, 0) * std::max(blocks_per_cu, 0);
+    const bool in_lds_only = n_wg > 0 && p.wg_t512 && p.split_vtx.empty() && p.n_waves() == 0 && p.n_term == 0;
+    const bool lds_room = wg_launch_lds_bytes(p.wg_lds_bytes, true) + RESIDENT_LDS_BYTES <= LDS_CU_BYTES;
+    const bool on = p.fused_tail && in_lds_only && lds_room && wg_threads > 0 && (long long)wg_launch_grid(n_wg, n_special, wg_threads) <= resident;
+    return p.resident_window = on ? gcs_resident::WINDOW_MAX : 0;
+}
+inline int resident_launch_window(int plan_window, int forced, int k_left)
+{
+    int j = plan_window;
+    if (forced > 0 && forced < j) j = forced;
+    return std::max(0, std::min(j, k_left));
+}
+
+}
diff --git a/gcs_admm_amd/csrc/edge_step.h b/gcs_admm_amd/csrc/edge_step.h
--- a/gcs_admm_amd/csrc/edge_step.h
+++ b/gcs_admm_amd/csrc/edge_step.h
@@ -46,6 +46,8 @@
     template <class T> static __device__ __forceinline__ T load_copy(const T *p) { return *p; }
     static __device__ __forceinline__ int load_counter(const int *p) { return *p; }
     static __device__ __forceinline__ void store_counter(int *p, int v) { *p = v; }
+    template <class T> static __device__ __forceinline__ T load(const T *p) { return *p; }
+    template <class T, class V> static __device__ __forceinline__ void store(T *p, V v) { *p = (T)v; }
     static __device__ __forceinline__ bool edge_thread() { return true; }
     static __device__ __forceinline__ void sync() { __syncthreads(); }
 };
@@ -54,8 +56,14 @@
     template <class T> static __device__ __forceinline__ T load_copy(const T *p) { return __hip_atomic_load(p, __ATOMIC_RELAXED, __HIP_MEMORY_SCOPE_AGENT); }
     static __device__ __forceinline__ int load_counter(const int *p) { return __hip_atomic_load(p, __ATOMIC_RELAXED, __HIP_MEMORY_SCOPE_AGENT); }
     static __device__ __forceinline__ void store_counter(int *p, int v) { __hip_atomic_store(p, v, __ATOMIC_RELAXED, __HIP_MEMORY_SCOPE_AGENT); }
+    template <class T> static __device__ __forceinline__ T load(const T *p) { return *p; }
+    template <class T, class V> static __device__ __forceinline__ void store(T *p, V v) { *p = (T)v; }
     static __device__ __forceinline__ bool edge_thread() { return threadIdx.x < (unsigned)EDGE_BLOCK; }
     static __device__ __forceinline__ void sync() { __syncthreads(); }
+};
+struct EdgeInWindow : EdgeInTail {
+    template <class T> static __device__ __forceinline__ T load(const T *p) { return __hip_atomic_load(p, __ATOMIC_RELAXED, __HIP_MEMORY_SCOPE_AGENT); }
+    template <class T, class V> static __device__ __forceinline__ void store(T *p, V v) { __hip_atomic_store(p, (T)v, __ATOMIC_RELAXED, __HIP_MEMORY_SCOPE_AGENT); }
 };
 
 struct EdgePre {
@@ -77,17 +85,17 @@
 __device__ void control_body(gcsadmm_control_block *cb, const double *sums, const ControlParams &p, int *counters, double *trace,
                              bool global_fails = false)
 {
-    if (cb->status != GCSADMM_RUNNING) return;
+    if (P::load(&cb->status) != GCSADMM_RUNNING) return;
     double s[5];
-    for (int k = 0; k < 5; ++k) { s[k] = sums[k]; cb->sums[k] = s[k]; }
-    const int it = cb->it;
-    double rho = cb->rho;
+    for (int k = 0; k < 5; ++k) { s[k] = sums[k]; P::store(&cb->sums[k], s[k]); }
+    const int it = P::load(&cb->it);
+    double rho = P::load(&cb->rho);
     const int fails = global_fails ? (int)(sums[5] + 0.5) : P::load_counter(&counters[0]), iters = P::load_counter(&counters[1]);
     P::store_counter(&counters[0], 0); P::store_counter(&counters[1], 0);
-    cb->inner_failures = fails; cb->inner_iters = iters;
+    P::store(&cb->inner_failures, fails); P::store(&cb->inner_iters, iters);
     const double tot = s[0] + s[1] + s[2] + s[3] + s[4];
     if (!(fabs(tot) <= 1.7976931348623157e308)) {
-        cb->status = GCSADMM_DIVERGED;
+        P::store(&cb->status, GCSADMM_DIVERGED);
         return;
     }
     const double pri = sqrt(s[0]), dual = rho * sqrt(2.0 * s[1]);
@@ -96,20 +104,20 @@
     else if (dual >= p.nu * pri && it < p.it_rho_limit) { rho *= 1.0 / p.tau_decr; mu_scale = p.tau_incr; }
     const double eps_pri = sqrt(p.nx) * p.eps_abs + p.eps_rel * fmax(sqrt(s[2]), sqrt(2.0 * s[3]));
     const double eps_dual = sqrt(p.nmu) * p.eps_abs + p.eps_rel * mu_scale * sqrt(s[4]);
-    cb->rho = rho; cb->mu_scale = mu_scale;
-    cb->pri = pri; cb->dual = dual; cb->eps_pri = eps_pri; cb->eps_dual = eps_dual;
+    P::store(&cb->rho, rho); P::store(&cb->mu_scale, mu_scale);
+    P::store(&cb->pri, pri); P::store(&cb->dual, dual); P::store(&cb->eps_pri, eps_pri); P::store(&cb->eps_dual, eps_dual);
     if (trace) {
         double *tr = trace + (size_t)(it - 1) * 6;
-        tr[0] = rho; tr[1] = pri; tr[2] = dual; tr[3] = eps_pri; tr[4] = eps_dual; tr[5] = (double)fails;
-    }
-    if (pri < eps_pri && dual < eps_dual) { cb->status = GCSADMM_CONVERGED; return; }
-    cb->it = it + 1;
-    if (it + 1 > p.max_it) cb->status = GCSADMM_MAX_IT;
+        P::store(&tr[0], rho); P::store(&tr[1], pri); P::store(&tr[2], dual); P::store(&tr[3], eps_pri); P::store(&tr[4], eps_dual); P::store(&tr[5], (double)fails);
+    }
+    if (pri < eps_pri && dual < eps_dual) { P::store(&cb->status, GCSADMM_CONVERGED); return; }
+    P::store(&cb->it, it + 1);
+    if (it + 1 > p.max_it) P::store(&cb->status, GCSADMM_MAX_IT);
 }
 
 template <class T, int C> __host__ __device__ constexpr int edge_unroll() { return sizeof(T) == 4 ? (C <= 7 ? 4 : 2) : (C <= 7 ? 2 : 1); }
 
-template <class T>
+template <class T, class P = EdgeInKernel>
 __device__ __forceinline__ void edge_word(const EdgeArgs<T> &a, int w, int e, int it, int ih, T cu_t, T cw_t, T zo_t, T mu_t, T mw_t, double mu_scale,
                                           double we, double wt, double wh, double (&s)[5])
 {
@@ -119,9 +127,9 @@
     const double ru = cu - zn, rw = cw - zn;
     const T mu_u_t = (T)scaled_plus(mu_scale, (double)mu_t, ru);
     const T mu_w_t = (T)scaled_plus(mu_scale, (double)mw_t, rw);
-    a.mu[(size_t)w * a.NI + it] = mu_u_t;
-    a.mu[(size_t)w * a.NI + ih] = mu_w_t;
-    a.zedge[(size_t)w * a.E + e] = zn_t;
+    P::store(&a.mu[(size_t)w * a.NI + it], mu_u_t);
+    P::store(&a.mu[(size_t)w * a.NI + ih], mu_w_t);
+    P::store(&a.zedge[(size_t)w * a.E + e], zn_t);
     const double mu_u = (double)mu_u_t, mu_w = (double)mu_w_t;
     s[0] += wt * ru * ru + wh * rw * rw;
     s[1] += we * (zn - zo) * (zn - zo);
@@ -164,14 +172,14 @@
                     const int w = w0 + j;
                     if (w >= C) break;
                     cu_[j] = P::load_copy(&a.copy[(size_t)w * a.NI + it]); cw_[j] = P::load_copy(&a.copy[(size_t)w * a.NI + ih]);
-                    zo_[j] = a.zedge[(size_t)w * a.E + e];
-                    mu_[j] = a.mu[(size_t)w * a.NI + it]; mw_[j] = a.mu[(size_t)w * a.NI + ih];
+                    zo_[j] = P::load(&a.zedge[(size_t)w * a.E + e]);
+                    mu_[j] = P::load(&a.mu[(size_t)w * a.NI + it]); mw_[j] = P::load(&a.mu[(size_t)w * a.NI + ih]);
                 }
 #pragma unroll
                 for (int j = 0; j < CH; ++j) {
                     const int w = w0 + j;
                     if (w >= C) break;
-                    edge_word(a, w, e, it, ih, cu_[j], cw_[j], zo_[j], mu_[j], mw_[j], mu_scale, we, wt, wh, s);
+                    edge_word<T, P>(a, w, e, it, ih, cu_[j], cw_[j], zo_[j], mu_[j], mw_[j], mu_scale, we, wt, wh, s);
                 }
             }
         }
@@ -213,8 +221,8 @@
         double t = 0;
         for (int q = 0; q < EDGE_BLOCK / EDGE_WAVE; ++q) t += red[q][threadIdx.x];
         if (MODE >= 2) __hip_atomic_store(&a.partials[(size_t)bx * 5 + threadIdx.x], t, __ATOMIC_RELAXED, __HIP_MEMORY_SCOPE_AGENT);
-        else a.partials[(size_t)bx * 5 + threadIdx.x] = t;
-        if (MODE == 1) sums[threadIdx.x] = t;
+        else P::store(&a.partials[(size_t)bx * 5 + threadIdx.x], t);
+        if (MODE == 1) P::store(&sums[threadIdx.x], t);
         if constexpr (P::TAIL) red[0][threadIdx.x] = t;
     }
     if (MODE == 1) {
diff --git a/gcs_admm_amd/csrc/gcsadmm.hip b/gcs_admm_amd/csrc/gcsadmm.hip
--- a/gcs_admm_amd/csrc/gcsadmm.hip
+++ b/gcs_admm_amd/csrc/gcsadmm.hip
@@ -69,7 +69,10 @@
     gcsadmm_batch_s *batch = nullptr;
     std::vector<gcsadmm_batch_s *> batches;
     int overlap_mode = 0;
-    int fused_tail_mode = 1;
+    int fused_tail_mode = -1;
+    int window_forced = 0;
+    unsigned window_gen = 0;
+    bool window_failed = false;
     std::string err;
     void *comm = nullptr;
     int rank = 0, world = 1;
@@ -92,6 +95,7 @@
         DevBuf<int> d_counters;
         DevBuf<double> d_partials, d_sums;
         DevBuf<unsigned> d_ticket;
+        DevBuf<unsigned> d_window;
         DevBuf<char> d_transfer;
     } loop;
     struct Prox { DevBuf<int> d_prox_vtx, d_prox_counters; } prox;
@@ -104,6 +108,11 @@
     int n_wg() const { return (int)g.d_wg_vtx.size(); }
     int n_split() const { return (int)g.d_split_vtx.size(); }
     bool fuses() const { return plan.fused_tail && fused_tail_mode != 0 && !halo.attached(); }
+    int resident() const
+    {
+        const bool asked = fused_tail_mode == 2 || (fused_tail_mode < 0 && RESIDENT_WINDOW_AUTO);
+        return fuses() && asked ? resident_launch_window(plan.resident_window, window_forced, plan.resident_window) : 0;
+    }
 };
 
 struct gcsadmm_batch_s {
@@ -127,6 +136,8 @@
 };
 
 
+static const char *const WINDOW_FAILED_TEXT = "resident window: a workgroup waited past its budget for the others of its launch (the device was "
+                                              "busy with other work); the run is incomplete, reset the handle";
 static thread_local std::string g_create_error;
 
 #define HIPCHK(obj, call)                                                                            \
@@ -777,6 +788,7 @@
         UP(loop, d_partials, nullptr, (size_t)p.edge_blocks * 5);
         UP(loop, d_sums, nullptr, 5);
         UP(loop, d_ticket, nullptr, 1);
+        UP(loop, d_window, nullptr, 2);
         if (p.n_term > 0) {
             UP(term, d_term_ws, nullptr, p.term_ws_doubles);
             UP(term, d_term_rec, nullptr, p.term_rec_doubles);
@@ -794,6 +806,18 @@
         UP(prox, d_prox_vtx, p.prox_vtx.data(), p.prox_vtx.size());
         UP(prox, d_prox_counters, nullptr, 2);
 #undef UP
+        int wg_attr_bytes = p.wg_lds_bytes;
+        if (p.fused_tail) {
+            const int lds = wg_launch_lds_bytes(p.wg_lds_bytes, true) + RESIDENT_LDS_BYTES;
+            int cus = 0;
+            if (lds <= LDS_CU_BYTES && hipDeviceGetAttribute(&cus, hipDeviceAttributeMultiprocessorCount, g->device) == hipSuccess) {
+                if (lds > 48 * 1024 && (p.wg_t512 ? gcsadmm_wg_set_lds_t512(h->n, h->dtype, lds) : gcsadmm_wg_set_lds(h->n, h->dtype, lds)) == hipSuccess) wg_attr_bytes = lds;
+                if (lds <= 48 * 1024 || wg_attr_bytes == lds) {
+                    const int nb = p.wg_t512 ? gcsadmm_wg_resident_blocks_t512(h->n, h->dtype, p.wg_box, lds) : gcsadmm_wg_resident_blocks(h->n, h->dtype, p.wg_box, lds);
+                    set_resident_window(p, (int)p.special_vtx.size(), p.wg_t512 ? 512 : 256, cus, nb);
+                }
+            }
+        }
         auto release = [](auto &v) { v.clear(); v.shrink_to_fit(); };
         release(p.bc); release(p.deg_in); release(p.warm_ptr); release(p.prox_vtx); release(p.special_vtx); release(p.special_kind);
         release(p.wg_vtx); release(p.split_vtx); release(p.split_off);
@@ -801,7 +825,7 @@
             e = with_state(h.get(), [&](auto t) { return set_lds_attr<2, decltype(t)>(p.all_m4, p.lds_bytes); });
             if (e != hipSuccess) return bail(e, "hipFuncSetAttribute(MaxDynamicSharedMemorySize)");
         }
-        if (p.wg_lds_bytes > 48 * 1024 && (e = p.wg_t512 ? gcsadmm_wg_set_lds_t512(h->n, h->dtype, p.wg_lds_bytes)
+        if (p.wg_lds_bytes > 48 * 1024 && wg_attr_bytes == p.wg_lds_bytes && (e = p.wg_t512 ? gcsadmm_wg_set_lds_t512(h->n, h->dtype, p.wg_lds_bytes)
                                                           : gcsadmm_wg_set_lds(h->n, h->dtype, p.wg_lds_bytes)) != hipSuccess)
             return bail(e, "hipFuncSetAttribute(MaxDynamicSharedMemorySize, workgroup program)");
         if (p.split_lds_bytes > 48 * 1024 && (e = gcsadmm_wg_set_split_lds(h->n, h->dtype, p.split_lds_bytes)) != hipSuccess)
@@ -824,6 +848,9 @@
         hipStream_t s = (hipStream_t)stream;
         HIPCHK(h, hipMemcpyAsync(h->loop.d_cb.get(), &cb, sizeof(cb), hipMemcpyHostToDevice, s));
         HIPCHK(h, h->loop.d_counters.zero(s));
+        HIPCHK(h, h->loop.d_ticket.zero(s));
+        HIPCHK(h, h->loop.d_window.zero(s));
+        h->window_gen = 0; h->window_failed = false;
         HIPCHK(h, h->g.d_warm.zero(s));
         HIPCHK(h, h->term.d_term_rec.zero(s));
         h->vertex_steps = 0;
@@ -861,8 +888,19 @@
     return handle_entry(h, [&] { return bad_unless(state_ok(h, st) && k >= 0); }, [&] {
         hipStream_t s = (hipStream_t)stream;
         gcsadmm_status r = GCSADMM_OK;
+        if (h->window_failed) { h->err = WINDOW_FAILED_TEXT; return GCSADMM_ERR_HIP; }
         if (h->fuses()) {
-            const WgTailDesc tail = make_wg_tail(h, st, trace_dev);
+            WgTailDesc tail = make_wg_tail(h, st, trace_dev);
+            const int window = h->resident();
+            if (window > 0) {
+                tail.gen = h->loop.d_window.get();
+                for (int i = 0; i < k && r == GCSADMM_OK; i += tail.window) {
+                    tail.window = resident_launch_window(window, 0, k - i); tail.gen_base = h->window_gen;
+                    h->window_gen += (unsigned)tail.window;
+                    r = launch_vertex(h, st, s, VertexLaunch{-1, false, &tail});
+                }
+                return r;
+            }
             for (int i = 0; i < k && r == GCSADMM_OK; ++i) r = launch_vertex(h, st, s, VertexLaunch{-1, false, &tail});
             return r;
         }
@@ -967,8 +1005,10 @@
 int32_t gcsadmm_set_fused_tail(gcsadmm_handle h, int32_t mode)
 {
     if (!h) return 0;
-    h->fused_tail_mode = mode != 0;
-    return h->fuses() ? 1 : 0;
+    const int m = mode & 0xff;
+    h->fused_tail_mode = mode < 0 ? -1 : (m == 2 ? 2 : mode != 0);
+    h->window_forced = m == 2 && mode > 0 ? mode >> 8 : 0;
+    return h->fuses() ? (h->resident() > 0 ? 2 : 1) : 0;
 }
 
 gcsadmm_status gcsadmm_set_overlap(gcsadmm_handle h, int32_t mode, int32_t *boundary_units)
@@ -1054,8 +1094,12 @@
 gcsadmm_status gcsadmm_read_control(gcsadmm_handle h, gcsadmm_control_block *out, void *stream)
 {
     return handle_entry(h, [&] { return bad_unless(out); }, [&] {
+        unsigned window[2] = {0, 0};
         HIPCHK(h, hipMemcpyAsync(out, h->loop.d_cb.get(), sizeof(*out), hipMemcpyDeviceToHost, (hipStream_t)stream));
+        HIPCHK(h, hipMemcpyAsync(window, h->loop.d_window.get(), sizeof(window), hipMemcpyDeviceToHost, (hipStream_t)stream));
         HIPCHK(h, hipStreamSynchronize((hipStream_t)stream));
+        if (window[1] != 0) h->window_failed = true;
+        if (h->window_failed) { h->err = WINDOW_FAILED_TEXT; return GCSADMM_ERR_HIP; }
         return GCSADMM_OK;
     });
 }
diff --git a/gcs_admm_amd/csrc/resident_wait.h b/gcs_admm_amd/csrc/resident_wait.h
--- /dev/null
+++ b/gcs_admm_amd/csrc/resident_wait.h
@@ -0,0 +1,29 @@
+#pragma once
+
+#if defined(__HIPCC__) || defined(__CUDACC__)
+#define GCS_RW_HD __host__ __device__ __forceinline__
+#else
+#define GCS_RW_HD inline
+#endif
+
+namespace gcs_resident {
+
+constexpr int WINDOW_MAX = 32;
+
+constexpr unsigned long long TICKS_PER_ITERATION_CEILING = 5000000ull;
+constexpr unsigned long long wait_budget_ticks(int window) { return TICKS_PER_ITERATION_CEILING * (unsigned long long)(window < 1 ? 1 : window); }
+
+GCS_RW_HD bool generation_reached(unsigned have, unsigned want) { return (int)(have - want) >= 0; }
+
+template <class Load, class Clock, class Pause>
+GCS_RW_HD bool wait_generation(Load &&load, Clock &&clock, Pause &&pause, unsigned want, unsigned long long budget)
+{
+    const unsigned long long t0 = (unsigned long long)clock();
+    for (;;) {
+        if (generation_reached(load(), want)) return true;
+        if ((unsigned long long)clock() - t0 > budget) return generation_reached(load(), want);
+        pause();
+    }
+}
+
+}
diff --git a/gcs_admm_amd/csrc/step_args.h b/gcs_admm_amd/csrc/step_args.h
--- a/gcs_admm_amd/csrc/step_args.h
+++ b/gcs_admm_amd/csrc/step_args.h
@@ -10,6 +10,7 @@
 constexpr int MAX_SPECIAL_DEG = 256;
 constexpr int EDGE_BLOCK = 256;
 constexpr int FUSED_TAIL_LDS_BYTES = (EDGE_BLOCK / 64 * 5 + 1) * 8;
+constexpr int RESIDENT_LDS_BYTES = 16;
 constexpr int wg_launch_lds_bytes(int plan_lds_bytes, bool fused_tail)
 {
     int b = 4 * MAX_SPECIAL_DEG * 8;
@@ -76,6 +77,19 @@
     return (double)a.zedge[(size_t)w * a.E + edge] - mu_scale * (double)a.mu[(size_t)w * a.NI + col];
 }
 
+template <class A> GCS_HD double consensus_target(const A &a, int w, int edge, int col, double mu_scale, int publish)
+{
+#if defined(__HIP_DEVICE_COMPILE__)
+    if (publish > 1) {
+        const auto z = __hip_atomic_load(&a.zedge[(size_t)w * a.E + edge], __ATOMIC_RELAXED, __HIP_MEMORY_SCOPE_AGENT);
+        const auto m = __hip_atomic_load(&a.mu[(size_t)w * a.NI + col], __ATOMIC_RELAXED, __HIP_MEMORY_SCOPE_AGENT);
+        return (double)z - mu_scale * (double)m;
+    }
+#endif
+    (void)publish;
+    return consensus_target(a, w, edge, col, mu_scale);
+}
+
 template <int... Ns, class F> bool dispatch_dim(int n, F &&f)
 {
     return ((n == Ns ? (f(std::integral_constant<int, Ns>()), true) : false) || ...);
diff --git a/gcs_admm_amd/csrc/vertex_wg.h b/gcs_admm_amd/csrc/vertex_wg.h
--- a/gcs_admm_amd/csrc/vertex_wg.h
+++ b/gcs_admm_amd/csrc/vertex_wg.h
@@ -426,7 +426,7 @@
 #define WG_ROWS_BEGIN_DS(pl) WG_ROWS_BEGIN_(pl, true)
 #define WG_ROWS_END() }}
 
-template <int N, class T, bool BOX = false, bool SPLIT = false>
+template <int N, class T, bool BOX = false, bool SPLIT = false, bool FRESH = false>
 GCS_HD void wg_solve_vertex(const WgArgs<T> &a, int v, double rho, double mu_scale, double *sm, int &status_out, int &iters_out,
                             double *units = nullptr)
 {
@@ -488,7 +488,7 @@
         const bool out = e >= d_in;
         const int inc = gcsadmm_k::state_column(a, lo, e, edge, out);
         double *un = UN(e + 1);
-        const double Tw = gcsadmm_k::consensus_target(a, w, edge, inc, mu_scale);
+        const double Tw = gcsadmm_k::consensus_target(a, w, edge, inc, mu_scale, FRESH ? 2 : 0);
         int slot = -1;
         if (w == 2 * N) slot = 2 * N;
         else if (out) slot = w;
diff --git a/gcs_admm_amd/csrc/vertex_wg.hip b/gcs_admm_amd/csrc/vertex_wg.hip
--- a/gcs_admm_amd/csrc/vertex_wg.hip
+++ b/gcs_admm_amd/csrc/vertex_wg.hip
@@ -7,6 +7,7 @@
 #endif
 
 hipError_t GCS_WG_SYM(gcsadmm_wg_set_lds_dims)(int n, int dtype, int lds_bytes);
+int GCS_WG_SYM(gcsadmm_wg_resident_blocks_dims)(int n, int dtype, int box, int lds_bytes);
 void GCS_WG_SYM(gcsadmm_wg_launch_dims)(const WgLaunchDesc &d, hipStream_t s);
 void GCS_WG_SYM(gcsadmm_wg_launch_prox_dims)(const WgLaunchDesc &d, const double *q, const double *c, int src, int dst, hipStream_t s);
 
@@ -19,6 +20,13 @@
     hipError_t e = hipSuccess;
     if (dispatch_dim<2, 3, 6>(n, [&](auto nn) { e = set_lds<InLdsKernels, decltype(nn)::value>(dtype, lds_bytes); })) return e;
     return GCS_WG_SYM(gcsadmm_wg_set_lds_dims)(n, dtype, lds_bytes);
+}
+
+int GCS_WG_SYM(gcsadmm_wg_resident_blocks)(int n, int dtype, int box, int lds_bytes)
+{
+    int nb = 0;
+    if (dispatch_dim<2, 3, 6>(n, [&](auto nn) { nb = resident_blocks<decltype(nn)::value>(dtype, box, lds_bytes); })) return nb;
+    return GCS_WG_SYM(gcsadmm_wg_resident_blocks_dims)(n, dtype, box, lds_bytes);
 }
 
 void GCS_WG_SYM(gcsadmm_wg_launch)(const WgLaunchDesc &d, hipStream_t s)
diff --git a/gcs_admm_amd/csrc/vertex_wg_dims.hip b/gcs_admm_amd/csrc/vertex_wg_dims.hip
--- a/gcs_admm_amd/csrc/vertex_wg_dims.hip
+++ b/gcs_admm_amd/csrc/vertex_wg_dims.hip
@@ -11,6 +11,13 @@
     hipError_t e = hipErrorInvalidValue;
     dispatch_dim<1, 4, 5, 7, 8>(n, [&](auto nn) { e = set_lds<InLdsKernels, decltype(nn)::value>(dtype, lds_bytes); });
     return e;
+}
+
+int GCS_WG_SYM(gcsadmm_wg_resident_blocks_dims)(int n, int dtype, int box, int lds_bytes)
+{
+    int nb = 0;
+    dispatch_dim<1, 4, 5, 7, 8>(n, [&](auto nn) { nb = resident_blocks<decltype(nn)::value>(dtype, box, lds_bytes); });
+    return nb;
 }
 
 void GCS_WG_SYM(gcsadmm_wg_launch_dims)(const WgLaunchDesc &d, hipStream_t s)
diff --git a/gcs_admm_amd/csrc/vertex_wg_kernel.h b/gcs_admm_amd/csrc/vertex_wg_kernel.h
--- a/gcs_admm_amd/csrc/vertex_wg_kernel.h
+++ b/gcs_admm_amd/csrc/vertex_wg_kernel.h
@@ -2,7 +2,9 @@
 #include <hip/hip_runtime.h>
 
 #include <algorithm>
-
+#include <cstddef>
+
+#include "resident_wait.h"
 #include "special_vertex.h"
 #include "vertex_wg.h"
 #include "vertex_wg_launch.h"
@@ -24,7 +26,7 @@
 __device__ unsigned long long g_wg_block_ticks[64], g_wg_block_iters[64];
 #endif
 template <int N, bool BOX> constexpr int wg_min_blocks() { return GCS_WG_MIN_BLOCKS == 1 ? 1 : (N <= 3 ? 4 : 2); }
-template <int N, class T, bool BOX>
+template <int N, class T, bool BOX, bool FRESH = false>
 __device__ __forceinline__ void vertex_wg_body(const gcs_wg::WgArgs<T> &a, const SpecialArgs &sp, double rho, double mu_scale, int bx, double *smem)
 {
     if (bx >= a.n_vtx) {
@@ -40,7 +42,7 @@
     const unsigned long long t_begin = __builtin_amdgcn_s_memtime();
 #endif
     const int slot = a.order ? a.order[bx] : bx;
-    gcs_wg::wg_solve_vertex<N, T, BOX>(a, a.vtx[slot], rho, mu_scale, smem, status, iters);
+    gcs_wg::wg_solve_vertex<N, T, BOX, false, FRESH>(a, a.vtx[slot], rho, mu_scale, smem, status, iters);
     if (threadIdx.x == 0) {
         if (status != 0) atomicAdd(&a.counters[0], 1);
         atomicAdd(&a.counters[1], iters);
@@ -63,10 +65,14 @@
     int *counters;
     double *trace;
     unsigned *ticket;
+    int window;
+    unsigned gen_base;
+    unsigned *gen;
+    int window_word;
 };
 
-template <class T, int C>
-__device__ __forceinline__ void wg_fused_tail(const WgTail<T> &t, double mu_scale, bool closed_form, double *smem)
+template <class T, int C, class P>
+__device__ __forceinline__ bool wg_fused_tail(const WgTail<T> &t, double mu_scale, bool closed_form, double *smem)
 {
     const EdgePre pre = edge_prefetch(t.edge, mu_scale);
     asm volatile("s_waitcnt vmcnt(0)" ::: "memory");
@@ -82,9 +88,48 @@
         *is_last = (k == gridDim.x - 1);
     }
     __syncthreads();
-    if (!*is_last) return;
-    edge_body<T, 1, C, 1, EdgeInTail>(t.edge, t.cb, t.sums, t.cp, t.counters, t.trace, t.ticket, 0, 1, red, is_last, pre);
+    if constexpr (std::is_same_v<P, EdgeInWindow>) {
+        if (!gcs_wg::wg_uniform(*is_last)) return false;
+    } else if (!*is_last) return false;
+    edge_body<T, 1, C, 1, P>(t.edge, t.cb, t.sums, t.cp, t.counters, t.trace, t.ticket, 0, 1, red, is_last, pre);
     if (threadIdx.x == 0) __hip_atomic_store(t.ticket, 0u, __ATOMIC_RELAXED, __HIP_MEMORY_SCOPE_AGENT);
+    return true;
+}
+
+template <class T>
+__device__ __forceinline__ bool wg_window_next(const WgTail<T> &t, bool was_last, bool closed_form, double *smem, double &rho, double &mu_scale)
+{
+    unsigned *const want_p = (unsigned *)(smem + t.window_word);
+    int *const go = (int *)(smem + t.window_word) + 1;
+    const unsigned want = (unsigned)gcs_wg::wg_uniform((int)*want_p);
+    if (was_last) {
+        asm volatile("s_waitcnt vmcnt(0)" ::: "memory");
+        __syncthreads();
+        if (threadIdx.x == 0) {
+            __hip_atomic_store(&t.gen[0], want, __ATOMIC_RELEASE, __HIP_MEMORY_SCOPE_AGENT);
+            *go = 1;
+        }
+    } else if (threadIdx.x == 0) {
+        unsigned *const gen = t.gen;
+        const bool ok = gcs_resident::wait_generation([gen] { return __hip_atomic_load(&gen[0], __ATOMIC_RELAXED, __HIP_MEMORY_SCOPE_AGENT); },
+                                                      [] { return wall_clock64(); }, [] { __builtin_amdgcn_s_sleep(2); }, want,
+                                                      gcs_resident::wait_budget_ticks(t.window));
+        if (!ok) __hip_atomic_store(&t.gen[1], 1u, __ATOMIC_RELAXED, __HIP_MEMORY_SCOPE_AGENT);
+        *go = ok;
+    }
+    __syncthreads();
+    if (!gcs_wg::wg_uniform(*go)) return false;
+    if (closed_form) {
+        __builtin_amdgcn_fence(__ATOMIC_ACQUIRE, "agent");
+        asm volatile("s_waitcnt vmcnt(0)" ::: "memory");
+    }
+    const int status = gcs_wg::wg_uniform(__hip_atomic_load(&t.cb->status, __ATOMIC_RELAXED, __HIP_MEMORY_SCOPE_AGENT));
+    if (status != GCSADMM_RUNNING || want - t.gen_base >= (unsigned)t.window) return false;
+    rho = gcs_wg::wg_uniform(__hip_atomic_load(&t.cb->rho, __ATOMIC_RELAXED, __HIP_MEMORY_SCOPE_AGENT));
+    mu_scale = gcs_wg::wg_uniform(__hip_atomic_load(&t.cb->mu_scale, __ATOMIC_RELAXED, __HIP_MEMORY_SCOPE_AGENT));
+    __syncthreads();
+    if (threadIdx.x == 0) *want_p = want + 1;
+    return true;
 }
 
 template <class T> constexpr size_t wg_tail_kernarg_offset()
@@ -108,8 +153,43 @@
     if (!tp->enabled) return;
     const WgTail<T> tail = *(const WgTail<T> *)tp;
     const double mu_scale = __hip_atomic_load(&tail.cb->mu_scale, __ATOMIC_RELAXED, __HIP_MEMORY_SCOPE_WORKGROUP);
-    wg_fused_tail<T, 2 * N + 1>(tail, mu_scale, (int)blockIdx.x >= a.n_vtx, smem);
-}
+    wg_fused_tail<T, 2 * N + 1, EdgeInTail>(tail, mu_scale, (int)blockIdx.x >= a.n_vtx, smem);
+}
+
+#if GCS_WG_THREADS == 512
+template <int N, class T, bool BOX>
+__global__ __launch_bounds__(WG_THREADS, 1) void vertex_wg_window_kernel(gcs_wg::WgArgs<T> a, SpecialArgs sp, const gcsadmm_control_block *cb,
+                                                                         WgTail<T> )
+{
+    extern __shared__ __attribute__((aligned(16))) double smem[];
+    if (cb->status != GCSADMM_RUNNING) return;
+    typedef const __attribute__((address_space(4))) char *KernargPtr;
+    typedef const __attribute__((address_space(4))) WgTail<T> *TailPtr;
+    {
+        KernargPtr kp0 = (KernargPtr)__builtin_amdgcn_kernarg_segment_ptr();
+        asm volatile("" : "+s"(kp0));
+        TailPtr tp0 = (TailPtr)(kp0 + wg_tail_kernarg_offset<T>());
+        if (tp0->gen[1] != 0u) return;
+        if (threadIdx.x == 0) *(unsigned *)(smem + tp0->window_word) = tp0->gen_base + 1u;
+    }
+    double rho = cb->rho, mu_scale_in = cb->mu_scale;
+    for (;;) {
+        KernargPtr ka = (KernargPtr)__builtin_amdgcn_kernarg_segment_ptr();
+        asm volatile("" : "+s"(ka));
+        const gcs_wg::WgArgs<T> ap = *(const gcs_wg::WgArgs<T> *)(const __attribute__((address_space(4))) gcs_wg::WgArgs<T> *)ka;
+        const SpecialArgs spp = *(const SpecialArgs *)(const __attribute__((address_space(4))) SpecialArgs *)(ka + sizeof(gcs_wg::WgArgs<T>));
+        vertex_wg_body<N, T, BOX, true>(ap, spp, rho, mu_scale_in, (int)blockIdx.x, smem);
+        KernargPtr kp = (KernargPtr)__builtin_amdgcn_kernarg_segment_ptr();
+        asm volatile("" : "+s"(kp));
+        TailPtr tp = (TailPtr)(kp + wg_tail_kernarg_offset<T>());
+        const WgTail<T> tail = *(const WgTail<T> *)tp;
+        const bool closed_form = (int)blockIdx.x >= *(const __attribute__((address_space(4))) int *)(kp + offsetof(gcs_wg::WgArgs<T>, n_vtx));
+        const double mu_scale = gcs_wg::wg_uniform(__hip_atomic_load(&tail.cb->mu_scale, __ATOMIC_RELAXED, __HIP_MEMORY_SCOPE_AGENT));
+        const bool was_last = wg_fused_tail<T, 2 * N + 1, EdgeInWindow>(tail, mu_scale, closed_form, smem);
+        if (!wg_window_next(tail, was_last, closed_form, smem, rho, mu_scale_in)) return;
+    }
+}
+#endif
 
 #if GCS_WG_THREADS == 256
 template <class T> struct WgBatchEntry {
@@ -145,6 +225,9 @@
 }
 
 struct InLdsKernels { template <int N, class T, bool BOX> static constexpr auto kernel() { return vertex_wg_kernel<N, T, BOX>; } };
+#if GCS_WG_THREADS == 512
+struct WindowKernels { template <int N, class T, bool BOX> static constexpr auto kernel() { return vertex_wg_window_kernel<N, T, BOX>; } };
+#endif
 struct SplitKernels { template <int N, class T, bool BOX> static constexpr auto kernel() { return vertex_wg_split_kernel<N, T, BOX>; } };
 #if GCS_WG_THREADS == 256
 struct BatchKernels { template <int N, class T, bool BOX> static constexpr auto kernel() { return vertex_wg_batch_kernel<N, T, BOX>; } };
@@ -163,6 +246,12 @@
 
 template <class K, int N> hipError_t set_lds(int dtype, int lds_bytes)
 {
+#if GCS_WG_THREADS == 512
+    if constexpr (std::is_same_v<K, InLdsKernels>) {
+        const hipError_t ew = set_lds<WindowKernels, N>(dtype, lds_bytes);
+        if (ew != hipSuccess) return ew;
+    }
+#endif
     return with_state(dtype, [&](auto t) {
         using T = decltype(t);
         hipError_t e = hipFuncSetAttribute((const void *)K::template kernel<N, T, false>(), hipFuncAttributeMaxDynamicSharedMemorySize, lds_bytes);
@@ -172,6 +261,25 @@
     });
 }
 
+template <int N> int resident_blocks(int dtype, int box, int lds_bytes)
+{
+    return with_state(dtype, [&](auto t) {
+        using T = decltype(t);
+        int nb = 0;
+#if GCS_WG_THREADS == 512
+        hipError_t e = hipErrorInvalidValue;
+        if constexpr (WG_HAS_BOX<N>) {
+            if (box) e = hipOccupancyMaxActiveBlocksPerMultiprocessor(&nb, (const void *)vertex_wg_window_kernel<N, T, true>, WG_THREADS, (size_t)lds_bytes);
+        }
+        if (!(WG_HAS_BOX<N> && box)) e = hipOccupancyMaxActiveBlocksPerMultiprocessor(&nb, (const void *)vertex_wg_window_kernel<N, T, false>, WG_THREADS, (size_t)lds_bytes);
+        if (e != hipSuccess) nb = 0;
+#else
+        (void)box; (void)lds_bytes;
+#endif
+        return nb;
+    });
+}
+
 template <class T> gcs_wg::WgArgs<T> in_lds_args(const WgLaunchDesc &d)
 {
     gcs_wg::WgArgs<T> a;
@@ -182,7 +290,7 @@
 
 template <class T> WgTail<T> in_lds_tail(const WgTailDesc &d)
 {
-    return WgTail<T>{d.enabled, retype<T>(d.edge), d.cb, d.sums, d.cp, d.counters, d.trace, d.ticket};
+    return WgTail<T>{d.enabled, retype<T>(d.edge), d.cb, d.sums, d.cp, d.counters, d.trace, d.ticket, 0, 0u, nullptr, 0};
 }
 
 template <int N> void launch(const WgLaunchDesc &d, hipStream_t s)
@@ -190,11 +298,18 @@
     with_state(d.dtype, [&](auto t) {
         using T = decltype(t);
         gcs_wg::WgArgs<T> a = in_lds_args<T>(d);
-        a.publish = d.tail.enabled;
+        const bool window = GCS_WG_THREADS == 512 && d.tail.enabled && d.tail.window > 0;
+        a.publish = d.tail.enabled ? (window ? 2 : 1) : 0;
         const SpecialArgs sp{d.n_special, d.special_vtx, d.special_kind};
         const unsigned grid = (unsigned)(d.n_vtx + (d.n_special + WG_THREADS - 1) / WG_THREADS);
         if (grid == 0) return;
-        launch_kernels<InLdsKernels, N, T>(d, a, grid, wg_launch_lds_bytes(d.lds_bytes, d.tail.enabled != 0), sp, s, in_lds_tail<T>(d.tail));
+        const int lds = wg_launch_lds_bytes(d.lds_bytes, d.tail.enabled != 0);
+        WgTail<T> tail = in_lds_tail<T>(d.tail);
+        if (window) { tail.window = d.tail.window; tail.gen_base = d.tail.gen_base; tail.gen = d.tail.gen; tail.window_word = lds / 8; }
+#if GCS_WG_THREADS == 512
+        if (window) { launch_kernels<WindowKernels, N, T>(d, a, grid, lds + RESIDENT_LDS_BYTES, sp, s, tail); return; }
+#endif
+        launch_kernels<InLdsKernels, N, T>(d, a, grid, lds, sp, s, tail);
     });
 }
 
diff --git a/gcs_admm_amd/csrc/vertex_wg_launch.h b/gcs_admm_amd/csrc/vertex_wg_launch.h
--- a/gcs_admm_amd/csrc/vertex_wg_launch.h
+++ b/gcs_admm_amd/csrc/vertex_wg_launch.h
@@ -16,6 +16,9 @@
     int *counters = nullptr;
     double *trace = nullptr;
     unsigned *ticket = nullptr;
+    int window = 0;
+    unsigned gen_base = 0;
+    unsigned *gen = nullptr;
 };
 
 struct WgLaunchDesc {
@@ -46,9 +49,11 @@
 
 hipError_t gcsadmm_wg_set_lds(int n, int dtype, int lds_bytes);
 void gcsadmm_wg_launch(const gcsadmm_k::WgLaunchDesc &d, hipStream_t s);
+int gcsadmm_wg_resident_blocks(int n, int dtype, int box, int lds_bytes);
 
 hipError_t gcsadmm_wg_set_lds_t512(int n, int dtype, int lds_bytes);
 void gcsadmm_wg_launch_t512(const gcsadmm_k::WgLaunchDesc &d, hipStream_t s);
+int gcsadmm_wg_resident_blocks_t512(int n, int dtype, int box, int lds_bytes);
 
 hipError_t gcsadmm_wg_set_split_lds(int n, int dtype, int lds_bytes);
 void gcsadmm_wg_launch_split(const gcsadmm_k::WgLaunchDesc &d, const gcsadmm_k::WgSplitArgs &w, hipStream_t s);
diff --git a/gcs_admm_amd/solver.py b/gcs_admm_amd/solver.py
--- a/gcs_admm_amd/solver.py
+++ b/gcs_admm_amd/solver.py
@@ -114,6 +114,9 @@
     def set_fused_tail(self, mode: int = 1) -> bool:
         return bool(self.lib.gcsadmm_set_fused_tail(self.h, int(mode)))
 
+    def set_resident_window(self, window: int = 0) -> int:
+        return int(self.lib.gcsadmm_set_fused_tail(self.h, abi.resident_window_mode(window)))
+
     def enqueue_timed(self, k: int):
         vm, em = C.c_float(0), C.c_float(0)
         vl, el = C.c_int32(0), C.c_int32(0)
diff --git a/include/gcsadmm.h b/include/gcsadmm.h
--- a/include/gcsadmm.h
+++ b/include/gcsadmm.h
@@ -100,6 +100,7 @@
 
 gcsadmm_status gcsadmm_run(gcsadmm_handle h, const gcsadmm_state *st, int32_t k, double *trace_dev, void *stream);
 
+#define GCSADMM_RESIDENT_WINDOW(j) (2 | ((j) << 8))
 int32_t gcsadmm_set_fused_tail(gcsadmm_handle h, int32_t mode);
 
 gcsadmm_status gcsadmm_read_control(gcsadmm_handle h, gcsadmm_control_block *out, void *stream);
```

Result: slower. 10300 iterations/s (-1.6%).
